# trzy/FasterRCNN

Hardware: AMD Instinct MI355X
Metric: images/sec (600x1000) Faster-RCNN VGG-16 inference (higher is better)
Workload: dtype f32 (float32 tensors and accumulation; 15 GEMM layers in the f32x3 split-operand emulation = two fp16 terms per block-scaled operand, three fp16 MFMAs per product; 0 in f32x6 = three bf16 terms, six bf16 MFMAs; the other 2 on exact-f32 MFMA; strict exact-f32 everywhere: config.strict_f32_images_per_

## Files before the change

fasterrcnn_amd/csrc/api.hip:

```cpp
#include "common.h"
#include <algorithm>
#include <cmath>
#include <cstring>
#include <string>
#include <vector>
#include <new>

namespace frcnn {

static thread_local std::string g_hip_error;
void set_hip_error(hipError_t e) { g_hip_error = hipGetErrorString(e); }

static size_t align_up(size_t v, size_t a) { return (v + a - 1) / a * a; }

struct EventRec { int cls; hipEvent_t start, stop; };

}

using namespace frcnn;

struct frcnn_ctx {
    int max_h = 0, max_w = 0, max_rois = 0, max_images = 0;
    int max_fh = 0, max_fw = 0, a_cap = 0, pre_cap = 0;
    void* slab = nullptr;
// ... 435 lines not shown
    if (!out) return FRCNN_EINVAL;
    const unsigned* c = x3_saturation_counter();
    *out = c ? (unsigned long long)*reinterpret_cast<const volatile unsigned*>(c) : 0ull;
    return FRCNN_OK;
}

int frcnn_conv_nhwc_x3g(const float* d_x, const float* d_wp, const float* d_bias, const float* d_residual, float* d_y,
                        int N, int H, int W, int cin, int cout, int ksize, int stride, int pad, unsigned flags,
                        const float* d_xmax, const float* d_wmax, float* d_ymax, void* d_ws, size_t ws_bytes, void* stream)
{
    if (!d_x || !d_wp || !d_bias || !d_y || !d_xmax || !d_wmax) return FRCNN_EINVAL;
    if (flags & FRCNN_POOL2) return FRCNN_EUNSUPPORTED;
    const GatherX3 x3{d_xmax, d_wmax, d_ymax, nullptr, (flags & FRCNN_X3G_WSPLIT) != 0};
    return launch_conv_gather(d_x, d_wp, d_bias, d_residual, d_y, N, H, W, cin, cout, ksize, stride, pad, flags,
                              d_ws, ws_bytes, as_stream(stream), FRCNN_CONV_F32X3G, &x3);
}

int frcnn_pack_conv_x3g_weights(const float* d_wp, const float* d_wmax, void* d_out, int taps, int cout, int cin, void* stream)
{
    if (taps < 1 || cout < 1) return FRCNN_EINVAL;
    return launch_pack_x3g_weights(d_wp, d_wmax, d_out, (long long)taps * cout, cin, as_stream(stream));
}

int frcnn_conv_nhwc_x3g_tickets(const float* d_x, const float* d_wp, const float* d_bias, const float* d_residual, float* d_y,
                                int N, int H, int W, int cin, int cout, int ksize, int stride, int pad, unsigned flags,
                                const float* d_xmax, const float* d_wmax, float* d_ymax, void* d_ws, size_t ws_bytes,
                                unsigned* d_tile_counters, void* stream)
{
    static_assert(FRCNN_X3G_TILE_COUNTERS == GX_TILE_COUNTERS, "one bound on both sides of the ABI");
    if (!d_x || !d_wp || !d_bias || !d_y || !d_xmax || !d_wmax || !d_tile_counters) return FRCNN_EINVAL;
    if (flags & FRCNN_POOL2) return FRCNN_EUNSUPPORTED;
    const GatherX3 x3{d_xmax, d_wmax, d_ymax, d_tile_counters, (flags & FRCNN_X3G_WSPLIT) != 0};
    return launch_conv_gather(d_x, d_wp, d_bias, d_residual, d_y, N, H, W, cin, cout, ksize, stride, pad, flags,
                              d_ws, ws_bytes, as_stream(stream), FRCNN_CONV_F32X3G, &x3);
}

int frcnn_tensor_absmax(const float* d_x, long long n, float* d_out, void* stream)
{
    if (!d_x || !d_out) return FRCNN_EINVAL;
    return launch_tensor_absmax(d_x, n, d_out, as_stream(stream));
}

int frcnn_conv7x7_s2_c3(const float* d_x, const float* d_wp, const float* d_bias, float* d_y, int H, int W,
                        int cout, unsigned flags, void* stream)
{
    if (!d_x || !d_wp || !d_bias || !d_y) return FRCNN_EINVAL;
    return launch_conv7x7_s2_c3(d_x, d_wp, d_bias, d_y, H, W, cout, flags, as_stream(stream));
}

int frcnn_maxpool3x3_s2_nhwc(const float* d_x, float* d_y, int H, int W, int c, void* stream)
{
    if (!d_x || !d_y) return FRCNN_EINVAL;
    return launch_maxpool3x3_s2(d_x, d_y, H, W, c, as_stream(stream));
}

int frcnn_spatial_mean_nhwc(const float* d_x, float* d_y, int N, int H, int W, int c, void* stream)
{
    if (!d_x || !d_y) return FRCNN_EINVAL;
    return launch_spatial_mean(d_x, d_y, N, H, W, c, as_stream(stream));
}

size_t frcnn_linear_workspace_bytes(int M, int N, int K) { return linear_workspace_bytes(M, N, K); }

int frcnn_linear(const float* d_a, int lda, const float* d_w, const float* d_bias, float* d_y, int ldy,
                 int M, int N, int K, unsigned flags, void* d_ws, size_t ws_bytes, void* stream)
{
    if (!d_a || !d_w || !d_bias || !d_y) return FRCNN_EINVAL;
    return launch_linear(d_a, lda, d_w, d_bias, d_y, ldy, M, N, K, flags, d_ws, ws_bytes, as_stream(stream));
}

int frcnn_softmax_rows(const float* d_x, int ldx, float* d_y, int M, int ncls, void* stream)
{
    if (!d_x || !d_y) return FRCNN_EINVAL;
    return launch_softmax_rows(d_x, ldx, d_y, M, ncls, as_stream(stream));
}

int frcnn_rpn_proposals(frcnn_ctx* ctx, const float* d_head, int ld_head, const float* d_anchor_map,
                        const float* d_valid_map, int fh, int fw, int image_h, int image_w, int pre_nms,
                        int post_nms, float nms_threshold, float min_side, float* d_scores,
                        int32_t* d_sorted_idx, float* d_props, int32_t* d_counts, void* stream)
{
    if (!ctx || !d_head || !d_anchor_map || !d_scores || !d_sorted_idx || !d_props || !d_counts) return FRCNN_EINVAL;
    FRCNN_HIP_TRY(hipMemsetAsync(d_counts, 0, 4 * sizeof(int32_t), as_stream(stream)));
    return launch_rpn_proposals(ctx->ps, d_head, ld_head, d_anchor_map, d_valid_map, fh, fw, image_h, image_w,
                                pre_nms, post_nms, nms_threshold, min_side, d_scores, d_sorted_idx, d_props,
                                d_counts, as_stream(stream));
}

int frcnn_nms(frcnn_ctx* ctx, const float* d_boxes, const float* d_scores, int n, float threshold,
              int max_keep, int32_t* d_keep, int32_t* d_n_keep, void* stream)
{
    if (!ctx || !d_boxes || !d_scores || !d_keep || !d_n_keep) return FRCNN_EINVAL;
    return launch_nms(ctx->ps, d_boxes, d_scores, n, threshold, max_keep, d_keep, d_n_keep, as_stream(stream));
}

int frcnn_roi_pool(const float* d_fm, int fh, int fw, int c, const float* d_rois, const int32_t* d_n_rois,
                   int max_rois, int pooled, float spatial_scale, float* d_out, void* stream)
{
    if (!d_fm || !d_rois || !d_n_rois || !d_out) return FRCNN_EINVAL;
    return launch_roi_pool(d_fm, fh, fw, c, d_rois, d_n_rois, max_rois, pooled, spatial_scale, d_out,
                           as_stream(stream));
}

int frcnn_roi_pool_x3t(const float* d_fm, int fh, int fw, int c, const float* d_rois, const int32_t* d_n_rois, int max_rois, int pooled,
                       float spatial_scale, float* d_cmax, float* d_inv_scale, void* d_rec, int rec_rows, void* stream)
{
    if (!d_fm || !d_rois || !d_n_rois || !d_cmax || !d_inv_scale || !d_rec) return FRCNN_EINVAL;
    return launch_roi_pool_x3t(d_fm, fh, fw, c, d_rois, d_n_rois, max_rois, pooled, spatial_scale, d_cmax, d_inv_scale, d_rec, rec_rows,
                               as_stream(stream));
}

int frcnn_roi_align(const float* d_fm, int fh, int fw, int c, const float* d_rois, const int32_t* d_n_rois, int max_rois,
                    int pooled, float spatial_scale, int sampling_ratio, int aligned, float* d_out, void* stream)
{
    if (!d_fm || !d_rois || !d_n_rois || !d_out) return FRCNN_EINVAL;
    return launch_roi_align(d_fm, fh, fw, c, d_rois, d_n_rois, max_rois, pooled, spatial_scale, sampling_ratio, aligned, d_out,
                            as_stream(stream));
}

int frcnn_roi_align_backward(const float* d_rois, int n_rois, int fh, int fw, int c, int pooled, float spatial_scale,
                             int sampling_ratio, int aligned, const float* d_dout, float* d_dfm, int accumulate, void* stream)
{
    if (!d_dfm || (n_rois > 0 && (!d_rois || !d_dout))) return FRCNN_EINVAL;
    return launch_roi_align_backward(d_rois, n_rois, fh, fw, c, pooled, spatial_scale, sampling_ratio, aligned, d_dout, d_dfm,
                                     accumulate, as_stream(stream));
}

int frcnn_detections(const float* d_props, const float* d_classes, const float* d_deltas,
                     const int32_t* d_n_rois, int max_rois, int ncls, int image_h, int image_w,
                     float score_threshold, float nms_threshold, double* d_out, int32_t* d_out_cnt, void* stream)
{
    if (!d_props || !d_classes || !d_deltas || !d_n_rois || !d_out || !d_out_cnt) return FRCNN_EINVAL;
    return launch_detections(d_props, d_classes, d_deltas, d_n_rois, max_rois, ncls, image_h, image_w,
                             score_threshold, nms_threshold, d_out, d_out_cnt, as_stream(stream));
}

int frcnn_label_proposals(const float* d_props, const int32_t* d_n_props, int max_props,
                          const float* d_gt_boxes, const int32_t* d_gt_class_idx, int n_gt, int num_classes,
                          float min_background_iou, float min_object_iou,
                          const float box_delta_means[4], const float box_delta_stds[4],
                          float* d_out_props, int32_t* d_out_class_idx, float* d_out_gt_classes,
                          float* d_out_gt_box_deltas, int32_t* d_out_count, void* stream)
{
    if ((!d_props && max_props > 0) || !d_n_props || !d_gt_boxes || !d_gt_class_idx || !box_delta_means || !box_delta_stds ||
        !d_out_props || !d_out_class_idx || !d_out_gt_classes || !d_out_gt_box_deltas || !d_out_count)
        return FRCNN_EINVAL;
    if (!(min_background_iou < min_object_iou)) return FRCNN_EINVAL;
    return launch_label_proposals(d_props, d_n_props, max_props, d_gt_boxes, d_gt_class_idx, n_gt, num_classes,
                                  min_background_iou, min_object_iou, box_delta_means, box_delta_stds, d_out_props,
                                  d_out_class_idx, d_out_gt_classes, d_out_gt_box_deltas, d_out_count, as_stream(stream));
}

int frcnn_gather_rows(const float* d_src, const int32_t* d_idx, int n, int row_floats, float* d_dst, void* stream)
{
    if (n > 0 && (!d_src || !d_idx || !d_dst)) return FRCNN_EINVAL;
    return launch_gather_rows(d_src, d_idx, n, row_floats, d_dst, as_stream(stream));
}

int frcnn_rpn_loss(const float* d_head, int ld_head, int cells, const int32_t* d_sample, int n_sample,
                   const float* d_rpn_map, float* d_losses, float* d_grad_head, void* stream)
{
    if (!d_head || (n_sample > 0 && !d_sample) || !d_rpn_map || !d_losses) return FRCNN_EINVAL;
    return launch_rpn_loss(d_head, ld_head, cells, d_sample, n_sample, d_rpn_map, d_losses, d_grad_head, as_stream(stream));
}

int frcnn_detector_loss(const float* d_classes, const float* d_deltas, const float* d_gt_classes,
// ... 371 lines not shown
    proposal_scratch_carve(c->ps, ps_base, c->a_cap, c->pre_cap, 2048);
    *out = c;
    return FRCNN_OK;
}

int frcnn_ctx_create_proposals(frcnn_ctx** out, int max_image_h, int max_image_w)
{
    if (!out || max_image_h < 16 || max_image_w < 16) return FRCNN_EINVAL;
    frcnn_ctx* c = new (std::nothrow) frcnn_ctx();
    if (!c) return FRCNN_ENOMEM;
    c->max_h = max_image_h; c->max_w = max_image_w; c->max_rois = 0;
    c->max_fh = cdiv(max_image_h, 16); c->max_fw = cdiv(max_image_w, 16);
    c->a_cap = c->max_fh * c->max_fw * 9;
    if (c->a_cap < 16384) c->a_cap = 16384;
    c->pre_cap = 16384;
    const size_t total = align_up(proposal_scratch_bytes(c->a_cap, c->pre_cap, 2048), 256);
    hipError_t e = hipMalloc(&c->slab, total);
    if (e != hipSuccess) { set_hip_error(e); delete c; return FRCNN_ENOMEM; }
    c->slab_bytes = total;
    proposal_scratch_carve(c->ps, c->slab, c->a_cap, c->pre_cap, 2048);
    *out = c;
    return FRCNN_OK;
}

void frcnn_ctx_destroy(frcnn_ctx* ctx)
{
    if (!ctx) return;
    for (auto& r : ctx->recs) { (void)hipEventDestroy(r.start); (void)hipEventDestroy(r.stop); }
    for (auto e : ctx->free_events) (void)hipEventDestroy(e);
    if (ctx->slab) (void)hipFree(ctx->slab);
    if (ctx->wino_ws) (void)hipFree(ctx->wino_ws);
    if (ctx->wx_ws) (void)hipFree(ctx->wx_ws);
    if (ctx->x3f_cmax) (void)hipFree(ctx->x3f_cmax);
    if (ctx->roi_rec) (void)hipFree(ctx->roi_rec);
    if (ctx->rx_rec) (void)hipFree(ctx->rx_rec);
    if (ctx->rx_ws) (void)hipFree(ctx->rx_ws);
    if (ctx->rx_aux) (void)hipFree(ctx->rx_aux);
    if (ctx->gx_max) (void)hipFree(ctx->gx_max);
    if (ctx->gx_cnt) (void)hipFree(ctx->gx_cnt);
    delete ctx;
}

size_t frcnn_ctx_bytes(const frcnn_ctx* ctx) { return ctx ? ctx->slab_bytes + ctx->wino_ws_bytes + ctx->wx_ws_bytes + ctx->rx_rec_bytes + ctx->rx_ws_bytes + (ctx->roi_rec ? (size_t)ctx->rec_rows * (49 * 512 + 4096) * 6 : 0) : 0; }

int frcnn_ctx_timing_enable(frcnn_ctx* ctx, int enable)
{
    if (!ctx) return FRCNN_EINVAL;
    ctx->timing = enable != 0;
    return FRCNN_OK;
}

int frcnn_ctx_timing_read(frcnn_ctx* ctx, double ms[FRCNN_NUM_KCLASS], int64_t launches[FRCNN_NUM_KCLASS], int reset)
{
    if (!ctx || !ms || !launches) return FRCNN_EINVAL;
    for (auto& r : ctx->recs) {
        FRCNN_HIP_TRY(hipEventSynchronize(r.stop));
        float t = 0.f;
        FRCNN_HIP_TRY(hipEventElapsedTime(&t, r.start, r.stop));
        ctx->t_ms[r.cls] += t;
        ctx->t_cnt[r.cls] += 1;
        ctx->free_events.push_back(r.start);
        ctx->free_events.push_back(r.stop);
    }
    ctx->recs.clear();
    for (int i = 0; i < FRCNN_NUM_KCLASS; ++i) { ms[i] = ctx->t_ms[i]; launches[i] = ctx->t_cnt[i]; }
    if (reset) for (int i = 0; i < FRCNN_NUM_KCLASS; ++i) { ctx->t_ms[i] = 0; ctx->t_cnt[i] = 0; }
    return FRCNN_OK;
}

int frcnn_ctx_tensor(frcnn_ctx* c, int which, void** d_ptr, size_t* bytes)
{
    if (!c || !d_ptr || !bytes) return FRCNN_EINVAL;
    const size_t fmsz = (size_t)c->last_fh * c->last_fw;
    switch (which) {
        case 0: *d_ptr = c->fm; *bytes = fmsz * c->last_c * 4; break;
        case 1: *d_ptr = c->rpn_head; *bytes = fmsz * 128 * 4; break;
        case 2: *d_ptr = c->scores; *bytes = fmsz * 9 * 4; break;
        case 3: *d_ptr = c->sorted_idx; *bytes = (size_t)c->last_pre * 4; break;
        case 4: *d_ptr = c->roi_out; *bytes = (size_t)c->last_post * 49 * c->last_c * 4; break;
        case 5: *d_ptr = c->fc2_out; *bytes = (size_t)c->last_post * c->last_vec * 4; break;
        case 6: *d_ptr = c->anchor_map; *bytes = fmsz * 9 * 16; break;
        case 7: *d_ptr = c->valid_map; *bytes = fmsz * 9 * 4; break;
        case 8: *d_ptr = c->head_logits; *bytes = (size_t)c->last_post * c->last_head_ld * 4; break;
        default: return FRCNN_EINVAL;
    }
    return FRCNN_OK;
}

namespace {
int ensure_wino_ws(frcnn_ctx* c)
{
    if (c->wino_ws) return FRCNN_OK;
    size_t need = 0;
    const int shapes[5][3] = {{4, 128, 256}, {4, 256, 256}, {8, 256, 512}, {8, 512, 512}, {16, 512, 512}};
    for (auto& sh : shapes) {
        const size_t b = c->max_h > 0 ? conv3x3_winograd_workspace_bytes(1, c->max_h / sh[0], c->max_w / sh[0], sh[1], sh[2]) : 0;
        if (b > need) need = b;
    }
    const int rois = c->max_rois > c->max_head_rois ? c->max_rois : c->max_head_rois;
    const size_t b1 = c->max_fh > 0 ? conv3x3_winograd_workspace_bytes(1, c->max_fh, c->max_fw, 1024, 1024) : 0;
    const size_t b2 = rois > 0 ? conv3x3_winograd_workspace_bytes(rois, 4, 4, 512, 512) : 0;
    if (b1 > need) need = b1;
    if (b2 > need) need = b2;
    if (need == 0) return FRCNN_EINVAL;
    hipError_t e = hipMalloc(&c->wino_ws, need);
    if (e != hipSuccess) { set_hip_error(e); c->wino_ws = nullptr; return FRCNN_ENOMEM; }
    c->wino_ws_bytes = need;
    return FRCNN_OK;
}

int run_winograd_layer(frcnn_ctx* c, const float* x, const float* u, const float* b, float* y, int N, int h, int w, int ci, int co,
                       unsigned flags, hipStream_t s)
{
    float *V = nullptr, *M = nullptr;
    int r = winograd_plan(N, h, w, ci, co, flags, c->wino_ws, c->wino_ws_bytes, &V, &M);
    if (r) return r;
    { Scope _t(c, 6, s); r = launch_winograd_input(x, V, N, h, w, ci, s); }
    if (r) return r;
    { Scope _g(c, 7, s); r = launch_winograd_gemm(V, u, M, N, h, w, ci, co, s); }
    if (r) return r;
    Scope _o(c, 6, s);
    return launch_winograd_output(M, b, y, N, h, w, co, flags, s);
}

int ensure_wx_ws(frcnn_ctx* c, size_t layer_need, hipStream_t s)
{
    if (c->wx_ws && layer_need <= c->wx_ws_bytes) return FRCNN_OK;
    size_t need = layer_need;
    const int shapes[4][4] = {{c->max_h / 8, c->max_w / 8, 256, 512}, {c->max_h / 8, c->max_w / 8, 512, 512},
                              {c->max_fh, c->max_fw, 512, 512}, {c->max_fh, c->max_fw, 1024, 1024}};
    for (auto& sh : shapes) {
        const size_t b = conv3x3_winograd_x6_workspace_bytes(1, sh[0], sh[1], sh[2], sh[3]);
        if (b > need) need = b;
    }
    if (need == 0) return FRCNN_EINVAL;
    if (c->wx_ws) {
        FRCNN_HIP_TRY(hipStreamSynchronize(s));
        (void)hipFree(c->wx_ws);
        c->wx_ws = nullptr; c->wx_ws_bytes = 0;
    }
    hipError_t e = hipMalloc(&c->wx_ws, need);
    if (e != hipSuccess) { set_hip_error(e); c->wx_ws = nullptr; return FRCNN_ENOMEM; }
    e = hipMemsetAsync(c->wx_ws, 0, need, s);
    if (e != hipSuccess) { set_hip_error(e); (void)hipFree(c->wx_ws); c->wx_ws = nullptr; return FRCNN_EHIP; }
    c->wx_ws_bytes = need;
    return FRCNN_OK;
}

int ensure_fc_records(frcnn_ctx* c, hipStream_t s)
{
    if (c->roi_rec) return FRCNN_OK;
    const size_t b1 = (size_t)c->rec_rows * 49 * 512 * 6, b2 = (size_t)c->rec_rows * 4096 * 6;
    const size_t b3 = align_up((size_t)c->rec_rows * sizeof(float), 256), b4 = align_up((size_t)c->max_fh * c->max_fw * sizeof(float), 256);
    void* p = nullptr;
    hipError_t e = hipMalloc(&p, b1 + b2 + 2 * b3 + b4);
    if (e != hipSuccess) { set_hip_error(e); return FRCNN_ENOMEM; }
    e = hipMemsetAsync(p, 0, b1 + b2 + 2 * b3 + b4, s);
    if (e != hipSuccess) { set_hip_error(e); (void)hipFree(p); return FRCNN_EHIP; }
    c->roi_rec = p;
    c->fc1_rec = static_cast<unsigned char*>(p) + b1;
    c->roi_inv = reinterpret_cast<float*>(static_cast<unsigned char*>(p) + b1 + b2);
    c->fc1_inv = reinterpret_cast<float*>(static_cast<unsigned char*>(p) + b1 + b2 + b3);
    c->fm_cmax = reinterpret_cast<float*>(static_cast<unsigned char*>(p) + b1 + b2 + 2 * b3);
    return FRCNN_OK;
}

int run_wino_x6_layer(frcnn_ctx* c, const float* x, const void* urec, const float* b, float* y, int h, int w, int ci, int co,
                      unsigned flags, hipStream_t s, int N = 1)
// ... 16 lines not shown

int run_wino_x3_layer(frcnn_ctx* c, const float* x, const void* ublob, const float* b, float* y, int h, int w, int ci, int co,
                      unsigned flags, hipStream_t s, int N = 1, const float* cmax_ready = nullptr, float* cmax_out = nullptr)
{
    if (N == 1 && !conv3x3_uses_winograd_x6(ci, co)) return FRCNN_EINVAL;
    int r = ensure_wx_ws(c, conv3x3_winograd_x3_workspace_bytes(N, h, w, ci, co), s);
    if (r) return r;
    void *V = nullptr, *G = nullptr;
    float *M = nullptr, *vinv = nullptr, *cmax = nullptr;
    size_t gb = 0;
    r = winograd_x3_plan(N, h, w, ci, co, flags, c->wx_ws, c->wx_ws_bytes, &V, &vinv, &cmax, &M, &G, &gb);
    if (r) return r;
    { Scope _t(c, 8, s); r = launch_winograd_x3_input(x, cmax, V, vinv, N, h, w, ci, s, cmax_ready); }
    if (r) return r;
    { Scope _g(c, 9, s); r = launch_winograd_x3_gemm(V, vinv, ublob, M, N, h, w, ci, co, G, gb, s); }
    if (r) return r;
    Scope _o(c, 8, s);
    return launch_winograd_output(M, b, y, N, h, w, co, flags, s, cmax_out);
}

int ensure_x3f_cmax(frcnn_ctx* c, size_t need, hipStream_t s)
{
    if (c->x3f_cmax && c->x3f_cmax_bytes >= need) return FRCNN_OK;
    if (c->x3f_cmax) { FRCNN_HIP_TRY(hipStreamSynchronize(s)); (void)hipFree(c->x3f_cmax); c->x3f_cmax = nullptr; c->x3f_cmax_bytes = 0; }
    const size_t cap = std::max(need, (size_t)c->max_h * c->max_w * sizeof(float));
    hipError_t e = hipMalloc(reinterpret_cast<void**>(&c->x3f_cmax), 3 * cap);
    if (e != hipSuccess) { set_hip_error(e); c->x3f_cmax = nullptr; return FRCNN_ENOMEM; }
    c->x3f_cmax_bytes = cap;
    return FRCNN_OK;
}
float* x3f_cmax_buffer(frcnn_ctx* c, int which) { return reinterpret_cast<float*>(reinterpret_cast<unsigned char*>(c->x3f_cmax) + (size_t)which * c->x3f_cmax_bytes); }

int run_wino_x3f_layer(frcnn_ctx* c, const float* x, const void* ublob, const float* b, float* y, int h, int w, int ci, int co,
                       unsigned flags, hipStream_t s, const float* cmax_ready = nullptr, float* cmax_out = nullptr)
{
    int r = ensure_x3f_cmax(c, conv3x3_winograd_x3_fused_workspace_bytes(1, h, w), s);
    if (r) return r;
    Scope _w(c, 10, s);
    return launch_conv3x3_winograd_x3_fused(x, ublob, b, y, 1, h, w, ci, co, flags, x3f_cmax_buffer(c, 0), c->x3f_cmax_bytes, s, cmax_ready, cmax_out);
}

int run_wino_fused_layer(frcnn_ctx* c, bool , const float* x, const float* u, const float* b, float* y, int h, int w, int ci,
                         int co, unsigned flags, hipStream_t s, int n_maps = 1)
{
    Scope _w(c, 7, s);
    return launch_conv3x3_winograd_fused(x, u, b, y, h, w, ci, co, flags, s, n_maps);
}

struct BlocksTargetScope {
    explicit BlocksTargetScope(int t, int wino_rows = 0, int x6_tiles = 0) { conv3x3_set_blocks_target(t); linear_batched_set_tile(wino_rows); gemm_x6t_set_tiles(x6_tiles); }
    ~BlocksTargetScope() { conv3x3_set_blocks_target(0); linear_batched_set_tile(0); gemm_x6t_set_tiles(0); }
};
}

int frcnn_vgg16_forward(frcnn_ctx* c, const frcnn_vgg16_weights* w, const frcnn_forward_params* p,
                        const float* d_image, int H, int W, const float* d_anchor_map,
                        const float* d_valid_map, float* d_props, float* d_classes, float* d_deltas,
                        int32_t* d_counts, void* stream)
{
    if (!c || !w || !p || !d_image || !d_props || !d_classes || !d_deltas || !d_counts) return FRCNN_EINVAL;
    if (H < 16 || W < 16 || H > c->max_h || W > c->max_w) return FRCNN_EINVAL;
    if (p->post_nms < 1 || p->post_nms > c->max_rois || p->pre_nms < 1 || p->pre_nms > c->pre_cap) return FRCNN_EINVAL;
    if (w->num_classes < 2 || w->num_classes > FRCNN_MAX_NUM_CLASSES) return FRCNN_EUNSUPPORTED;
    for (int i = 0; i < 13; ++i) if (!w->conv_w[i] || !w->conv_b[i]) return FRCNN_EINVAL;
    if (!w->rpn_conv_w || !w->rpn_conv_b || !w->rpn_head_w || !w->rpn_head_b || !w->fc1_w || !w->fc1_b ||
        !w->fc2_w || !w->fc2_b || !w->head_w || !w->head_b)
        return FRCNN_EINVAL;
    hipStream_t s = as_stream(stream);
    const unsigned R = FRCNN_RELU, RP = FRCNN_RELU | FRCNN_POOL2;
    int rc;
    if (p->math_mode != FRCNN_MATH_F32 && p->math_mode != FRCNN_MATH_F32_WINOGRAD) return FRCNN_EINVAL;
    if (p->conv_blocks_target < 0) return FRCNN_EINVAL;
    if (p->fc_math_mode != FRCNN_FC_F32 && p->fc_math_mode != FRCNN_FC_F32X6T && p->fc_math_mode != FRCNN_FC_F32X3T) return FRCNN_EINVAL;
    if ((p->roi_op != FRCNN_ROI_POOL && p->roi_op != FRCNN_ROI_ALIGN) || p->roi_sampling_ratio > 2) return FRCNN_EINVAL;
    if (p->winograd_tile_rows != 0 && p->winograd_tile_rows != 64 && p->winograd_tile_rows != 128) return FRCNN_EINVAL;
    if (p->x6_gemm_tiles < 0 || p->x6_gemm_tiles > 2) return FRCNN_EINVAL;
    if ((p->winograd_x3_mask & ~p->winograd_x6_mask) != 0) return FRCNN_EINVAL;
    BlocksTargetScope target_scope(p->conv_blocks_target, p->winograd_tile_rows, p->x6_gemm_tiles);
    const bool wino = p->math_mode == FRCNN_MATH_F32_WINOGRAD;
    if (p->winograd_x6_mask != 0 && (!wino || (p->winograd_x6_mask & ~0x3FFE) != 0)) return FRCNN_EINVAL;
    if (p->winograd_x3f_mask != 0 && (!wino || (p->winograd_x3f_mask & ~0x3FFE) != 0 || (p->winograd_x3f_mask & p->winograd_x6_mask) != 0)) return FRCNN_EINVAL;
    int layer_index = 0;
    const float* cmax_ready = nullptr;
    size_t cmax_used = 0, cmax_cleared = 0;
    if (wino && ((p->winograd_x3f_mask | (p->winograd_x3_mask & p->winograd_x6_mask)) & 0x1FFE) != 0) {
        int r0 = ensure_x3f_cmax(c, (size_t)H * W * sizeof(float), s);
        if (r0) return r0;
        static const int co_of[13] = {0, 64, 128, 128, 256, 256, 256, 512, 512, 512, 512, 512, 512};
        static const bool pool_of[13] = {false, true, false, true, false, false, true, false, false, true, false, false, false};
        size_t want = 0;
        int eh = H, ew = W;
        for (int li = 1; li <= 12; ++li) {
            const bool f3 = ((p->winograd_x3f_mask >> li) & 1) != 0;
            const bool t3 = !f3 && ((p->winograd_x6_mask >> li) & 1) && ((p->winograd_x3_mask >> li) & 1);
            const unsigned efl = FRCNN_RELU | (pool_of[li] ? FRCNN_POOL2 : 0u);
            if (pool_of[li]) { eh /= 2; ew /= 2; }
            if ((f3 || t3) && (f3 || winograd_output_emits_cmax(co_of[li], efl))) want += ((size_t)eh * ew + 63) & ~(size_t)63;
        }
        if (want > 2 * c->x3f_cmax_bytes / sizeof(float)) return FRCNN_EINVAL;
        cmax_cleared = want;
        if (want) FRCNN_HIP_TRY(hipMemsetAsync(x3f_cmax_buffer(c, 1), 0, cmax_cleared * sizeof(float), s));
    }
    auto conv3 = [&](const float* xin, const float* wgt, const float* bs, float* yout, int hh, int ww, int ci, int co,
                     unsigned fl) -> int {
        ++layer_index;
        const float* in_cmax = cmax_ready;
        cmax_ready = nullptr;
        const bool is_x3f = wino && ((p->winograd_x3f_mask >> layer_index) & 1);
        const bool is_x3 = wino && !is_x3f && ((p->winograd_x6_mask >> layer_index) & 1) && ((p->winograd_x3_mask >> layer_index) & 1);
        float* out_cmax = nullptr;
        if ((is_x3f || is_x3) && layer_index != FRCNN_X6_RPN_TRUNK_BIT && (fl & FRCNN_RELU) && (is_x3f || winograd_output_emits_cmax(co, fl))) {
            const int oh = (fl & FRCNN_POOL2) ? hh / 2 : hh, ow = (fl & FRCNN_POOL2) ? ww / 2 : ww;
            const size_t need = ((size_t)oh * ow + 63) & ~(size_t)63;
            out_cmax = x3f_cmax_buffer(c, 1) + cmax_used;
            cmax_used += need;
            if (cmax_used > cmax_cleared) return FRCNN_EINVAL;
        }
        int r1;
        if (is_x3f)
            r1 = run_wino_x3f_layer(c, xin, wgt, bs, yout, hh, ww, ci, co, fl, s, in_cmax, out_cmax);
        else if (is_x3)
            r1 = run_wino_x3_layer(c, xin, wgt, bs, yout, hh, ww, ci, co, fl, s, 1, in_cmax, out_cmax);
        else if (wino && ((p->winograd_x6_mask >> layer_index) & 1))
            r1 = run_wino_x6_layer(c, xin, wgt, bs, yout, hh, ww, ci, co, fl, s);
        else
            r1 = -9999;
        if (r1 != -9999) {
            if (r1 == FRCNN_OK) cmax_ready = out_cmax;
            return r1;
        }
        if (wino && conv3x3_uses_winograd_fused(ci, co)) {
            return run_wino_fused_layer(c, p->conv_blocks_target == 0, xin, wgt, bs, yout, hh, ww, ci, co, fl, s);
        }
        Scope _d(c, 0, s);
        return launch_conv3x3_nhwc(xin, wgt, bs, yout, hh, ww, ci, co, fl, c->conv_ws, c->conv_ws_bytes, s);
    };
#define STEP(cls, call) do { Scope _sc(c, cls, s); rc = (call); } while (0); if (rc) return rc
#define CONV(call) do { rc = (call); } while (0); if (rc) return rc

    float *A = c->act_a, *B = c->act_b;
    int h = H, wd = W;
    float* c11_cmax = (wino && ((p->winograd_x3f_mask >> 1) & 1)) ? x3f_cmax_buffer(c, 0) : nullptr;
    STEP(1, launch_conv3x3_c3(d_image, w->conv_w[0], w->conv_b[0], A, h, wd, 64, R, s, c11_cmax));
    cmax_ready = c11_cmax;
    CONV(conv3(A, w->conv_w[1], w->conv_b[1], B, h, wd, 64, 64, RP));   h /= 2; wd /= 2;
    CONV(conv3(B, w->conv_w[2], w->conv_b[2], A, h, wd, 64, 128, R));
    CONV(conv3(A, w->conv_w[3], w->conv_b[3], B, h, wd, 128, 128, RP)); h /= 2; wd /= 2;
    CONV(conv3(B, w->conv_w[4], w->conv_b[4], A, h, wd, 128, 256, R));
    CONV(conv3(A, w->conv_w[5], w->conv_b[5], B, h, wd, 256, 256, R));
    CONV(conv3(B, w->conv_w[6], w->conv_b[6], A, h, wd, 256, 256, RP)); h /= 2; wd /= 2;
    CONV(conv3(A, w->conv_w[7], w->conv_b[7], B, h, wd, 256, 512, R));
    CONV(conv3(B, w->conv_w[8], w->conv_b[8], A, h, wd, 512, 512, R));
    CONV(conv3(A, w->conv_w[9], w->conv_b[9], B, h, wd, 512, 512, RP)); h /= 2; wd /= 2;
    CONV(conv3(B, w->conv_w[10], w->conv_b[10], A, h, wd, 512, 512, R));
    CONV(conv3(A, w->conv_w[11], w->conv_b[11], B, h, wd, 512, 512, R));
    CONV(conv3(B, w->conv_w[12], w->conv_b[12], c->fm, h, wd, 512, 512, R));
    const float* fm_cmax_ready = cmax_ready;
    const int fh = h, fw = wd;
    c->last_fh = fh; c->last_fw = fw; c->last_pre = p->pre_nms; c->last_post = p->post_nms; c->last_c = 512; c->last_vec = 4096;

    CONV(conv3(c->fm, w->rpn_conv_w, w->rpn_conv_b, c->rpn_trunk, fh, fw, 512, 512, R));
    STEP(2, launch_linear(c->rpn_trunk, 512, w->rpn_head_w, w->rpn_head_b, c->rpn_head, 128, fh * fw, 45, 512,
                          0u, c->lin_ws, c->lin_ws_bytes, s));
    const float* amap = d_anchor_map;
    const float* vmap = d_valid_map;
    if (!amap || !vmap) {
        if (c->anc_h != H || c->anc_w != W || c->anc_fh != fh || c->anc_fw != fw) {
            STEP(5, launch_anchors(H, W, fh, fw, 16, c->anchor_map, c->valid_map, s));
            c->anc_h = H; c->anc_w = W; c->anc_fh = fh; c->anc_fw = fw;
        }
        amap = c->anchor_map; vmap = c->valid_map;
    }
    FRCNN_HIP_TRY(hipMemsetAsync(d_counts, 0, 4 * sizeof(int32_t), s));
    STEP(3, launch_rpn_proposals(c->ps, c->rpn_head, 128, amap, p->allow_edge_proposals ? nullptr : vmap, fh, fw,
                                 H, W, p->pre_nms, p->post_nms, p->rpn_nms_threshold, p->min_side, c->scores,
                                 c->sorted_idx, d_props, d_counts, s));

    const int R_ = p->post_nms;
    const bool fc_x6t = p->fc_math_mode == FRCNN_FC_F32X6T;
    const bool fc_x3t = p->fc_math_mode == FRCNN_FC_F32X3T;
    if (fc_x6t || fc_x3t) { rc = ensure_fc_records(c, s); if (rc) return rc; }
    if (fc_x3t) {
        const int rr = c->rec_rows;
        const size_t w1rec = x3t_record_bytes(4096, 49 * 512), w2rec = x3t_record_bytes(4096, 4096);
        const float* w1inv = reinterpret_cast<const float*>(reinterpret_cast<const unsigned char*>(w->fc1_w) + w1rec);
        const float* w2inv = reinterpret_cast<const float*>(reinterpret_cast<const unsigned char*>(w->fc2_w) + w2rec);
        if (p->roi_op == FRCNN_ROI_ALIGN) {
            STEP(4, launch_roi_align(c->fm, fh, fw, 512, d_props, d_counts + 2, R_, 7, 1.0f / 16.0f, p->roi_sampling_ratio, 0, c->roi_out, s));
            STEP(2, launch_rows_scale_x3t(c->roi_out, 49 * 512, 0, c->roi_inv, R_, rr, 49 * 512, 1, s));
            STEP(2, launch_split_rows_x3t(c->roi_out, 49 * 512, 0, c->roi_inv, c->roi_rec, R_, rr, 49 * 512, 1, s));
        } else {
            STEP(4, launch_roi_pool_x3t(c->fm, fh, fw, 512, d_props, d_counts + 2, R_, 7, 1.0f / 16.0f,
                                        fm_cmax_ready ? const_cast<float*>(fm_cmax_ready) : c->fm_cmax, c->roi_inv, c->roi_rec, rr, s, fm_cmax_ready != nullptr));
        }
        STEP(2, launch_gemm_x3t(c->roi_rec, c->roi_inv, rr, 0, 0, w->fc1_w, w1inv, 4096, 0, 0, w->fc1_b, nullptr, c->fc1_out, 4096, 0, R_, 4096,
                                49 * 512, 1, R, c->lin_ws, c->lin_ws_bytes, s, 0));
        STEP(2, launch_rows_scale_x3t(c->fc1_out, 4096, 0, c->fc1_inv, R_, rr, 4096, 1, s));
        STEP(2, launch_split_rows_x3t(c->fc1_out, 4096, 0, c->fc1_inv, c->fc1_rec, R_, rr, 4096, 1, s));
        STEP(2, launch_gemm_x3t(c->fc1_rec, c->fc1_inv, rr, 0, 0, w->fc2_w, w2inv, 4096, 0, 0, w->fc2_b, nullptr, c->fc2_out, 4096, 0, R_, 4096,
                                4096, 1, R, c->lin_ws, c->lin_ws_bytes, s, 2));
    } else
    if (fc_x6t) {
        const int rr = c->rec_rows;
        if (p->roi_op == FRCNN_ROI_ALIGN) {
            STEP(4, launch_roi_align(c->fm, fh, fw, 512, d_props, d_counts + 2, R_, 7, 1.0f / 16.0f, p->roi_sampling_ratio, 0, c->roi_out, s));
            STEP(2, launch_split_rows_x6t(c->roi_out, 49 * 512, 0, c->roi_rec, R_, rr, 49 * 512, 1, s));
        } else {
            STEP(4, launch_roi_pool_x6t(c->fm, fh, fw, 512, d_props, d_counts + 2, R_, 7, 1.0f / 16.0f, c->roi_rec, rr, s));
        }
        static const int fc_tiles = []() { const char* e = frcnn_knob("FRCNN_FC_TILES"); return e ? atoi(e) : 0; }();
        STEP(2, launch_gemm_x6t(c->roi_rec, rr, 0, w->fc1_w, 4096, 0, w->fc1_b, nullptr, c->fc1_out, 4096, 0, R_, 4096, 49 * 512, 1, R,
                                c->lin_ws, c->lin_ws_bytes, s, fc_tiles));
        STEP(2, launch_split_rows_x6t(c->fc1_out, 4096, 0, c->fc1_rec, R_, rr, 4096, 1, s));
        STEP(2, launch_gemm_x6t(c->fc1_rec, rr, 0, w->fc2_w, 4096, 0, w->fc2_b, nullptr, c->fc2_out, 4096, 0, R_, 4096, 4096, 1, R,
                                c->lin_ws, c->lin_ws_bytes, s, fc_tiles));
    } else
    {
        if (p->roi_op == FRCNN_ROI_ALIGN) {
            STEP(4, launch_roi_align(c->fm, fh, fw, 512, d_props, d_counts + 2, R_, 7, 1.0f / 16.0f, p->roi_sampling_ratio, 0, c->roi_out, s));
        } else {
            STEP(4, launch_roi_pool(c->fm, fh, fw, 512, d_props, d_counts + 2, R_, 7, 1.0f / 16.0f, c->roi_out, s));
        }
        STEP(2, launch_linear(c->roi_out, 49 * 512, w->fc1_w, w->fc1_b, c->fc1_out, 4096, R_, 4096, 49 * 512, R,
                              c->lin_ws, c->lin_ws_bytes, s));
        STEP(2, launch_linear(c->fc1_out, 4096, w->fc2_w, w->fc2_b, c->fc2_out, 4096, R_, 4096, 4096, R,
                              c->lin_ws, c->lin_ws_bytes, s));
    }
    const int ncls = w->num_classes, nd = (ncls - 1) * 4;
    const int hld = cdiv(ncls + nd, 128) * 128;
    c->last_head_ld = hld;
    STEP(2, launch_linear(c->fc2_out, 4096, w->head_w, w->head_b, c->head_logits, hld, R_, ncls + nd, 4096, 0u,
                          c->lin_ws, c->lin_ws_bytes, s));
    STEP(5, launch_head_finish(c->head_logits, hld, R_, ncls, nd, d_classes, d_deltas, s));
#undef STEP
#undef CONV
    return FRCNN_OK;
}

namespace {
int run_conv1x1_x6(frcnn_ctx* c, const float* x, const void* wrec, const float* bias, const float* residual, float* y, int N, int h,
                   int w, int cin, int cout, int stride, unsigned flags, int cls, hipStream_t s, int ksize = 1)
{
    if (cin % 16 != 0 || cout % 4 != 0 || (ksize != 1 && ksize != 3)) return FRCNN_EINVAL;
    const int ho = (h - 1) / stride + 1, wo = (w - 1) / stride + 1;
    const int K = ksize == 3 ? 9 * cin : cin;
    const long long rows = (long long)N * ho * wo;
    if (rows > 0x7fffffffLL / 8) return FRCNN_EINVAL;
    const int M = (int)rows;
    const int Mp = cdiv(M, gemm_x6t_row_tile(M)) * gemm_x6t_row_tile(M), Np = cdiv(cout, gemm_x6t_col_tile(cout)) * gemm_x6t_col_tile(cout);
    const size_t need = x6t_record_bytes(Mp, K), gneed = gemm_x6t_workspace_bytes(M, cout, K, 1);
    if (need > c->rx_rec_bytes) {
        if (c->rx_rec) { FRCNN_HIP_TRY(hipStreamSynchronize(s)); (void)hipFree(c->rx_rec); c->rx_rec = nullptr; c->rx_rec_bytes = 0; }
        hipError_t e = hipMalloc(&c->rx_rec, need);
        if (e != hipSuccess) { set_hip_error(e); c->rx_rec = nullptr; return FRCNN_ENOMEM; }
        c->rx_rec_bytes = need;
    }
    if (gneed > c->rx_ws_bytes) {
        if (c->rx_ws) { FRCNN_HIP_TRY(hipStreamSynchronize(s)); (void)hipFree(c->rx_ws); c->rx_ws = nullptr; c->rx_ws_bytes = 0; }
        hipError_t e = hipMalloc(&c->rx_ws, gneed);
        if (e != hipSuccess) { set_hip_error(e); c->rx_ws = nullptr; return FRCNN_ENOMEM; }
        c->rx_ws_bytes = gneed;
    }
    int rc;
    { Scope _t(c, 8, s); rc = ksize == 3 ? launch_split_patches3x3_x6t(x, c->rx_rec, N, h, w, cin, stride, Mp, s)
                                        : launch_split_pixels_x6t(x, c->rx_rec, N, h, w, cin, stride, Mp, s); }
    if (rc) return rc;
    Scope _g(c, cls, s);
    return launch_gemm_x6t(c->rx_rec, Mp, 0, wrec, Np, 0, bias, residual, y, cout, 0, M, cout, K, 1, flags, c->rx_ws, c->rx_ws_bytes, s);
}

int run_conv1x1_x3(frcnn_ctx* c, const float* x, const void* wblob, const float* bias, const float* residual, float* y, int N, int h,
                   int w, int cin, int cout, int stride, unsigned flags, int cls, hipStream_t s, int ksize = 1)
{
    if (cin % 16 != 0 || cout % 4 != 0 || (ksize != 1 && ksize != 3)) return FRCNN_EINVAL;
    const int ho = (h - 1) / stride + 1, wo = (w - 1) / stride + 1;
    const int K = ksize == 3 ? 9 * cin : cin;
    const long long rows = (long long)N * ho * wo;
    if (rows > 0x7fffffffLL / 8) return FRCNN_EINVAL;
    const int M = (int)rows;
    const int Mp = cdiv(M, gemm_x6t_row_tile(M)) * gemm_x6t_row_tile(M), Np = cdiv(cout, gemm_x6t_col_tile(cout)) * gemm_x6t_col_tile(cout);
    const size_t need = x3t_record_bytes(Mp, K), gneed = gemm_x3t_workspace_bytes(M, cout, K, 1);
    const size_t aneed = (size_t)Mp + (size_t)N * h * w;
    if (need > c->rx_rec_bytes) {
        if (c->rx_rec) { FRCNN_HIP_TRY(hipStreamSynchronize(s)); (void)hipFree(c->rx_rec); c->rx_rec = nullptr; c->rx_rec_bytes = 0; }
        hipError_t e = hipMalloc(&c->rx_rec, need);
        if (e != hipSuccess) { set_hip_error(e); c->rx_rec = nullptr; return FRCNN_ENOMEM; }
        c->rx_rec_bytes = need;
    }
    if (gneed > c->rx_ws_bytes) {
        if (c->rx_ws) { FRCNN_HIP_TRY(hipStreamSynchronize(s)); (void)hipFree(c->rx_ws); c->rx_ws = nullptr; c->rx_ws_bytes = 0; }
        hipError_t e = hipMalloc(&c->rx_ws, gneed);
        if (e != hipSuccess) { set_hip_error(e); c->rx_ws = nullptr; return FRCNN_ENOMEM; }
        c->rx_ws_bytes = gneed;
    }
    if (aneed > c->rx_aux_floats) {
        if (c->rx_aux) { FRCNN_HIP_TRY(hipStreamSynchronize(s)); (void)hipFree(c->rx_aux); c->rx_aux = nullptr; c->rx_aux_floats = 0; }
        hipError_t e = hipMalloc(reinterpret_cast<void**>(&c->rx_aux), aneed * sizeof(float));
        if (e != hipSuccess) { set_hip_error(e); c->rx_aux = nullptr; return FRCNN_ENOMEM; }
        c->rx_aux_floats = aneed;
    }
    float* ainv = c->rx_aux;
    float* cmax = c->rx_aux + Mp;
    int rc;
    {
        Scope _t(c, 8, s);
        static const bool two_pass = frcnn_knob("FRCNN_SPLIT_TWO_PASS") != nullptr;
        rc = (ksize == 3 || two_pass) ? launch_pixel_absmax(x, cmax, (long long)N * h * w, cin, s) : FRCNN_OK;
        if (!rc) rc = ksize == 3 ? launch_split_patches3x3_x3t(x, cmax, c->rx_rec, ainv, N, h, w, cin, stride, Mp, s)
                                 : launch_split_pixels_x3t(x, two_pass ? cmax : nullptr, c->rx_rec, ainv, N, h, w, cin, stride, Mp, s);
    }
    if (rc) return rc;
    const float* winv = reinterpret_cast<const float*>(static_cast<const unsigned char*>(wblob) + x3t_record_bytes(Np, K));
    Scope _g(c, cls, s);
    return launch_gemm_x3t(c->rx_rec, ainv, Mp, 0, 0, wblob, winv, Np, 0, 0, bias, residual, y, cout, 0, M, cout, K, 1, flags, c->rx_ws,
                           c->rx_ws_bytes, s);
}
// ... 448 lines not shown
```

fasterrcnn_amd/csrc/common.h:

```cpp
#pragma once
#include <hip/hip_runtime.h>
#include <stdint.h>
#include <stddef.h>
#include <stdlib.h>
#include "../../include/frcnn_hip.h"

typedef float f32x4  __attribute__((ext_vector_type(4)));
typedef float f32x16 __attribute__((ext_vector_type(16)));

inline const char* frcnn_knob(const char* name)
{
#ifdef FRCNN_EXPERIMENT_KNOBS
    return getenv(name);
#else
    (void)name;
    return nullptr;
#endif
}

namespace frcnn {

void set_hip_error(hipError_t e);

inline int check_launch() {
    hipError_t e = hipGetLastError();
    if (e != hipSuccess) { set_hip_error(e); return FRCNN_EHIP; }
    return FRCNN_OK;
}

#define FRCNN_HIP_TRY(expr)                                   \
    do {                                                      \
        hipError_t _e = (expr);                               \
        if (_e != hipSuccess) { ::frcnn::set_hip_error(_e); return FRCNN_EHIP; } \
    } while (0)

static inline int cdiv(int a, int b) { return (a + b - 1) / b; }

struct DeviceOnce { unsigned char done[64]; };
inline int set_max_dynamic_lds(DeviceOnce& once, const void* kern, size_t bytes)
{
    int dev = 0;
    FRCNN_HIP_TRY(hipGetDevice(&dev));
    if (dev < 0 || dev >= 64) return FRCNN_EINVAL;
    if (!once.done[dev]) {
        FRCNN_HIP_TRY(hipFuncSetAttribute(kern, hipFuncAttributeMaxDynamicSharedMemorySize, (int)bytes));
        once.done[dev] = 1;
    }
    return FRCNN_OK;
}
#define FRCNN_MAX_LDS_ONCE(kern, bytes)                                                                  \
    do {                                                                                                 \
        static ::frcnn::DeviceOnce _once = {};                                                           \
        const int _rc = ::frcnn::set_max_dynamic_lds(_once, reinterpret_cast<const void*>(kern), (bytes)); \
        if (_rc) return _rc;                                                                             \
    } while (0)

static inline bool conv3x3_uses_winograd(int cin, int cout) { return cin >= 128 && cout >= 256 && cin % 16 == 0 && cout % 128 == 0; }
static inline bool resnet_block_uses_winograd(int width, int stride) { return stride == 1 && width >= 256 && width % 128 == 0; }

struct KernelTimer;

}

namespace frcnn {

int launch_anchors(int image_h, int image_w, int fh, int fw, int feature_pixels,
                   float* anchor_map, float* valid_map, hipStream_t s);

int launch_pack_conv3x3(const float* w, float* wp, int cout, int cin, hipStream_t s);
int launch_pack_conv3x3_c3(const float* w, float* wp, int cout, hipStream_t s);
int launch_pack_fc_chw_to_hwc(const float* w, float* wp, int out_f, int c, int phw, hipStream_t s);
int launch_pack_stack_rows(const float* w1, const float* b1, int n1, const float* w2, const float* b2,
                           int n2, int k, int n_pad, float* wo, float* bo, hipStream_t s);

int launch_conv3x3_c3(const float* x, const float* wp, const float* b, float* y, int H, int W,
                      int cout, unsigned flags, hipStream_t s, float* cmax_out = nullptr);
size_t conv3x3_workspace_bytes(int H, int W, int cin, int cout);
int conv3x3_blocks_target();
void conv3x3_set_blocks_target(int target);
int launch_conv3x3_nhwc(const float* x, const float* wp, const float* b, float* y, int H, int W,
                        int cin, int cout, unsigned flags, void* ws, size_t ws_bytes, hipStream_t s);
int launch_maxpool2x2(const float* x, float* y, int H, int W, int c, hipStream_t s);

size_t conv_gather_workspace_bytes(int N, int H, int W, int cin, int cout, int R, int stride, int pad);
#define FRCNN_CONV_F32X3G 2
static constexpr int GX_TILE_COUNTERS = 16384;
struct GatherX3 { const float* xmax; const float* wmax; float* ymax; unsigned* tile_counters = nullptr; bool wsplit = false; bool trusted = false; };
int launch_pack_x3g_weights(const float* wp, const float* wmax, void* out, long long rows, int cin, hipStream_t s);
int launch_conv_gather(const float* x, const float* wp, const float* bias, const float* residual, float* y,
                       int N, int H, int W, int cin, int cout, int R, int stride, int pad, unsigned flags,
                       void* ws, size_t ws_bytes, hipStream_t s, int math = FRCNN_GRAD_F32, const GatherX3* x3 = nullptr);
unsigned* x3_saturation_counter();
int launch_tensor_absmax(const float* x, long long n, float* out, hipStream_t s);
int launch_conv7x7_s2_c3(const float* x, const float* wp, const float* b, float* y, int H, int W, int cout,
                         unsigned flags, hipStream_t s);
int launch_maxpool3x3_s2(const float* x, float* y, int H, int W, int c, hipStream_t s);
int launch_spatial_mean(const float* x, float* y, int N, int H, int W, int c, hipStream_t s);
int launch_fold_bn_pack(const float* w, const float* gamma, const float* beta, const float* mean, const float* var,
                        float eps, int cout, int cin, int ksize, float* wp, float* bp, hipStream_t s);

size_t linear_workspace_bytes(int M, int N, int K);
int launch_linear(const float* a, int lda, const float* w, const float* bias, float* y, int ldy,
                  int M, int N, int K, unsigned flags, void* ws, size_t ws_bytes, hipStream_t s);
int launch_linear_batched(const float* a, int lda, size_t a_stride, const float* w, size_t w_stride, float* y, int ldy,
                          size_t y_stride, int M, int N, int K, int batches, hipStream_t s);
void linear_batched_set_tile(int rows);
size_t conv3x3_winograd_workspace_bytes(int N, int H, int W, int cin, int cout);
int launch_pack_conv3x3_winograd(const float* w, const float* scale, float* u, int cout, int cin, hipStream_t s);
int launch_pack_conv3x3_winograd_taps(const float* wp, float* u, int cout, int cin, int data_gradient, hipStream_t s);
int launch_conv3x3_winograd(const float* x, const float* u, const float* b, float* y, int N, int H, int W, int cin, int cout,
                            unsigned flags, void* ws, size_t ws_bytes, hipStream_t s);
int winograd_plan(int N, int H, int W, int cin, int cout, unsigned flags, void* ws, size_t ws_bytes, float** V, float** M);
int launch_winograd_input(const float* x, float* V, int N, int H, int W, int cin, hipStream_t s);
int launch_winograd_gemm(const float* V, const float* u, float* M, int N, int H, int W, int cin, int cout, hipStream_t s);
int launch_winograd_output(const float* M, const float* b, float* y, int N, int H, int W, int cout, unsigned flags, hipStream_t s,
                           float* cmax_out = nullptr);
bool winograd_output_emits_cmax(int cout, unsigned flags);
static inline bool conv3x3_uses_winograd_fused(int cin, int cout) { return cin >= 64 && cin % 16 == 0 && cout >= 64 && cout % 64 == 0; }
static inline bool resnet_block_uses_winograd_fused(int n_maps, int width, int stride)
{
    return n_maps == 1 && stride == 1 && conv3x3_uses_winograd_fused(width, width);
}
bool conv3x3_winograd_fused_ok(int H, int W, int cin, int cout);
int launch_pack_conv3x3_winograd_fused(const float* w, const float* scale, float* u, int cout, int cin, hipStream_t s);
int launch_pack_conv3x3_winograd_fused_taps(const float* wp, float* u, int cout, int cin, int data_gradient, hipStream_t s);
int launch_conv3x3_winograd_fused(const float* x, const float* u, const float* b, float* y, int H, int W, int cin, int cout,
                                  unsigned flags, hipStream_t s, int n_maps = 1);
int gemm_x6t_row_tile(int M);
int gemm_x6t_col_tile(int N);
size_t x6t_record_bytes(int rows_padded, int K);
int launch_split_rows_x6t(const float* a, int lda, size_t a_batch_floats, void* rec, int R, int rows_padded, int K, int batches, hipStream_t s);
bool gemm_x6t_shape_ok(int M, int N, int K, int batches);
size_t gemm_x6t_workspace_bytes(int M, int N, int K, int batches);
void gemm_x6t_set_tiles(int mode);
int launch_gemm_x6t(const void* a_rec, int a_rows, size_t a_batch_bytes, const void* b_rec, int b_rows, size_t b_batch_bytes,
                    const float* bias, const float* residual, float* c, int ldc, size_t c_batch_floats, int M, int N, int K, int batches,
                    unsigned flags, void* ws, size_t ws_bytes, hipStream_t s, int tiles_mode = -1);
int launch_split_pixels_x6t(const float* x, void* rec, int N, int H, int W, int C, int stride, int rows_padded, hipStream_t s);
int gemm_x6t_get_tiles();
int launch_gemm_x6t_reduce(const float* ws, const float* bias, const float* residual, float* c, int ldc, size_t c_batch_floats, int M, int N,
                           int batches, int splits, int relu, hipStream_t s);
size_t x3t_record_bytes(int rows_padded, int K);
int launch_rows_scale_x3t(const float* a, int lda, size_t a_batch_floats, float* inv_scale, int R, int rows_padded, int K, int batches,
                          hipStream_t s);
int launch_split_rows_x3t(const float* a, int lda, size_t a_batch_floats, const float* inv_scale, void* rec, int R, int rows_padded, int K,
                          int batches, hipStream_t s);
int launch_split_pixels_x3t(const float* x, const float* cmax, void* rec, float* inv, int N, int H, int W, int C, int stride, int rows_padded,
                            hipStream_t s);
int launch_split_patches3x3_x3t(const float* x, const float* cmax, void* rec, float* inv, int N, int H, int W, int C, int stride,
                                int rows_padded, hipStream_t s);
size_t gemm_x3t_workspace_bytes(int M, int N, int K, int batches);
int launch_gemm_x3t(const void* a_rec, const float* a_inv, int a_rows, size_t a_batch_bytes, size_t a_inv_batch, const void* b_rec,
                    const float* b_inv, int b_rows, size_t b_batch_bytes, size_t b_inv_batch, const float* bias, const float* residual,
                    float* c, int ldc, size_t c_batch_floats, int M, int N, int K, int batches, unsigned flags, void* ws, size_t ws_bytes,
                    hipStream_t s, int tiles_mode = -1);
size_t x3t_blob_bytes(int rows_padded, int K, int batches);
int launch_pack_rows_x3t(const float* a, int lda, size_t a_batch_floats, void* blob, int R, int rows_padded, int K, int batches, hipStream_t s);
int launch_pixel_absmax(const float* x, float* cmax, long long pixels, int C, hipStream_t s);
size_t conv3x3_winograd_x3_pack_bytes(int cout, int cin);
int launch_pack_conv3x3_winograd_x3(const float* u_f32, void* ublob, int cout, int cin, hipStream_t s);
size_t conv3x3_winograd_x3_workspace_bytes(int N, int H, int W, int cin, int cout);
int winograd_x3_plan(int N, int H, int W, int cin, int cout, unsigned flags, void* ws, size_t ws_bytes, void** V, float** vinv, float** cmax,
                     float** M, void** G, size_t* g_bytes);
int launch_winograd_x3_input(const float* x, float* cmax, void* vrec, float* vinv, int N, int H, int W, int cin, hipStream_t s,
                             const float* cmax_ready = nullptr);
int launch_winograd_x3_gemm(const void* vrec, const float* vinv, const void* ublob, float* M, int N, int H, int W, int cin, int cout, void* gws,
                            size_t gws_bytes, hipStream_t s);
int launch_conv3x3_winograd_x3(const float* x, const void* ublob, const float* b, float* y, int N, int H, int W, int cin, int cout,
                               unsigned flags, void* ws, size_t ws_bytes, hipStream_t s,
                               const float* cmax_ready = nullptr, float* cmax_out = nullptr);
size_t conv3x3_winograd_x3_fused_workspace_bytes(int N, int H, int W);
int launch_conv3x3_winograd_x3_fused(const float* x, const void* ublob, const float* b, float* y, int N, int H, int W, int cin, int cout,
                                     unsigned flags, void* ws, size_t ws_bytes, hipStream_t s, const float* cmax_ready = nullptr,
                                     float* cmax_out = nullptr);
int launch_roi_pool_x3t(const float* fm, int fh, int fw, int c, const float* rois, const int32_t* n_rois, int max_rois, int pooled,
                        float scale, float* cmax, float* inv, void* rec, int rec_rows, hipStream_t s, bool cmax_ready = false);
bool conv3x3_uses_winograd_x6(int cin, int cout);
size_t conv3x3_winograd_x6_pack_bytes(int cout, int cin);
size_t conv3x3_winograd_x6_workspace_bytes(int N, int H, int W, int cin, int cout);
int launch_pack_conv3x3_winograd_x6(const float* w, const float* scale, void* urec, int cout, int cin, hipStream_t s);
int launch_winograd_x6_input(const float* x, void* vrec, int N, int H, int W, int cin, hipStream_t s);
int launch_winograd_x6_gemm(const void* vrec, const void* urec, float* M, int N, int H, int W, int cin, int cout, void* gws, size_t gws_bytes, hipStream_t s);
int winograd_x6_plan(int N, int H, int W, int cin, int cout, unsigned flags, void* ws, size_t ws_bytes, void** V, float** M, void** G, size_t* g_bytes);
int launch_conv3x3_winograd_x6(const float* x, const void* urec, const float* b, float* y, int N, int H, int W, int cin, int cout,
                               unsigned flags, void* ws, size_t ws_bytes, hipStream_t s);
int launch_split_patches3x3_x6t(const float* x, void* rec, int N, int H, int W, int C, int stride, int rows_padded, hipStream_t s);
int launch_softmax_rows(const float* x, int ldx, float* y, int M, int ncls, hipStream_t s);
int launch_head_finish(const float* x, int ldx, int M, int ncls, int ndelta, float* classes,
                       float* deltas, hipStream_t s);

struct ProposalScratch {
    unsigned long long* keys;
    float*    boxes_all;
    float*    cand_boxes;
    float*    cand_scores;
    unsigned long long* mask;
    int32_t*  keep;
    int       a_cap, pre_cap, post_cap;
};
size_t proposal_scratch_bytes(int a_cap, int pre_cap, int post_cap);
void   proposal_scratch_carve(ProposalScratch& ps, void* base, int a_cap, int pre_cap, int post_cap);

int launch_rpn_proposals(const ProposalScratch& ps, const float* head, int ld_head,
                         const float* anchor_map, const float* valid_map, int fh, int fw,
                         int image_h, int image_w, int pre_nms, int post_nms, float nms_thr,
                         float min_side, float* scores, int32_t* sorted_idx, float* props,
                         int32_t* counts, hipStream_t s);
int launch_nms(const ProposalScratch& ps, const float* boxes, const float* scores, int n, float thr,
               int max_keep, int32_t* keep, int32_t* n_keep, hipStream_t s);

int launch_roi_pool(const float* fm, int fh, int fw, int c, const float* rois, const int32_t* n_rois,
                    int max_rois, int pooled, float scale, float* out, hipStream_t s);
int launch_roi_pool_x6t(const float* fm, int fh, int fw, int c, const float* rois, const int32_t* n_rois,
                        int max_rois, int pooled, float scale, void* rec, int rec_rows, hipStream_t s);

int launch_roi_align(const float* fm, int fh, int fw, int c, const float* rois, const int32_t* n_rois, int max_rois, int pooled,
                     float scale, int sampling_ratio, int aligned, float* out, hipStream_t s);
int launch_roi_align_backward(const float* rois, int n_rois, int fh, int fw, int c, int pooled, float scale, int sampling_ratio,
                              int aligned, const float* dout, float* dfm, int accumulate, hipStream_t s);

int launch_rpn_targets(const float* anchor_map, const float* valid_map, int A, const float* gt, int M,
                       double obj_thr, double bg_thr, float* rpn_map, int32_t* obj_idx, int32_t* bg_idx,
                       int32_t* counts, void* ws, hipStream_t s);

size_t preprocess_workspace_bytes(int H, int W, int Ho, int Wo);
int launch_preprocess(const unsigned char* rgb, int H, int W, int Ho, int Wo, int bgr, int flip, float scaling,
                      const float* means, const float* stds, float* out, unsigned char* out_u8, void* ws,
                      size_t ws_bytes, hipStream_t s);

int launch_detections(const float* props, const float* classes, const float* deltas,
                      const int32_t* n_rois, int max_rois, int ncls, int image_h, int image_w,
                      float score_thr, float nms_thr, double* out, int32_t* out_cnt, hipStream_t s);

size_t gemm_tn_workspace_bytes(int M, int N, int R, int taps);
int launch_gemm_tn(const float* A, int lda, const float* B, int ldb, float* C, int ldc, int M, int N, int R,
                   void* ws, size_t ws_bytes, hipStream_t s, int math = FRCNN_GRAD_F32);
int launch_conv3x3_wgrad(const float* x, const float* dz, float* dwp, int H, int W, int cin, int cout,
                         void* ws, size_t ws_bytes, hipStream_t s, int math = FRCNN_GRAD_F32);
int launch_label_proposals(const float* props, const int32_t* n_props, int max_props, const float* gt,
                           const int32_t* gt_cls, int M, int ncls, float bg_thr, float obj_thr,
                           const float means[4], const float stds[4], float* out_props, int32_t* out_cls,
                           float* out_onehot, float* out_deltas, int32_t* out_count, hipStream_t s);
int launch_gather_rows(const float* src, const int32_t* idx, int n, int row_floats, float* dst, hipStream_t s);
int launch_rpn_loss(const float* head, int ld, int cells, const int32_t* sample, int n_sample, const float* rpn_map,
                    float* losses, float* d_head, hipStream_t s);
int launch_detector_loss(const float* classes, const float* deltas, const float* gt_onehot, const float* gt_deltas,
                         int S, int ncls, float* losses, float* d_logits, int ld, hipStream_t s);
int launch_relu_backward(float* dy, const float* y, size_t n, hipStream_t s);
int launch_dropout(float* x, size_t n, float p, float scale, const uint64_t* seed, uint32_t stream_id, uint32_t rank,
                   uint8_t* keep_out, hipStream_t s);
int launch_dropout_relu_backward(float* dy, const float* y, size_t n, float scale, hipStream_t s);
int launch_add_inplace(float* a, const float* b, size_t n, hipStream_t s);
int launch_maxpool2x2_backward(const float* x, const float* dy, float* dx, int H, int W, int C, hipStream_t s);
size_t roi_pool_backward_workspace_bytes(int n_rois, int pooled, int C);
int launch_roi_pool_backward(const float* fm, int fh, int fw, int C, const float* rois, int n_rois, int pooled,
                             float scale, const float* dout, float* dfm, int accumulate, void* ws, size_t ws_bytes,
                             hipStream_t s);
int launch_transpose(const float* x, int ldi, float* y, int ldo, int rows, int cols, hipStream_t s);
int launch_pack_conv3x3_dgrad(const float* wp, float* wd, int cout, int cin, hipStream_t s);
int launch_conv_wgrad(const float* x, const float* dz, float* dwp, int N, int H, int W, int cin, int cout, int ks, int stride,
                      int pad, void* ws, size_t ws_bytes, hipStream_t s, int math = FRCNN_GRAD_F32);
size_t conv_dgrad_workspace_bytes(int N, int H, int W, int cin, int cout, int R, int stride, int pad);
int launch_conv_dgrad(const float* dz, const float* wd, const float* residual, float* dx, int N, int H, int W, int cin,
                      int cout, int R, int stride, int pad, void* ws, size_t ws_bytes, hipStream_t s, int math = FRCNN_GRAD_F32);
int launch_pack_conv_dgrad(const float* wp, float* wd, int taps, int cout, int cin, hipStream_t s);
int launch_scale_rows(const float* src, const float* scale, float* dst, int taps, int cout, int cin, hipStream_t s);
int launch_bn_scale_shift(const float* gamma, const float* beta, const float* mean, const float* var, float eps, int c,
                          float* scale, float* shift, hipStream_t s);
int launch_spatial_mean_backward(const float* dy, float* dx, int N, int H, int W, int c, hipStream_t s);
int launch_sgd(float* w, const float* g, float* buf, size_t n, float lr, float momentum, float weight_decay, int first,
               hipStream_t s);
int launch_sgd_fold(float* w, const float* g, float* buf, size_t n, float lr, float momentum, float weight_decay, int first,
                    const float* scale, float* folded, int cout, int cin, hipStream_t s);

}
```

fasterrcnn_amd/csrc/conv.hip:

```cpp
#include "common.h"
#include <cstdlib>
#include <type_traits>

namespace frcnn {

static constexpr int LDK = 20;
static constexpr int HC  = 34;

template <int WM, int WN>
struct ConvCfg {
    static constexpr int TR  = 2 * WM;
    static constexpr int BN  = 64 * WN;
    static constexpr int HR  = TR + 2;
    static constexpr int HALO_F = HR * HC * LDK;
    static constexpr int WT_F   = BN * LDK;
    static constexpr int NHP = HR * HC * 4;
    static constexpr int NH  = (NHP + 255) / 256;
    static constexpr int NW  = BN * 4 / 256;
    static constexpr size_t LDS_BYTES = (size_t)(2 * HALO_F + 2 * WT_F) * sizeof(float);
};

template <int WM, int WN, bool POOL>
__global__ __launch_bounds__(256)
void conv3x3_mfma_kernel(const float* __restrict__ x, const float* __restrict__ wp,
// ... 225 lines not shown
                               float* __restrict__ y, int H, int W, int Cout, int relu, int pool)
{
    const int C4 = Cout >> 2;
    const int Ho = pool ? H >> 1 : H, Wo = pool ? W >> 1 : W;
    const size_t total = (size_t)Ho * Wo * C4;
    const size_t plane = (size_t)H * W * Cout;
    for (size_t i = (size_t)blockIdx.x * 256 + threadIdx.x; i < total; i += (size_t)gridDim.x * 256) {
        const int c4 = (int)(i % C4);
        const size_t p = i / C4;
        const int ox = (int)(p % Wo), oy = (int)(p / Wo);
        const f32x4 bv = reinterpret_cast<const f32x4*>(bias)[c4];
        f32x4 best;
        const int np = pool ? 4 : 1;
        for (int q = 0; q < np; ++q) {
            const int iy = pool ? 2 * oy + (q >> 1) : oy, ix = pool ? 2 * ox + (q & 1) : ox;
            const size_t off = ((size_t)iy * W + ix) * Cout + 4 * c4;
            f32x4 v = *reinterpret_cast<const f32x4*>(ws + off);
            for (int k = 1; k < ksplit; ++k) {
                const f32x4 t = *reinterpret_cast<const f32x4*>(ws + k * plane + off);
#pragma unroll
                for (int j = 0; j < 4; ++j) v[j] += t[j];
            }
            if (q == 0) best = v;
            else {
#pragma unroll
                for (int j = 0; j < 4; ++j) best[j] = fmaxf(best[j], v[j]);
            }
        }
#pragma unroll
        for (int j = 0; j < 4; ++j) {
            float t = best[j] + bv[j];
            best[j] = relu ? fmaxf(t, 0.f) : t;
        }
        reinterpret_cast<f32x4*>(y)[i] = best;
    }
}

__global__ __launch_bounds__(256)
void conv3x3_c3_kernel(const float* __restrict__ x, const float* __restrict__ wp,
                       const float* __restrict__ bias, float* __restrict__ y,
                       int H, int W, int Cout, int relu)
{
    const int pix = blockIdx.x * 256 + threadIdx.x;
    if (pix >= H * W) return;
    const int yy = pix / W, xx = pix - yy * W;
    float in[27];
#pragma unroll
    for (int ci = 0; ci < 3; ++ci)
#pragma unroll
        for (int r = 0; r < 3; ++r)
#pragma unroll
            for (int s = 0; s < 3; ++s) {
                const int gy = yy + r - 1, gx = xx + s - 1;
                const bool inb = gy >= 0 && gy < H && gx >= 0 && gx < W;
                in[ci * 9 + r * 3 + s] = inb ? x[((size_t)ci * H + gy) * W + gx] : 0.f;
            }
    for (int og = 0; og < (Cout >> 4); ++og) {
        float acc[16];
#pragma unroll
        for (int o = 0; o < 16; ++o) acc[o] = 0.f;
        const float* wg = wp + og * 16;
#pragma unroll
        for (int k = 0; k < 27; ++k)
#pragma unroll
            for (int o = 0; o < 16; ++o) acc[o] = fmaf(in[k], wg[k * Cout + o], acc[o]);
        float* out = y + (size_t)pix * Cout + og * 16;
#pragma unroll
        for (int o4 = 0; o4 < 4; ++o4) {
            f32x4 v;
#pragma unroll
            for (int j = 0; j < 4; ++j) {
                float t = acc[o4 * 4 + j] + bias[og * 16 + o4 * 4 + j];
                v[j] = relu ? fmaxf(t, 0.f) : t;
            }
            *reinterpret_cast<f32x4*>(out + 4 * o4) = v;
        }
    }
}

typedef float c3_f32x2 __attribute__((ext_vector_type(2)));
template <bool RELU, bool CMAX, int BPC>
__global__ __launch_bounds__(256, BPC)
void conv3x3_c3_p_kernel(const float* __restrict__ x, const float* __restrict__ wp, const float* __restrict__ bias,
                         float* __restrict__ y, int H, int W, float* __restrict__ cmax_out, int tiles_x, int ntiles)
{
    constexpr int COUT = 64, SEG = 64, ROWS = 2, LW = 68;
    constexpr int NEL = 3 * (ROWS + 2) * (SEG + 2);
    __shared__ __attribute__((aligned(16))) float in_s[2][3][ROWS + 2][LW];
    const int tid = threadIdx.x, q = tid & 15, g = tid >> 4;
    int e_off[4], e_rc[4];
    const int HW = H * W;
#pragma unroll
    for (int k = 0; k < 4; ++k) {
        const int e = tid + 256 * k;
        const int ci = e / ((ROWS + 2) * (SEG + 2)), rem = e - ci * (ROWS + 2) * (SEG + 2);
        const int r = rem / (SEG + 2), c = rem - r * (SEG + 2);
        e_off[k] = ci * HW + (r - 1) * W + c - 1;
        e_rc[k] = e < NEL ? (c | (r << 8) | (((ci * (ROWS + 2) + r) * LW + c) << 12)) : -1;
    }
    auto fetch = [&](int tile, float (&v)[4]) {
        const int ty = tile / tiles_x, tx = tile - ty * tiles_x;
        const int y0 = ty * ROWS, x0 = tx * SEG;
        const int base = y0 * W + x0;
#pragma unroll
        for (int k = 0; k < 4; ++k) {
            const int gy = y0 + ((e_rc[k] >> 8) & 7) - 1, gx = x0 + (e_rc[k] & 127) - 1;
            const bool inb = e_rc[k] >= 0 && gy >= 0 && gy < H && gx >= 0 && gx < W;
            v[k] = inb ? x[base + e_off[k]] : 0.f;
        }
    };
    auto stage = [&](int buf, const float (&v)[4]) {
        float* dst = &in_s[buf][0][0][0];
#pragma unroll
        for (int k = 0; k < 4; ++k)
            if (e_rc[k] >= 0) dst[e_rc[k] >> 12] = v[k];
    };
    f32x4 wq[27];
#pragma unroll
    for (int k = 0; k < 27; ++k) wq[k] = *reinterpret_cast<const f32x4*>(wp + k * COUT + 4 * q);
    const f32x4 bq = *reinterpret_cast<const f32x4*>(bias + 4 * q);
    int tile = blockIdx.x;
    if (tile >= ntiles) return;
    {
        float v[4];
        fetch(tile, v);
        stage(0, v);
    }
    __syncthreads();
    int buf = 0;
    for (; tile < ntiles; tile += gridDim.x) {
        const int next = tile + gridDim.x;
        float nv_[4];
        if (next < ntiles) fetch(next, nv_);
        const int ty = tile / tiles_x, tx = tile - ty * tiles_x;
        const int y0 = ty * ROWS, x0 = tx * SEG;
#pragma unroll
        for (int row = 0; row < ROWS; ++row) {
            const int yy = y0 + row;
            if (yy >= H) break;
            c3_f32x2 acc[4][2];
#pragma unroll
            for (int i = 0; i < 4; ++i) acc[i][0] = acc[i][1] = c3_f32x2{0.f, 0.f};
#pragma unroll
            for (int ci = 0; ci < 3; ++ci)
#pragma unroll
                for (int r = 0; r < 3; ++r) {
                    const float* src = &in_s[buf][ci][row + r][4 * g];
                    const f32x4 a = *reinterpret_cast<const f32x4*>(src);
                    c3_f32x2 pr[3];
                    pr[0] = c3_f32x2{a[0], a[1]}; pr[1] = c3_f32x2{a[2], a[3]};
                    pr[2] = *reinterpret_cast<const c3_f32x2*>(src + 4);
#pragma unroll
                    for (int s_ = 0; s_ < 3; ++s_) {
                        const f32x4 w4 = wq[ci * 9 + r * 3 + s_];
                        const c3_f32x2 wlo = {w4[0], w4[1]}, whi = {w4[2], w4[3]};
#pragma unroll
                        for (int i = 0; i < 4; ++i) {
                            const int k = i + s_;
                            if ((k & 1) == 0) {
                                asm("v_pk_fma_f32 %0, %1, %2, %0 op_sel_hi:[0,1,1]" : "+v"(acc[i][0]) : "v"(pr[k >> 1]), "v"(wlo));
                                asm("v_pk_fma_f32 %0, %1, %2, %0 op_sel_hi:[0,1,1]" : "+v"(acc[i][1]) : "v"(pr[k >> 1]), "v"(whi));
                            } else {
                                asm("v_pk_fma_f32 %0, %1, %2, %0 op_sel:[1,0,0]" : "+v"(acc[i][0]) : "v"(pr[k >> 1]), "v"(wlo));
                                asm("v_pk_fma_f32 %0, %1, %2, %0 op_sel:[1,0,0]" : "+v"(acc[i][1]) : "v"(pr[k >> 1]), "v"(whi));
                            }
                        }
                    }
                }
// ... 83 lines not shown
    dim3 grid(cdiv(W, 32), cdiv(H, C::TR), cout_tiles * ksplit);
    auto kern = conv3x3_mfma_kernel<WM, WN, POOL>;
    FRCNN_MAX_LDS_ONCE(kern, C::LDS_BYTES);
    hipLaunchKernelGGL(kern, grid, dim3(256), C::LDS_BYTES, s, x, wp, b, y, H, W, cin, cout, relu, cout_tiles,
                       cdiv(nchunks, ksplit), ksplit > 1 ? ws : (float*)nullptr);
    return check_launch();
}

static thread_local int g_blocks_target_override = 0;
void conv3x3_set_blocks_target(int target) { g_blocks_target_override = target > 0 ? target : 0; }

static int conv_blocks_target()
{
    static int env_target = -1;
    if (env_target < 0) {
        const char* e = frcnn_knob("FRCNN_CONV_BLOCKS_TARGET");
        env_target = e ? atoi(e) : 0;
        if (env_target < 0) env_target = 0;
    }
    if (env_target > 0) return env_target;
    return g_blocks_target_override > 0 ? g_blocks_target_override : 1280;
}

static int choose_ksplit(int H, int W, int cin, int cout)
{
    const bool narrow = (cout % 128) != 0;
    const int tr = narrow ? 8 : 4, bn = narrow ? 64 : 128;
    const int blocks = cdiv(W, 32) * cdiv(H, tr) * (cout / bn);
    const int nchunks = cin / 16;
    const int target = conv_blocks_target();
    if (blocks * 2 > target) return 1;
    if ((size_t)H * W * cout * sizeof(float) > ((size_t)40 << 20)) return 1;
    int k = 1;
    while (k * 2 * blocks <= target && nchunks % (k * 2) == 0 && nchunks / (k * 2) >= 4) k *= 2;
    return k;
}

int conv3x3_choose_ksplit(int H, int W, int cin, int cout) { return choose_ksplit(H, W, cin, cout); }
int conv3x3_blocks_target() { return conv_blocks_target(); }

int launch_conv_splitk_finish(const float* ws, int ksplit, const float* b, float* y, int H, int W, int cout, int relu,
                              int pool, hipStream_t s)
{
    const size_t total = (size_t)(pool ? H / 2 : H) * (pool ? W / 2 : W) * (cout / 4);
    int blocks = (int)((total + 255) / 256);
    if (blocks > 4096) blocks = 4096;
    hipLaunchKernelGGL(conv_splitk_finish_kernel, dim3(blocks), dim3(256), 0, s, ws, ksplit, b, y, H, W, cout, relu, pool);
    return check_launch();
}

size_t conv3x3_workspace_bytes(int H, int W, int cin, int cout)
{
    if (cin % 16 != 0 || cout % 64 != 0 || H < 1 || W < 1) return 0;
    const int k = choose_ksplit(H, W, cin, cout);
    return k > 1 ? (size_t)k * H * W * cout * sizeof(float) : 0;
}

int launch_conv3x3_nhwc(const float* x, const float* wp, const float* b, float* y, int H, int W,
                        int cin, int cout, unsigned flags, void* ws, size_t ws_bytes, hipStream_t s)
{
    if (cin % 16 != 0 || cout % 64 != 0 || H < 1 || W < 1) return FRCNN_EINVAL;
    const int relu = (flags & FRCNN_RELU) ? 1 : 0;
    const bool pool = (flags & FRCNN_POOL2) != 0;
    if (pool && (H < 2 || W < 2)) return FRCNN_EINVAL;
    int ksplit = choose_ksplit(H, W, cin, cout);
    if (ksplit > 1 && (ws == nullptr || ws_bytes < (size_t)ksplit * H * W * cout * sizeof(float))) ksplit = 1;
    float* wsf = static_cast<float*>(ws);
    int rc;
    if (ksplit > 1) {
        rc = (cout % 128 != 0) ? launch_cfg<4, 1, false>(x, wp, b, y, H, W, cin, cout, relu, ksplit, wsf, s)
                               : launch_cfg<2, 2, false>(x, wp, b, y, H, W, cin, cout, relu, ksplit, wsf, s);
        if (rc) return rc;
        return launch_conv_splitk_finish(wsf, ksplit, b, y, H, W, cout, relu, pool ? 1 : 0, s);
    }
    if (cout % 128 != 0) {
        return pool ? launch_cfg<4, 1, true>(x, wp, b, y, H, W, cin, cout, relu, 1, nullptr, s)
                    : launch_cfg<4, 1, false>(x, wp, b, y, H, W, cin, cout, relu, 1, nullptr, s);
    }
    return pool ? launch_cfg<2, 2, true>(x, wp, b, y, H, W, cin, cout, relu, 1, nullptr, s)
                : launch_cfg<2, 2, false>(x, wp, b, y, H, W, cin, cout, relu, 1, nullptr, s);
}

int launch_conv3x3_c3(const float* x, const float* wp, const float* b, float* y, int H, int W,
                      int cout, unsigned flags, hipStream_t s, float* cmax_out)
{
    if (cout % 16 != 0 || H < 1 || W < 1) return FRCNN_EINVAL;
    if (cmax_out && cout != 64) return FRCNN_EINVAL;
    if (cout == 64) {
        const int tiles_x = cdiv(W, 64), tiles_y = cdiv(H, 2);
        if ((long long)tiles_x * tiles_y > 0x7fffffffLL) return FRCNN_EINVAL;
        const int ntiles = tiles_x * tiles_y;
        static const int cus = []() { hipDeviceProp_t p; int d = 0; return (hipGetDevice(&d) == hipSuccess && hipGetDeviceProperties(&p, d) == hipSuccess) ? p.multiProcessorCount : 256; }();
        static const int bpc = []() { const char* e = frcnn_knob("FRCNN_C3_BPC"); return e && atoi(e) == 3 ? 3 : 2; }();
        const int grid = ntiles < bpc * cus ? ntiles : bpc * cus;
        const bool relu = (flags & FRCNN_RELU) != 0;
#define C3P_LAUNCH(R_, C_) do { if (bpc == 3) hipLaunchKernelGGL((conv3x3_c3_p_kernel<R_, C_, 3>), dim3(grid), dim3(256), 0, s, x, wp, b, y, H, W, cmax_out, tiles_x, ntiles); \
                                else hipLaunchKernelGGL((conv3x3_c3_p_kernel<R_, C_, 2>), dim3(grid), dim3(256), 0, s, x, wp, b, y, H, W, cmax_out, tiles_x, ntiles); } while (0)
        if (relu) { if (cmax_out) C3P_LAUNCH(true, true); else C3P_LAUNCH(true, false); }
        else { if (cmax_out) C3P_LAUNCH(false, true); else C3P_LAUNCH(false, false); }
#undef C3P_LAUNCH
        return check_launch();
    }
    dim3 grid(cdiv(H * W, 256), 1);
    hipLaunchKernelGGL(conv3x3_c3_kernel, grid, dim3(256), 0, s, x, wp, b, y, H, W, cout,
                       (flags & FRCNN_RELU) ? 1 : 0);
    return check_launch();
}

int launch_maxpool2x2(const float* x, float* y, int H, int W, int c, hipStream_t s)
{
    if (c % 4 != 0 || H < 2 || W < 2) return FRCNN_EINVAL;
    const size_t total = (size_t)(H / 2) * (W / 2) * (c / 4);
    int blocks = (int)((total + 255) / 256);
    if (blocks > 8192) blocks = 8192;
    hipLaunchKernelGGL(maxpool2x2_kernel, dim3(blocks), dim3(256), 0, s, x, y, H, W, c);
    return check_launch();
}

int launch_pack_conv3x3(const float* w, float* wp, int cout, int cin, hipStream_t s)
{
    if (cout < 1 || cin < 1) return FRCNN_EINVAL;
    const size_t total = (size_t)9 * cout * cin;
    int blocks = (int)((total + 255) / 256);
    if (blocks > 4096) blocks = 4096;
    hipLaunchKernelGGL(pack_conv3x3_kernel, dim3(blocks), dim3(256), 0, s, w, wp, cout, cin);
    return check_launch();
}

int launch_pack_conv3x3_c3(const float* w, float* wp, int cout, hipStream_t s)
{
    if (cout < 1) return FRCNN_EINVAL;
    hipLaunchKernelGGL(pack_conv3x3_c3_kernel, dim3(cdiv(27 * cout, 256)), dim3(256), 0, s, w, wp, cout);
    return check_launch();
}

}
```

fasterrcnn_amd/csrc/gemm_x3t.hip:

```cpp
#include "x3t.h"

namespace frcnn {

typedef _Float16 hx_f16x8 __attribute__((ext_vector_type(8)));

#ifndef HX_ABLATE
#define HX_ABLATE 0
#endif
__global__ __launch_bounds__(256)
void rows_scale_x3t_kernel(const float* __restrict__ a, int lda, size_t a_batch, float* __restrict__ inv_scale, int R, int rows_padded,
                           int K, int batches)
{
    const int lane = threadIdx.x & 63;
    const long long wave = (long long)blockIdx.x * 4 + (threadIdx.x >> 6);
    if (wave >= (long long)batches * rows_padded) return;
    const int row = (int)(wave % rows_padded), batch = (int)(wave / rows_padded);
    float mx = 0.f;
    if (row < R) {
        const float* src = a + (size_t)batch * a_batch + (size_t)row * lda;
        for (int k = 4 * lane; k < K; k += 256) {
            const f32x4 v = *reinterpret_cast<const f32x4*>(src + k);
            mx = fmaxf(fmaxf(mx, fmaxf(fabsf(v[0]), fabsf(v[1]))), fmaxf(fabsf(v[2]), fabsf(v[3])));
        }
    }
#pragma unroll
    for (int off = 32; off >= 1; off >>= 1) mx = fmaxf(mx, __shfl_xor(mx, off));
    float mult, inv;
    hx_row_scale(mx, mult, inv);
    if (lane == 0) inv_scale[(size_t)batch * rows_padded + row] = inv;
}

__global__ __launch_bounds__(256)
void split_rows_x3t_kernel(const float* __restrict__ a, int lda, size_t a_batch, const float* __restrict__ inv_scale,
                           unsigned char* __restrict__ rec, int R, int rbt, int K16, int batches)
{
    const int lane = threadIdx.x & 63;
    const long long wave = (long long)blockIdx.x * 4 + (threadIdx.x >> 6);
    const long long total = (long long)batches * K16 * rbt;
    if (wave >= total) return;
    const int rb = (int)(wave % rbt);
    const long long t = wave / rbt;
    const int chunk = (int)(t % K16), batch = (int)(t / K16);
    const int row = rb * 32 + (lane & 31), k = chunk * 16 + 8 * (lane >> 5);
    float v[8] = {0.f, 0.f, 0.f, 0.f, 0.f, 0.f, 0.f, 0.f};
    if (row < R) {
        const float inv = inv_scale[(size_t)batch * rbt * 32 + row];
        const float mult = hx_mult_of_inv(inv);
        const float* src = a + (size_t)batch * a_batch + (size_t)row * lda + k;
        const f32x4 v0 = *reinterpret_cast<const f32x4*>(src), v1 = *reinterpret_cast<const f32x4*>(src + 4);
#pragma unroll
        for (int j = 0; j < 4; ++j) { v[j] = v0[j] * mult; v[4 + j] = v1[j] * mult; }
    }
    uint4 ph, pl;
    hx_split8(v, ph, pl);
    unsigned char* dst = rec + (size_t)wave * HX_RB + lane * 16;
    *reinterpret_cast<uint4*>(dst) = ph;
    *reinterpret_cast<uint4*>(dst + HX_PIECE) = pl;
}

__global__ __launch_bounds__(256)
void split_pixels_x3t_kernel(const float* __restrict__ x, const float* __restrict__ cmax, unsigned char* __restrict__ rec,
                             float* __restrict__ inv_out, int H, int W, int Ho, int Wo, int C, int stride, int R, int rbt, int K16)
{
    const int lane = threadIdx.x & 63;
    const long long wave = (long long)blockIdx.x * 4 + (threadIdx.x >> 6);
    if (wave >= (long long)K16 * rbt) return;
    const int chunk = (int)(wave % K16), rb = (int)(wave / K16);
    const int row = rb * 32 + (lane & 31), k = chunk * 16 + 8 * (lane >> 5);
    float v[8] = {0.f, 0.f, 0.f, 0.f, 0.f, 0.f, 0.f, 0.f};
    float mult = 1.f, inv = 1.f;
    if (row < R) {
        const int n = row / (Ho * Wo), rem = row - n * (Ho * Wo);
        const int oy = rem / Wo, ox = rem - oy * Wo;
        const size_t pix = ((size_t)n * H + (size_t)oy * stride) * W + (size_t)ox * stride;
        hx_row_scale(cmax[pix], mult, inv);
        const float* src = x + pix * C + k;
        const f32x4 v0 = *reinterpret_cast<const f32x4*>(src), v1 = *reinterpret_cast<const f32x4*>(src + 4);
#pragma unroll
        for (int j = 0; j < 4; ++j) { v[j] = v0[j] * mult; v[4 + j] = v1[j] * mult; }
    }
    if (chunk == 0 && lane < 32) inv_out[row] = inv;
    uint4 ph, pl;
    hx_split8(v, ph, pl);
    unsigned char* dst = rec + ((size_t)chunk * rbt + rb) * HX_RB + lane * 16;
    *reinterpret_cast<uint4*>(dst) = ph;
    *reinterpret_cast<uint4*>(dst + HX_PIECE) = pl;
}

__global__ __launch_bounds__(256)
void split_pixels_x3t_max_kernel(const float* __restrict__ x, unsigned char* __restrict__ rec, float* __restrict__ inv_out, int H, int W, int Ho,
                                 int Wo, int C, int stride, int R, int rbt, int K16)
{
    __shared__ float smax[32];
    const int lane = threadIdx.x & 63, wave = threadIdx.x >> 6;
    const int rb = blockIdx.x;
    auto pixel_of = [&](int row) -> size_t {
        const int n = row / (Ho * Wo), rem = row - n * (Ho * Wo);
        const int oy = rem / Wo, ox = rem - oy * Wo;
        return ((size_t)n * H + (size_t)oy * stride) * W + (size_t)ox * stride;
    };
    {
        const float* src[8];
        float mx[8];
#pragma unroll
        for (int r = 0; r < 8; ++r) {
            const int row = rb * 32 + wave * 8 + r;
            src[r] = row < R ? x + pixel_of(row) * C : nullptr;
            mx[r] = 0.f;
        }
        for (int c = 4 * lane; c < C; c += 256) {
            f32x4 v[8];
#pragma unroll
            for (int r = 0; r < 8; ++r) v[r] = src[r] ? *reinterpret_cast<const f32x4*>(src[r] + c) : f32x4{0.f, 0.f, 0.f, 0.f};
#pragma unroll
            for (int r = 0; r < 8; ++r)
                mx[r] = fmaxf(fmaxf(mx[r], fmaxf(fabsf(v[r][0]), fabsf(v[r][1]))), fmaxf(fabsf(v[r][2]), fabsf(v[r][3])));
        }
#pragma unroll
        for (int r = 0; r < 8; ++r) {
            float m = mx[r];
#pragma unroll
            for (int off = 32; off >= 1; off >>= 1) m = fmaxf(m, __shfl_xor(m, off));
            if (lane == 0) smax[wave * 8 + r] = m;
        }
    }
    __syncthreads();
    const int row = rb * 32 + (lane & 31);
    float mult = 1.f, inv = 1.f;
    const float* src = nullptr;
    if (row < R) {
        hx_row_scale(smax[lane & 31], mult, inv);
        src = x + pixel_of(row) * C + 8 * (lane >> 5);
    }
    if (wave == 0 && lane < 32) inv_out[row] = inv;
    for (int chunk = wave; chunk < K16; chunk += 4) {
        float v[8] = {0.f, 0.f, 0.f, 0.f, 0.f, 0.f, 0.f, 0.f};
        if (src) {
            const f32x4 v0 = *reinterpret_cast<const f32x4*>(src + chunk * 16), v1 = *reinterpret_cast<const f32x4*>(src + chunk * 16 + 4);
#pragma unroll
            for (int j = 0; j < 4; ++j) { v[j] = v0[j] * mult; v[4 + j] = v1[j] * mult; }
// ... 292 lines not shown
    const long long waves = (long long)batches * (K / 16) * (rows_padded / 32);
    const long long blocks = (waves + 3) / 4;
    if (blocks > 0x7fffffffLL) return FRCNN_EINVAL;
    hipLaunchKernelGGL(split_rows_x3t_kernel, dim3((unsigned)blocks), dim3(256), 0, s, a, lda, a_batch_floats, inv_scale,
                       static_cast<unsigned char*>(rec), R, rows_padded / 32, K / 16, batches);
    return check_launch();
}

int launch_split_pixels_x3t(const float* x, const float* cmax, void* rec, float* inv, int N, int H, int W, int C, int stride, int rows_padded,
                            hipStream_t s)
{
    if (N < 1 || H < 1 || W < 1 || C < 16 || C % 16 != 0 || stride < 1 || stride > 2 || rows_padded % 32 != 0 || !inv) return FRCNN_EINVAL;
    const int Ho = (H - 1) / stride + 1, Wo = (W - 1) / stride + 1;
    const long long R = (long long)N * Ho * Wo;
    if (R > rows_padded || R > 0x7fffffffLL) return FRCNN_EINVAL;
    if (!cmax) {
        hipLaunchKernelGGL(split_pixels_x3t_max_kernel, dim3((unsigned)(rows_padded / 32)), dim3(256), 0, s, x, static_cast<unsigned char*>(rec), inv, H, W,
                           Ho, Wo, C, stride, (int)R, rows_padded / 32, C / 16);
        return check_launch();
    }
    const long long waves = (long long)(C / 16) * (rows_padded / 32);
    hipLaunchKernelGGL(split_pixels_x3t_kernel, dim3((unsigned)((waves + 3) / 4)), dim3(256), 0, s, x, cmax, static_cast<unsigned char*>(rec),
                       inv, H, W, Ho, Wo, C, stride, (int)R, rows_padded / 32, C / 16);
    return check_launch();
}

int launch_split_patches3x3_x3t(const float* x, const float* cmax, void* rec, float* inv, int N, int H, int W, int C, int stride,
                                int rows_padded, hipStream_t s)
{
    if (N < 1 || H < 1 || W < 1 || C < 16 || C % 16 != 0 || stride < 1 || stride > 2 || rows_padded % 32 != 0 || !cmax || !inv) return FRCNN_EINVAL;
    const int Ho = (H - 1) / stride + 1, Wo = (W - 1) / stride + 1;
    const long long R = (long long)N * Ho * Wo;
    if (R > rows_padded || R > 0x7fffffffLL) return FRCNN_EINVAL;
    const long long waves = (long long)(9 * C / 16) * (rows_padded / 32);
    hipLaunchKernelGGL(split_patches3x3_x3t_kernel, dim3((unsigned)((waves + 3) / 4)), dim3(256), 0, s, x, cmax,
                       static_cast<unsigned char*>(rec), inv, H, W, Ho, Wo, C, stride, (int)R, rows_padded / 32, 9 * C / 16);
    return check_launch();
}

struct HxPlan { int cfg, mtiles, ntiles, splits, chunks_per_split; };

static HxPlan plan_gemm_x3t(int M, int N, int K, int batches, int tiles_mode = -1)
{
    HxPlan pl;
    const int chunks = K / 16;
    static const int env_force = []() { const char* e = frcnn_knob("FRCNN_HX_CFG"); return e ? atoi(e) : -1; }();
    const int mode = tiles_mode >= 0 ? tiles_mode : gemm_x6t_get_tiles();
    const int force = (env_force >= 0 && tiles_mode < 0) ? env_force : (mode == 1 ? 0 : mode == 2 ? 1 : -1);
    const long long u0 = (long long)cdiv(M, 320) * cdiv(N, 256) * batches;
    const long long u1 = (long long)cdiv(M, 160) * cdiv(N, 128) * batches;
    int splits0 = 1;
    while (u0 * splits0 * 2 <= 256 && chunks / (splits0 * 2) >= 8) splits0 *= 2;
    const double c0 = (double)((u0 * splits0 + 255) / 256) * 1920.0 / splits0 + (splits0 > 1 ? 600.0 : 0.0);
    int splits1 = 1;
    while (u1 * splits1 * 2 <= 256 && chunks / (splits1 * 2) >= 8) splits1 *= 2;
    const double c1 = (double)((u1 * splits1 + 255) / 256) * 480.0 / 0.85 / splits1 + (splits1 > 1 ? 600.0 : 0.0);
    pl.cfg = (force == 0 || force == 1) ? force : (c1 < c0 ? 1 : 0);
    static const bool big_unsplit = frcnn_knob("FRCNN_HX_BIG_UNSPLIT") != nullptr;
    if (big_unsplit && force < 0 && pl.cfg == 1 && splits1 == 1) { pl.cfg = 0; splits0 = 1; }
    int splits = pl.cfg == 1 ? splits1 : splits0;
    if (splits > chunks) splits = chunks;
    pl.mtiles = pl.cfg == 1 ? cdiv(M, 160) : cdiv(M, 320);
    pl.ntiles = pl.cfg == 1 ? cdiv(N, 128) : cdiv(N, 256);
    pl.chunks_per_split = cdiv(chunks, splits);
    pl.splits = cdiv(chunks, pl.chunks_per_split);
    return pl;
}

size_t gemm_x3t_workspace_bytes(int M, int N, int K, int batches)
{
    if (!gemm_x6t_shape_ok(M, N, K, batches)) return 0;
    size_t need = 0;
    for (int mode = 0; mode < 3; ++mode) {
        const HxPlan pl = plan_gemm_x3t(M, N, K, batches, mode);
        const size_t b = pl.splits > 1 ? (size_t)pl.splits * batches * M * N * sizeof(float) : 0;
        if (b > need) need = b;
    }
    return need;
}

int launch_gemm_x3t(const void* a_rec, const float* a_inv, int a_rows, size_t a_batch_bytes, size_t a_inv_batch, const void* b_rec,
                    const float* b_inv, int b_rows, size_t b_batch_bytes, size_t b_inv_batch, const float* bias, const float* residual,
                    float* c, int ldc, size_t c_batch_floats, int M, int N, int K, int batches, unsigned flags, void* ws, size_t ws_bytes,
                    hipStream_t s, int tiles_mode)
{
    if (!gemm_x6t_shape_ok(M, N, K, batches)) return FRCNN_EUNSUPPORTED;
    if (!a_rec || !b_rec || !a_inv || !b_inv || !c || a_rows % 320 != 0 || a_rows < M || b_rows % 256 != 0 || b_rows < N || ldc < N ||
        ldc % 4 != 0)
        return FRCNN_EINVAL;
    const HxPlan pl = plan_gemm_x3t(M, N, K, batches, tiles_mode);
    if (pl.splits > 1 && (ws == nullptr || ws_bytes < (size_t)pl.splits * batches * M * N * sizeof(float))) return FRCNN_EINVAL;
    HxParams p;
    p.a = static_cast<const unsigned char*>(a_rec);
    p.b = static_cast<const unsigned char*>(b_rec);
    p.a_inv = a_inv; p.b_inv = b_inv;
    p.c = c;
    p.ws = static_cast<float*>(ws);
    p.bias = bias;
    p.residual = residual;
    p.a_batch = a_batch_bytes; p.b_batch = b_batch_bytes; p.c_batch = c_batch_floats;
    p.a_inv_batch = a_inv_batch; p.b_inv_batch = b_inv_batch;
    p.a_rbt = a_rows / 32; p.b_rbt = b_rows / 32;
    p.M = M; p.N = N; p.ldc = ldc;
    p.nchunks = K / 16; p.chunks_per_split = pl.chunks_per_split; p.splits = pl.splits; p.batches = batches;
    p.mtiles = pl.mtiles; p.ntiles = pl.ntiles;
    p.relu = (flags & FRCNN_RELU) ? 1 : 0;
    const long long total = (long long)pl.mtiles * pl.ntiles * batches * pl.splits;
    if (total > 0x7fffffffLL) return FRCNN_EINVAL;
    p.total = (int)total;
    static const int env_nsub = []() { const char* e = frcnn_knob("FRCNN_HX_NSUB"); return e ? atoi(e) : 0; }();
    const int last = p.nchunks - (pl.splits - 1) * pl.chunks_per_split;
    const bool even = pl.chunks_per_split % 2 == 0 && last % 2 == 0;
    const int nsub = !even ? 1 : (env_nsub == 1 || env_nsub == 2) ? env_nsub : (pl.chunks_per_split >= 64 ? 2 : 1);
#define HX_LAUNCH(TM, TN, VM, VN, NS)                                                                          \
    do {                                                                                                      \
        using C = HxCfg<TM, TN, VM, VN, NS>;                                                                    \
        auto kern = gemm_x3t_kernel<TM, TN, VM, VN, NS>;                                                        \
        FRCNN_MAX_LDS_ONCE(kern, C::LDS_BYTES);                                                                 \
        hipLaunchKernelGGL(kern, dim3((unsigned)total), dim3(C::THREADS), C::LDS_BYTES, s, p);                  \
    } while (0)
    if (pl.cfg == 1) { if (nsub == 2) HX_LAUNCH(5, 1, 1, 4, 2); else HX_LAUNCH(5, 1, 1, 4, 1); }
    else             { if (nsub == 2) HX_LAUNCH(5, 2, 2, 4, 2); else HX_LAUNCH(5, 2, 2, 4, 1); }
#undef HX_LAUNCH
    int rc = check_launch();
    if (rc || pl.splits == 1) return rc;
    return launch_gemm_x6t_reduce(static_cast<const float*>(ws), bias, residual, c, ldc, c_batch_floats, M, N, batches, pl.splits, p.relu, s);
}

}
```

fasterrcnn_amd/csrc/linear.hip:

```cpp
#include "common.h"
#include <cstdlib>

namespace frcnn {

static constexpr int LLDK = 20;

template <int TM, int TN, int WM, int WN>
struct GemmCfg {
    static constexpr int BM = 32 * TM * WM;
    static constexpr int BN = 32 * TN * WN;
    static constexpr int THREADS = 64 * WM * WN;
    static constexpr int NA = (BM * 4 + THREADS - 1) / THREADS;
    static constexpr int NB = (BN * 4 + THREADS - 1) / THREADS;
    static constexpr int A_F = BM * LLDK;
    static constexpr int B_F = BN * LLDK;
    static constexpr size_t LDS_BYTES = (size_t)2 * (A_F + B_F) * sizeof(float);
    static_assert(THREADS == 256 || THREADS == 512, "4 or 8 waves per block");
};

struct BatchGeom { long long a_stride, w_stride, y_stride; int nblocks, mblocks, batches; };

template <int TM, int TN, int WM, int WN, bool BATCHED, int NSETS = 2>
__global__ __launch_bounds__(64 * WM * WN)
void linear_mfma_kernel(const float* __restrict__ a, int lda, const float* __restrict__ w,
// ... 148 lines not shown
            if (s < nst) stage(s, areg[0], breg[0]);
        } else {
            for (int s = 0; s < nst; ++s) stage(s, areg[0], breg[0]);
        }
    }

    const bool direct = (gridDim.z == 1);
    float* const dst = direct ? y : ws + (size_t)blockIdx.z * M * N;
    const int ldd = direct ? ldy : N;
#pragma unroll
    for (int j = 0; j < TN; ++j) {
        const int n = n0 + 32 * (TN * wn + j) + li;
        if (n >= N) continue;
        const float bv = (direct && bias != nullptr) ? bias[n] : 0.f;
#pragma unroll
        for (int i = 0; i < TM; ++i) {
#pragma unroll
            for (int r = 0; r < 16; ++r) {
                const int m = m0 + 32 * (TM * wm + i) + (r & 3) + 8 * (r >> 2) + 4 * lh;
                if (m < M) {
                    float v = acc[i][j][r] + bv;
                    if (direct && relu) v = fmaxf(v, 0.f);
                    dst[(size_t)m * ldd + n] = v;
                }
            }
        }
    }
}

__global__ __launch_bounds__(256)
void splitk_reduce_kernel(const float* __restrict__ ws, const float* __restrict__ bias,
                          float* __restrict__ y, int ldy, int M, int N, int splits, int relu)
{
    const size_t total = (size_t)M * N;
    for (size_t i = (size_t)blockIdx.x * 256 + threadIdx.x; i < total; i += (size_t)gridDim.x * 256) {
        const int n = (int)(i % N);
        const size_t m = i / N;
        float v = ws[i];
        for (int z = 1; z < splits; ++z) v += ws[(size_t)z * total + i];
        v += bias[n];
        if (relu) v = fmaxf(v, 0.f);
        y[m * ldy + n] = v;
    }
}

__global__ __launch_bounds__(256)
void softmax_rows_kernel(const float* __restrict__ x, int ldx, float* __restrict__ y, int M, int ncls)
{
    const int row = blockIdx.x * 4 + (threadIdx.x >> 6);
    const int lane = threadIdx.x & 63;
    if (row >= M) return;
    const float* xr = x + (size_t)row * ldx;
    const float v0 = lane < ncls ? xr[lane] : -INFINITY, v1 = lane + 64 < ncls ? xr[lane + 64] : -INFINITY;
    float mx = fmaxf(v0, v1);
#pragma unroll
    for (int o = 32; o > 0; o >>= 1) mx = fmaxf(mx, __shfl_xor(mx, o));
    const float e0 = lane < ncls ? expf(v0 - mx) : 0.f, e1 = lane + 64 < ncls ? expf(v1 - mx) : 0.f;
    float sum = e0 + e1;
#pragma unroll
    for (int o = 32; o > 0; o >>= 1) sum += __shfl_xor(sum, o);
    if (lane < ncls) y[(size_t)row * ncls + lane] = e0 / sum;
    if (lane + 64 < ncls) y[(size_t)row * ncls + lane + 64] = e1 / sum;
}

__global__ __launch_bounds__(256)
void head_finish_kernel(const float* __restrict__ x, int ldx, int M, int ncls, int ndelta,
                        float* __restrict__ classes, float* __restrict__ deltas)
{
    const int row = blockIdx.x * 4 + (threadIdx.x >> 6);
    const int lane = threadIdx.x & 63;
    if (row >= M) return;
    const float* xr = x + (size_t)row * ldx;
    const float v0 = lane < ncls ? xr[lane] : -INFINITY, v1 = lane + 64 < ncls ? xr[lane + 64] : -INFINITY;
    float mx = fmaxf(v0, v1);
#pragma unroll
    for (int o = 32; o > 0; o >>= 1) mx = fmaxf(mx, __shfl_xor(mx, o));
    const float e0 = lane < ncls ? expf(v0 - mx) : 0.f, e1 = lane + 64 < ncls ? expf(v1 - mx) : 0.f;
    float sum = e0 + e1;
#pragma unroll
    for (int o = 32; o > 0; o >>= 1) sum += __shfl_xor(sum, o);
    if (lane < ncls) classes[(size_t)row * ncls + lane] = e0 / sum;
    if (lane + 64 < ncls) classes[(size_t)row * ncls + lane + 64] = e1 / sum;
    for (int j = lane; j < ndelta; j += 64) deltas[(size_t)row * ndelta + j] = xr[ncls + j];
}

__global__ void pack_fc_chw_to_hwc_kernel(const float* __restrict__ w, float* __restrict__ wp,
                                          int out_f, int c, int hw)
{
    const size_t K = (size_t)c * hw;
    const size_t total = (size_t)out_f * K;
    for (size_t i = (size_t)blockIdx.x * 256 + threadIdx.x; i < total; i += (size_t)gridDim.x * 256) {
        const size_t o = i / K, kk = i % K;
        const int p = (int)(kk / c), ch = (int)(kk % c);
        wp[i] = w[o * K + (size_t)ch * hw + p];
    }
}

__global__ void pack_stack_rows_kernel(const float* __restrict__ w1, const float* __restrict__ b1, int n1,
                                       const float* __restrict__ w2, const float* __restrict__ b2, int n2,
                                       int k, int n_pad, float* __restrict__ wo, float* __restrict__ bo)
{
    const size_t total = (size_t)n_pad * k;
    for (size_t i = (size_t)blockIdx.x * 256 + threadIdx.x; i < total; i += (size_t)gridDim.x * 256) {
        const int row = (int)(i / k), col = (int)(i % k);
        float v = 0.f;
        if (row < n1) v = w1[(size_t)row * k + col];
        else if (row < n1 + n2) v = w2[(size_t)(row - n1) * k + col];
        wo[i] = v;
        if (col == 0) bo[row] = row < n1 ? b1[row] : (row < n1 + n2 ? b2[row - n1] : 0.f);
    }
}

struct LinearPlan { bool big; int mblocks, nblocks, splits, stages_per_split; };

static LinearPlan plan_linear(int M, int N, int K)
{
    LinearPlan p;
    p.big = (M <= 320) || (M % 320 == 0);
    const int bm = p.big ? 320 : 128;
    p.mblocks = cdiv(M, bm);
    p.nblocks = cdiv(N, 128);
    const int stages = K / 16;
    static int target = -1;
    if (target < 0) { const char* e = frcnn_knob("FRCNN_LINEAR_BLOCKS_TARGET"); target = e ? atoi(e) : 256; if (target < 1) target = 1; }
    int want = target / (p.mblocks * p.nblocks);
    int cap = stages / 8;
    if (cap < 1) cap = 1;
    if (want > cap) want = cap;
    if (want < 1) want = 1;
    p.stages_per_split = cdiv(stages, want);
    p.splits = cdiv(stages, p.stages_per_split);
    return p;
}

size_t linear_workspace_bytes(int M, int N, int K)
{
    if (M < 1 || N < 1 || K < 16) return 0;
    const LinearPlan p = plan_linear(M, N, K);
    return p.splits > 1 ? (size_t)p.splits * M * N * sizeof(float) : 0;
}

template <int TM, int TN, int WM, int WN>
static int launch_linear_cfg(const LinearPlan& p, const float* a, int lda, const float* w,
                             const float* bias, float* y, int ldy, float* ws, int M, int N, int K,
                             int relu, hipStream_t s)
{
    using C = GemmCfg<TM, TN, WM, WN>;
    auto kern = linear_mfma_kernel<TM, TN, WM, WN, false>;
    FRCNN_MAX_LDS_ONCE(kern, C::LDS_BYTES);
    dim3 grid(p.nblocks, p.mblocks, p.splits);
    hipLaunchKernelGGL(kern, grid, dim3(C::THREADS), C::LDS_BYTES, s, a, lda, w, bias, y, ldy, ws, M, N, K,
                       p.stages_per_split, relu, BatchGeom{0, 0, 0, 0, 0, 0});
    return check_launch();
}

template <int TM, int TN, int WM, int WN, int NSETS>
static int launch_linear_batched_cfg(const float* a, int lda, const float* w, float* y, int ldy, int M, int N, int K,
                                     const BatchGeom& bg, hipStream_t s)
{
    using C = GemmCfg<TM, TN, WM, WN>;
    auto kern = linear_mfma_kernel<TM, TN, WM, WN, true, NSETS>;
    FRCNN_MAX_LDS_ONCE(kern, C::LDS_BYTES);
    const long long total = (long long)bg.nblocks * bg.mblocks * bg.batches;
    if (total < 1 || total > 0x7fffffffLL) return FRCNN_EINVAL;
    hipLaunchKernelGGL(kern, dim3((unsigned)total), dim3(C::THREADS), C::LDS_BYTES, s, a, lda, w,
                       (const float*)nullptr, y, ldy, (float*)nullptr, M, N, K, K >> 4, 0, bg);
    return check_launch();
}

static thread_local int g_batched_tile = 0;
void linear_batched_set_tile(int rows) { g_batched_tile = rows; }

int launch_linear_batched(const float* a, int lda, size_t a_stride, const float* w, size_t w_stride, float* y, int ldy,
                          size_t y_stride, int M, int N, int K, int batches, hipStream_t s)
{
    if (M < 1 || N < 1 || K < 16 || K % 16 != 0 || lda % 4 != 0 || lda < K || ldy < N || batches < 1) return FRCNN_EINVAL;
    static int env_tile = -1;
    if (env_tile < 0) { const char* e = frcnn_knob("FRCNN_WINO_TILE"); env_tile = e ? atoi(e) : 0; }
    const int tile = env_tile ? env_tile : (g_batched_tile ? g_batched_tile : 64);
    BatchGeom bg{(long long)a_stride, (long long)w_stride, (long long)y_stride, cdiv(N, 128), cdiv(M, 128), batches};
    if (tile == 128) return launch_linear_batched_cfg<2, 2, 2, 2, 1>(a, lda, w, y, ldy, M, N, K, bg, s);
    bg.mblocks = cdiv(M, 64);
    return launch_linear_batched_cfg<1, 2, 2, 2, 1>(a, lda, w, y, ldy, M, N, K, bg, s);
}

int launch_linear(const float* a, int lda, const float* w, const float* bias, float* y, int ldy,
                  int M, int N, int K, unsigned flags, void* ws, size_t ws_bytes, hipStream_t s)
{
    if (M < 1 || N < 1 || K < 16 || K % 16 != 0 || lda % 4 != 0 || lda < K || ldy < N) return FRCNN_EINVAL;
    const LinearPlan p = plan_linear(M, N, K);
    const size_t need = p.splits > 1 ? (size_t)p.splits * M * N * sizeof(float) : 0;
    if (need > ws_bytes || (need > 0 && ws == nullptr)) return FRCNN_EINVAL;
    const int relu = (flags & FRCNN_RELU) ? 1 : 0;
    int rc = p.big ? launch_linear_cfg<5, 1, 2, 4>(p, a, lda, w, bias, y, ldy, (float*)ws, M, N, K, relu, s)
                   : launch_linear_cfg<2, 2, 2, 2>(p, a, lda, w, bias, y, ldy, (float*)ws, M, N, K, relu, s);
    if (rc != FRCNN_OK) return rc;
    if (p.splits > 1) {
        const size_t total = (size_t)M * N;
        int blocks = (int)((total + 255) / 256);
        if (blocks > 2048) blocks = 2048;
        hipLaunchKernelGGL(splitk_reduce_kernel, dim3(blocks), dim3(256), 0, s, (const float*)ws, bias,
                           y, ldy, M, N, p.splits, relu);
        rc = check_launch();
    }
    return rc;
}

int launch_softmax_rows(const float* x, int ldx, float* y, int M, int ncls, hipStream_t s)
{
    if (M < 1 || ncls < 1 || ncls > 128 || ldx < ncls) return FRCNN_EINVAL;
    hipLaunchKernelGGL(softmax_rows_kernel, dim3(cdiv(M, 4)), dim3(256), 0, s, x, ldx, y, M, ncls);
    return check_launch();
}

int launch_head_finish(const float* x, int ldx, int M, int ncls, int ndelta, float* classes,
                       float* deltas, hipStream_t s)
{
    if (M < 1 || ncls < 1 || ncls > 128 || ndelta < 0 || ldx < ncls + ndelta) return FRCNN_EINVAL;
    hipLaunchKernelGGL(head_finish_kernel, dim3(cdiv(M, 4)), dim3(256), 0, s, x, ldx, M, ncls, ndelta,
                       classes, deltas);
    return check_launch();
}

int launch_pack_fc_chw_to_hwc(const float* w, float* wp, int out_f, int c, int phw, hipStream_t s)
{
    if (out_f < 1 || c < 1 || phw < 1) return FRCNN_EINVAL;
    hipLaunchKernelGGL(pack_fc_chw_to_hwc_kernel, dim3(8192), dim3(256), 0, s, w, wp, out_f, c, phw);
    return check_launch();
}

int launch_pack_stack_rows(const float* w1, const float* b1, int n1, const float* w2, const float* b2,
                           int n2, int k, int n_pad, float* wo, float* bo, hipStream_t s)
{
    if (n1 < 0 || n2 < 0 || n1 + n2 > n_pad || k < 1) return FRCNN_EINVAL;
    const size_t total = (size_t)n_pad * k;
    int blocks = (int)((total + 255) / 256);
    if (blocks > 2048) blocks = 2048;
    hipLaunchKernelGGL(pack_stack_rows_kernel, dim3(blocks), dim3(256), 0, s, w1, b1, n1, w2, b2, n2, k,
                       n_pad, wo, bo);
    return check_launch();
}

}
```

fasterrcnn_amd/csrc/proposals.hip:

```cpp
#include "geometry.h"
#include <type_traits>

namespace frcnn {

typedef unsigned long long u64;

__device__ __forceinline__ unsigned ordered_bits(float f)
{
    const unsigned b = __float_as_uint(f);
    return (b & 0x80000000u) ? ~b : (b | 0x80000000u);
}
__device__ __forceinline__ float from_ordered_bits(unsigned o)
{
    const unsigned b = (o & 0x80000000u) ? (o & 0x7fffffffu) : ~o;
    return __uint_as_float(b);
}

__global__ __launch_bounds__(256)
void rpn_decode_kernel(const float* __restrict__ head, int ld, const float* __restrict__ anchors,
                       const float* __restrict__ valid, int A, float* __restrict__ scores,
                       f32x4* __restrict__ boxes_all, u64* __restrict__ keys)
{
    const int n = blockIdx.x * 256 + threadIdx.x;
    if (n >= A) return;
    const int pix = n / 9, k = n - pix * 9;
    const float* row = head + (size_t)pix * ld;
    const float logit = row[k];
    const float score = 1.0f / (1.0f + expf(-logit));
    const float dy = row[9 + 4 * k + 0], dx = row[9 + 4 * k + 1];
    const float dh = row[9 + 4 * k + 2], dw = row[9 + 4 * k + 3];
    const f32x4 a = reinterpret_cast<const f32x4*>(anchors)[n];
    const float cy = __fadd_rn(__fmul_rn(a[2], dy), a[0]);
    const float cx = __fadd_rn(__fmul_rn(a[3], dx), a[1]);
    const float h = __fmul_rn(a[2], expf(dh));
    const float w = __fmul_rn(a[3], expf(dw));
    const float hh = 0.5f * h, hw = 0.5f * w;
    f32x4 b;
    b[0] = cy - hh; b[1] = cx - hw; b[2] = cy + hh; b[3] = cx + hw;
    scores[n] = score;
    boxes_all[n] = b;
    const bool ok = (valid == nullptr) || (valid[n] > 0.f);
    keys[n] = ok ? (((u64)ordered_bits(score) << 32) | (u64)(unsigned)(n + 1)) : 0ull;
}

__global__ __launch_bounds__(256)
void nms_keys_kernel(const float* __restrict__ scores, int n, u64* __restrict__ keys)
{
    const int i = blockIdx.x * 256 + threadIdx.x;
    if (i >= n) return;
    const float f = scores[i];
    const unsigned hi = f != f ? 0u : ordered_bits(f == 0.f ? 0.f : f);
    keys[i] = ((u64)hi << 32) | (u64)(0xFFFFFFFFu - (unsigned)i);
}

__device__ __forceinline__ u64 shfl_xor_u64(u64 v, int lane_mask)
{
    const unsigned lo = __shfl_xor((unsigned)(v & 0xFFFFFFFFull), lane_mask);
    const unsigned hi = __shfl_xor((unsigned)(v >> 32), lane_mask);
    return ((u64)hi << 32) | lo;
}

__device__ __forceinline__ u64 bitonic_pick(u64 mine, u64 other, int g, int j, int k)
{
    const bool keep_max = (((g & k) == 0) == ((g & j) == 0));
    const bool other_bigger = other > mine;
    return (keep_max == other_bigger) ? other : mine;
}

template <int PER, int J>
__device__ __forceinline__ void bitonic_inthread(u64 (&e)[PER], int base, int k)
{
#pragma unroll
    for (int r = 0; r < PER; ++r) {
        if ((r & J) == 0) {
            const u64 a = e[r], b = e[r | J];
            e[r] = bitonic_pick(a, b, base + r, J, k);
            e[r | J] = bitonic_pick(b, a, base + (r | J), J, k);
        }
    }
}

template <int PER>
__device__ void bitonic_sort_regs(u64* buf, int tid)
{
    constexpr int N = 1024 * PER;
    u64 e[PER];
    const int base = tid * PER;
#pragma unroll
    for (int r = 0; r < PER; ++r) e[r] = buf[base + r];
    for (int k = 2; k <= N; k <<= 1) {
        for (int j = k >> 1; j > 0; j >>= 1) {
            if (j >= 64 * PER) {
#pragma unroll
                for (int r = 0; r < PER; ++r) buf[base + r] = e[r];
                __syncthreads();
#pragma unroll
                for (int r = 0; r < PER; ++r) e[r] = bitonic_pick(e[r], buf[(base + r) ^ j], base + r, j, k);
                __syncthreads();
            } else if (j >= PER) {
                const int lane_mask = j / PER;
#pragma unroll
                for (int r = 0; r < PER; ++r) e[r] = bitonic_pick(e[r], shfl_xor_u64(e[r], lane_mask), base + r, j, k);
            } else {
                if (PER > 8 && j == 8) bitonic_inthread<PER, (PER > 8 ? 8 : 1)>(e, base, k);
                else if (PER > 4 && j == 4) bitonic_inthread<PER, (PER > 4 ? 4 : 1)>(e, base, k);
                else if (PER > 2 && j == 2) bitonic_inthread<PER, (PER > 2 ? 2 : 1)>(e, base, k);
                else if (PER > 1 && j == 1) bitonic_inthread<PER, 1>(e, base, k);
            }
        }
    }
#pragma unroll
    for (int r = 0; r < PER; ++r) buf[base + r] = e[r];
    __syncthreads();
}

template <int MODE, bool SPLIT = false>
__global__ __launch_bounds__(1024)
void topk_sort_kernel(const u64* __restrict__ keys, int n_keys, int K, int sort_n,
                      const f32x4* __restrict__ boxes_src, float image_h, float image_w, float min_side,
                      int32_t* __restrict__ sorted_idx, f32x4* __restrict__ cand_boxes,
                      float* __restrict__ cand_scores, int32_t* __restrict__ counts, u64* __restrict__ sel_out = nullptr)
{
    extern __shared__ __attribute__((aligned(16))) unsigned char smem_raw[];
    u64* buf = reinterpret_cast<u64*>(smem_raw);
    int* hist = reinterpret_cast<int*>(buf + sort_n);
// ... 603 lines not shown
    if (lane == 0) *n_keep_out = kept;
#ifdef NMS_CLOCKS
    if (lane == 0 && props && max_keep >= 4) {
        const unsigned long long t_out = __builtin_amdgcn_s_memrealtime();
        props[max_keep - 1] = f32x4{nms_acc[1], nms_acc[2], nms_acc[3], nms_acc[4]};
        props[max_keep - 2] = f32x4{nms_acc[5], nms_acc[6], (float)(t_out - nms_t_in), (float)c_done};
        props[max_keep - 3] = f32x4{nms_acc[0], nms_acc[7], (float)n, (float)kept};
    }
#endif
}
#undef NMS_T

static size_t align_up(size_t v, size_t a) { return (v + a - 1) / a * a; }

size_t proposal_scratch_bytes(int a_cap, int pre_cap, int post_cap)
{
    size_t b = 0;
    b += align_up((size_t)a_cap * 8, 256);
    b += align_up((size_t)a_cap * 16, 256);
    b += align_up((size_t)pre_cap * 16, 256);
    b += align_up((size_t)pre_cap * 4, 256);
    b += align_up((size_t)pre_cap * (pre_cap / 64) * 8 + 256, 256);
    b += align_up((size_t)post_cap * 4, 256);
    return b;
}

void proposal_scratch_carve(ProposalScratch& ps, void* base, int a_cap, int pre_cap, int post_cap)
{
    unsigned char* p = static_cast<unsigned char*>(base);
    ps.keys = reinterpret_cast<u64*>(p);         p += align_up((size_t)a_cap * 8, 256);
    ps.boxes_all = reinterpret_cast<float*>(p);  p += align_up((size_t)a_cap * 16, 256);
    ps.cand_boxes = reinterpret_cast<float*>(p); p += align_up((size_t)pre_cap * 16, 256);
    ps.cand_scores = reinterpret_cast<float*>(p); p += align_up((size_t)pre_cap * 4, 256);
    ps.mask = reinterpret_cast<u64*>(p);         p += align_up((size_t)pre_cap * (pre_cap / 64) * 8 + 256, 256);
    ps.keep = reinterpret_cast<int32_t*>(p);
    ps.a_cap = a_cap; ps.pre_cap = pre_cap; ps.post_cap = post_cap;
}

static int pow2_at_least(int v) { int p = 1024; while (p < v) p <<= 1; return p; }

template <int MODE>
static int launch_topk(const u64* keys, int n_keys, int K, const float* boxes_src, float ih, float iw,
                       float min_side, int32_t* sorted_idx, float* cand_boxes, float* cand_scores,
                       int32_t* counts, hipStream_t s, void* tmp = nullptr)
{
    const int sort_n = pow2_at_least(K);
    if (sort_n > 16384) return FRCNN_EUNSUPPORTED;
    const size_t lds = (size_t)sort_n * 8 + 4096 * 4 + 64 * 4;
    static const bool no_split = frcnn_knob("FRCNN_TOPK_ONE_BLOCK") != nullptr;
    if (MODE == 0 && tmp != nullptr && !no_split) {
        unsigned char* tb = static_cast<unsigned char*>(tmp);
        u64* sel = reinterpret_cast<u64*>(tb);
        f32x4* tboxes = reinterpret_cast<f32x4*>(tb + (size_t)sort_n * 8);
        float* tscores = reinterpret_cast<float*>(tb + (size_t)sort_n * 24);
        int32_t* flags = reinterpret_cast<int32_t*>(tb + (size_t)sort_n * 28);
        auto k1 = topk_sort_kernel<0, true>;
        FRCNN_MAX_LDS_ONCE(k1, 16384 * 8 + 4096 * 4 + 64 * 4);
        hipLaunchKernelGGL(k1, dim3(1), dim3(1024), lds, s, keys, n_keys, K, sort_n, reinterpret_cast<const f32x4*>(boxes_src), ih, iw,
                           min_side, sorted_idx, reinterpret_cast<f32x4*>(cand_boxes), cand_scores, counts, sel);
        int rc = check_launch();
        if (rc) return rc;
        const size_t lds2 = (size_t)sort_n * 8 + 32 * 32 * 4;
        FRCNN_MAX_LDS_ONCE(topk_rank_kernel, 16384 * 8 + 32 * 32 * 4);
        hipLaunchKernelGGL(topk_rank_kernel, dim3(cdiv(K, 32)), dim3(1024), lds2, s, sel, counts, sort_n,
                           reinterpret_cast<const f32x4*>(boxes_src), ih, iw, min_side, sorted_idx, tboxes, tscores, flags);
        rc = check_launch();
        if (rc) return rc;
        hipLaunchKernelGGL(topk_emit_kernel, dim3(1), dim3(1024), 0, s, tboxes, tscores, flags, sort_n, reinterpret_cast<f32x4*>(cand_boxes),
                           cand_scores, counts);
        return check_launch();
    }
    auto kern = topk_sort_kernel<MODE>;
    FRCNN_MAX_LDS_ONCE(kern, 16384 * 8 + 4096 * 4 + 64 * 4);
    hipLaunchKernelGGL(kern, dim3(1), dim3(1024), lds, s, keys, n_keys, K, sort_n,
                       reinterpret_cast<const f32x4*>(boxes_src), ih, iw, min_side, sorted_idx,
                       reinterpret_cast<f32x4*>(cand_boxes), cand_scores, counts, (u64*)nullptr);
    return check_launch();
}

int launch_rpn_proposals(const ProposalScratch& ps, const float* head, int ld_head,
                         const float* anchor_map, const float* valid_map, int fh, int fw,
                         int image_h, int image_w, int pre_nms, int post_nms, float nms_thr,
                         float min_side, float* scores, int32_t* sorted_idx, float* props,
                         int32_t* counts, hipStream_t s)
{
    const int A = fh * fw * 9;
    if (A < 1 || A > ps.a_cap || pre_nms < 1 || pre_nms > ps.pre_cap || post_nms < 1 ||
        post_nms > ps.post_cap || post_nms > 2048 || ld_head < 45)
        return FRCNN_EINVAL;
    hipLaunchKernelGGL(rpn_decode_kernel, dim3(cdiv(A, 256)), dim3(256), 0, s, head, ld_head, anchor_map,
                       valid_map, A, scores, reinterpret_cast<f32x4*>(ps.boxes_all), ps.keys);
    int rc = check_launch();
    if (rc) return rc;
    rc = launch_topk<0>(ps.keys, A, pre_nms, ps.boxes_all, (float)image_h, (float)image_w, min_side,
                        sorted_idx, ps.cand_boxes, ps.cand_scores, counts, s, ps.mask);
    if (rc) return rc;
    const int nw = cdiv(pre_nms, 64);
    const int nw_stride = ps.pre_cap / 64;
    hipLaunchKernelGGL(nms_mask_kernel, dim3(nw, nw), dim3(64), 0, s,
                       reinterpret_cast<const f32x4*>(ps.cand_boxes), counts + 1, nms_thr, nw_stride, ps.mask);
    rc = check_launch();
    if (rc) return rc;
    FRCNN_MAX_LDS_ONCE(nms_reduce_kernel, NMS_LDS_BYTES);
    hipLaunchKernelGGL(nms_reduce_kernel, dim3(1), dim3(64), NMS_LDS_BYTES, s, ps.mask, nw_stride, counts + 1, post_nms,
                       reinterpret_cast<const f32x4*>(ps.cand_boxes), (const int32_t*)nullptr,
                       (int32_t*)nullptr, reinterpret_cast<f32x4*>(props), counts + 2);
    return check_launch();
}

int launch_nms(const ProposalScratch& ps, const float* boxes, const float* scores, int n, float thr,
               int max_keep, int32_t* keep, int32_t* n_keep, hipStream_t s)
{
    if (n < 0 || n > ps.pre_cap || n > ps.a_cap || max_keep < 1 || max_keep > 2048) return FRCNN_EINVAL;
    if (n == 0) {
        FRCNN_HIP_TRY(hipMemsetAsync(n_keep, 0, sizeof(int32_t), s));
        return FRCNN_OK;
    }
    hipLaunchKernelGGL(nms_keys_kernel, dim3(cdiv(n, 256)), dim3(256), 0, s, scores, n, ps.keys);
    int rc = check_launch();
    if (rc) return rc;
    int32_t* order = reinterpret_cast<int32_t*>(ps.boxes_all);
    int32_t* counts = order + ps.a_cap;
    rc = launch_topk<1>(ps.keys, n, n, boxes, 0.f, 0.f, 0.f, order, ps.cand_boxes, ps.cand_scores, counts, s);
    if (rc) return rc;
    const int nw = cdiv(n, 64);
    const int nw_stride = ps.pre_cap / 64;
    hipLaunchKernelGGL(nms_mask_kernel, dim3(nw, nw), dim3(64), 0, s,
                       reinterpret_cast<const f32x4*>(ps.cand_boxes), counts + 1, thr, nw_stride, ps.mask);
    rc = check_launch();
    if (rc) return rc;
    FRCNN_MAX_LDS_ONCE(nms_reduce_kernel, NMS_LDS_BYTES);
    hipLaunchKernelGGL(nms_reduce_kernel, dim3(1), dim3(64), NMS_LDS_BYTES, s, ps.mask, nw_stride, counts + 1, max_keep,
                       reinterpret_cast<const f32x4*>(ps.cand_boxes), order, keep, (f32x4*)nullptr, n_keep);
    return check_launch();
}

}
```

fasterrcnn_amd/csrc/roipool.hip:

```cpp
#include "x3t.h"
#include <cfloat>
#include <cmath>

namespace frcnn {

__global__ __launch_bounds__(128)
void roi_pool_kernel(const float* __restrict__ fm, int fh, int fw, int C,
                     const float* __restrict__ rois, const int32_t* __restrict__ n_rois,
                     int pooled, float scale, float* __restrict__ out)
{
    const int r = blockIdx.x, ph = blockIdx.y, pw = blockIdx.z;
    const int C4 = C >> 2;
    f32x4* obin = reinterpret_cast<f32x4*>(out + (((size_t)(r * pooled + ph) * pooled) + pw) * C);
    if (r >= *n_rois) {
        for (int i = threadIdx.x; i < C4; i += 128) obin[i] = f32x4{0.f, 0.f, 0.f, 0.f};
        return;
    }
    const f32x4 roi = reinterpret_cast<const f32x4*>(rois)[r];
    const int rs_h = (int)roundf(roi[0] * scale), rs_w = (int)roundf(roi[1] * scale);
    const int re_h = (int)roundf(roi[2] * scale), re_w = (int)roundf(roi[3] * scale);
    const int roi_h = max(re_h - rs_h + 1, 1), roi_w = max(re_w - rs_w + 1, 1);
    const float bin_h = (float)roi_h / (float)pooled, bin_w = (float)roi_w / (float)pooled;
    int hs = (int)floorf((float)ph * bin_h) + rs_h;
    int he = (int)ceilf((float)(ph + 1) * bin_h) + rs_h;
// ... 18 lines not shown
            if (two && ++cw == we) { cw = ws; ++ch; }
            f32x4 a0 = lowest, a1 = lowest, b0 = lowest, b1 = lowest;
            if (has_a) { a0 = p0[c4a]; a1 = p1[c4a]; }
            if (has_b) { b0 = p0[c4b]; b1 = p1[c4b]; }
#pragma unroll
            for (int j = 0; j < 4; ++j) {
                const float a = a0[j] > a1[j] ? a0[j] : a1[j], b = b0[j] > b1[j] ? b0[j] : b1[j];
                ma[j] = a > ma[j] ? a : ma[j]; mb[j] = b > mb[j] ? b : mb[j];
            }
        }
        if (empty) { ma = f32x4{0.f, 0.f, 0.f, 0.f}; mb = ma; }
        if (has_a) obin[c40 + c4a] = ma;
        if (has_b) obin[c40 + c4b] = mb;
    }
}

__device__ __forceinline__ unsigned short rp_bf16_rne(float f)
{
    unsigned u = __float_as_uint(f);
    u += 0x7FFFu + ((u >> 16) & 1u);
    return (unsigned short)(u >> 16);
}
__device__ __forceinline__ float rp_bf16_f32(unsigned short h) { return __uint_as_float((unsigned)h << 16); }

__global__ __launch_bounds__(256)
void roi_pool_x6t_kernel(const float* __restrict__ fm, int fh, int fw, int C, const float* __restrict__ rois,
                         const int32_t* __restrict__ n_rois, int max_rois, int pooled, float scale, unsigned char* __restrict__ rec, int rbt)
{
    const int lane = threadIdx.x & 63;
    const int K16c = C >> 4;
    const long long wave = (long long)blockIdx.x * 4 + (threadIdx.x >> 6);
    const long long total = (long long)pooled * pooled * rbt * K16c;
    if (wave >= total) return;
    const int cc = (int)(wave % K16c);
    long long t = wave / K16c;
    const int rb = (int)(t % rbt);
    const int bin = (int)(t / rbt);
    const int ph = bin / pooled, pw = bin - ph * pooled;
    const int r = rb * 32 + (lane & 31);
    const int c0 = cc * 16 + 8 * (lane >> 5);
    float m[8] = {0.f, 0.f, 0.f, 0.f, 0.f, 0.f, 0.f, 0.f};
    int n = *n_rois;
    if (n > max_rois) n = max_rois;
    if (r < n) {
        const f32x4 roi = reinterpret_cast<const f32x4*>(rois)[r];
        const int rs_h = (int)roundf(roi[0] * scale), rs_w = (int)roundf(roi[1] * scale);
        const int re_h = (int)roundf(roi[2] * scale), re_w = (int)roundf(roi[3] * scale);
        const int roi_h = max(re_h - rs_h + 1, 1), roi_w = max(re_w - rs_w + 1, 1);
        const float bin_h = (float)roi_h / (float)pooled, bin_w = (float)roi_w / (float)pooled;
        int hs = (int)floorf((float)ph * bin_h) + rs_h;
        int he = (int)ceilf((float)(ph + 1) * bin_h) + rs_h;
        hs = min(max(hs, 0), fh); he = min(max(he, 0), fh);
        int ws = (int)floorf((float)pw * bin_w) + rs_w;
        int we = (int)ceilf((float)(pw + 1) * bin_w) + rs_w;
        ws = min(max(ws, 0), fw); we = min(max(we, 0), fw);
        if (he > hs && we > ws) {
#pragma unroll
            for (int e = 0; e < 8; ++e) m[e] = -FLT_MAX;
            for (int h = hs; h < he; ++h) {
                const float* p = fm + ((size_t)h * fw + ws) * C + c0;
                for (int w = ws; w < we; ++w, p += C) {
                    const f32x4 v0 = *reinterpret_cast<const f32x4*>(p), v1 = *reinterpret_cast<const f32x4*>(p + 4);
#pragma unroll
                    for (int e = 0; e < 4; ++e) { m[e] = v0[e] > m[e] ? v0[e] : m[e]; m[4 + e] = v1[e] > m[4 + e] ? v1[e] : m[4 + e]; }
                }
            }
        }
    }
    unsigned hi[8], mid[8], lo[8];
#pragma unroll
    for (int e = 0; e < 8; ++e) {
        hi[e] = rp_bf16_rne(m[e]);
        const float r1 = m[e] - rp_bf16_f32((unsigned short)hi[e]);
        mid[e] = rp_bf16_rne(r1);
        lo[e] = rp_bf16_rne(r1 - rp_bf16_f32((unsigned short)mid[e]));
    }
    const int chunk = bin * K16c + cc;
    unsigned char* dst = rec + ((size_t)chunk * rbt + rb) * 3072 + lane * 16;
    *reinterpret_cast<uint4*>(dst) = make_uint4(hi[0] | (hi[1] << 16), hi[2] | (hi[3] << 16), hi[4] | (hi[5] << 16), hi[6] | (hi[7] << 16));
    *reinterpret_cast<uint4*>(dst + 1024) = make_uint4(mid[0] | (mid[1] << 16), mid[2] | (mid[3] << 16), mid[4] | (mid[5] << 16), mid[6] | (mid[7] << 16));
    *reinterpret_cast<uint4*>(dst + 2048) = make_uint4(lo[0] | (lo[1] << 16), lo[2] | (lo[3] << 16), lo[4] | (lo[5] << 16), lo[6] | (lo[7] << 16));
}

__global__ __launch_bounds__(256)
void roi_scale_x3t_kernel(const float* __restrict__ cmax, int fh, int fw, const float* __restrict__ rois, const int32_t* __restrict__ n_rois,
                          int max_rois, int rec_rows, int pooled, float scale, float* __restrict__ inv)
{
    const int lane = threadIdx.x & 63;
    const int r = blockIdx.x * 4 + (threadIdx.x >> 6);
    if (r >= rec_rows) return;
    int n = *n_rois;
    if (n > max_rois) n = max_rois;
    float mx = 0.f;
    if (r < n) {
        const f32x4 roi = reinterpret_cast<const f32x4*>(rois)[r];
        const int rs_h = (int)roundf(roi[0] * scale), rs_w = (int)roundf(roi[1] * scale);
        const int re_h = (int)roundf(roi[2] * scale), re_w = (int)roundf(roi[3] * scale);
        const int roi_h = max(re_h - rs_h + 1, 1), roi_w = max(re_w - rs_w + 1, 1);
        const float bin_h = (float)roi_h / (float)pooled, bin_w = (float)roi_w / (float)pooled;
        const int hs = min(max(rs_h, 0), fh), he = min(max((int)ceilf((float)pooled * bin_h) + rs_h, 0), fh);
        const int ws = min(max(rs_w, 0), fw), we = min(max((int)ceilf((float)pooled * bin_w) + rs_w, 0), fw);
        const int ww = we - ws, cells = (he - hs) * ww;
        for (int i = lane; i < cells; i += 64) {
            const int h = hs + i / ww, w = ws + i % ww;
            mx = fmaxf(mx, cmax[(size_t)h * fw + w]);
        }
    }
#pragma unroll
    for (int off = 32; off >= 1; off >>= 1) mx = fmaxf(mx, __shfl_xor(mx, off));
    float mult, iv;
    hx_row_scale(mx, mult, iv);
    if (lane == 0) inv[r] = iv;
}

__global__ __launch_bounds__(256)
void roi_pool_x3t_kernel(const float* __restrict__ fm, int fh, int fw, int C, const float* __restrict__ rois,
                         const int32_t* __restrict__ n_rois, int max_rois, int pooled, float scale, const float* __restrict__ inv,
                         unsigned char* __restrict__ rec, int rbt)
{
    const int lane = threadIdx.x & 63;
    const int K16c = C >> 4;
    const long long wave = (long long)blockIdx.x * 4 + (threadIdx.x >> 6);
    const long long total = (long long)pooled * pooled * rbt * K16c;
    if (wave >= total) return;
    const int cc = (int)(wave % K16c);
    long long t = wave / K16c;
    const int rb = (int)(t % rbt);
    const int bin = (int)(t / rbt);
    const int ph = bin / pooled, pw = bin - ph * pooled;
    const int r = rb * 32 + (lane & 31);
    const int c0 = cc * 16 + 8 * (lane >> 5);
    float m[8] = {0.f, 0.f, 0.f, 0.f, 0.f, 0.f, 0.f, 0.f};
    int n = *n_rois;
    if (n > max_rois) n = max_rois;
    if (r < n) {
        const f32x4 roi = reinterpret_cast<const f32x4*>(rois)[r];
        const int rs_h = (int)roundf(roi[0] * scale), rs_w = (int)roundf(roi[1] * scale);
        const int re_h = (int)roundf(roi[2] * scale), re_w = (int)roundf(roi[3] * scale);
        const int roi_h = max(re_h - rs_h + 1, 1), roi_w = max(re_w - rs_w + 1, 1);
        const float bin_h = (float)roi_h / (float)pooled, bin_w = (float)roi_w / (float)pooled;
        int hs = (int)floorf((float)ph * bin_h) + rs_h;
        int he = (int)ceilf((float)(ph + 1) * bin_h) + rs_h;
        hs = min(max(hs, 0), fh); he = min(max(he, 0), fh);
        int ws = (int)floorf((float)pw * bin_w) + rs_w;
        int we = (int)ceilf((float)(pw + 1) * bin_w) + rs_w;
        ws = min(max(ws, 0), fw); we = min(max(we, 0), fw);
        if (he > hs && we > ws) {
#pragma unroll
            for (int e = 0; e < 8; ++e) m[e] = -FLT_MAX;
            for (int h = hs; h < he; ++h) {
                const float* p = fm + ((size_t)h * fw + ws) * C + c0;
                for (int w = ws; w < we; ++w, p += C) {
                    const f32x4 v0 = *reinterpret_cast<const f32x4*>(p), v1 = *reinterpret_cast<const f32x4*>(p + 4);
#pragma unroll
                    for (int e = 0; e < 4; ++e) { m[e] = v0[e] > m[e] ? v0[e] : m[e]; m[4 + e] = v1[e] > m[4 + e] ? v1[e] : m[4 + e]; }
                }
            }
        }
        const float mult = hx_mult_of_inv(inv[r]);
#pragma unroll
        for (int e = 0; e < 8; ++e) m[e] *= mult;
    }
    uint4 phh, pll;
    hx_split8(m, phh, pll);
    const int chunk = bin * K16c + cc;
    unsigned char* dst = rec + ((size_t)chunk * rbt + rb) * HX_RB + lane * 16;
    *reinterpret_cast<uint4*>(dst) = phh;
    *reinterpret_cast<uint4*>(dst + HX_PIECE) = pll;
}

#ifndef FRCNN_ROI_ROWS_WAVES
#define FRCNN_ROI_ROWS_WAVES 8
#endif
template <int NW>
__global__ __launch_bounds__(64 * NW)
void roi_pool_x3t_rows_kernel(const float* __restrict__ fm, int fh, int fw, int C, const float* __restrict__ rois,
                              const int32_t* __restrict__ n_rois, int max_rois, int pooled, float scale, const float* __restrict__ inv,
                              unsigned char* __restrict__ rec, int rbt)
{
    extern __shared__ __attribute__((aligned(16))) float rp_pool[];
    const int tid = threadIdx.x, lane = tid & 63, wave = tid >> 6;
    const int bin = blockIdx.x / rbt, rb = blockIdx.x - bin * rbt;
    const int ph = bin / pooled, pw = bin - ph * pooled;
    const int LD = C + 4;
    int n = *n_rois;
    if (n > max_rois) n = max_rois;
    for (int q = 0; q < 32 / NW; ++q) {
        const int rl = wave * (32 / NW) + q, r = rb * 32 + rl;
        int hs = 0, he = 0, ws = 0, we = 0;
        float mult = 0.f;
        if (r < n) {
            const f32x4 roi = reinterpret_cast<const f32x4*>(rois)[r];
            const int rs_h = (int)roundf(roi[0] * scale), rs_w = (int)roundf(roi[1] * scale);
            const int re_h = (int)roundf(roi[2] * scale), re_w = (int)roundf(roi[3] * scale);
            const int roi_h = max(re_h - rs_h + 1, 1), roi_w = max(re_w - rs_w + 1, 1);
            const float bin_h = (float)roi_h / (float)pooled, bin_w = (float)roi_w / (float)pooled;
            hs = (int)floorf((float)ph * bin_h) + rs_h;
            he = (int)ceilf((float)(ph + 1) * bin_h) + rs_h;
            hs = min(max(hs, 0), fh); he = min(max(he, 0), fh);
            ws = (int)floorf((float)pw * bin_w) + rs_w;
            we = (int)ceilf((float)(pw + 1) * bin_w) + rs_w;
            ws = min(max(ws, 0), fw); we = min(max(we, 0), fw);
            mult = hx_mult_of_inv(inv[r]);
        }
        const bool any = r < n && he > hs && we > ws;
        for (int c0 = 8 * lane; c0 < C; c0 += 512) {
            float m[8] = {0.f, 0.f, 0.f, 0.f, 0.f, 0.f, 0.f, 0.f};
            if (any) {
#pragma unroll
                for (int e = 0; e < 8; ++e) m[e] = -FLT_MAX;
                const int ww = we - ws, ncell = (he - hs) * ww;
                const float rww = __builtin_amdgcn_rcpf((float)ww);
                constexpr int UN = 4;
                for (int i0 = 0; i0 < ncell; i0 += UN) {
                    f32x4 v[UN][2];
#pragma unroll
                    for (int u = 0; u < UN; ++u) {
                        const int i = min(i0 + u, ncell - 1);
                        int dh = (int)((float)i * rww);
                        int dw = i - dh * ww;
                        if (dw < 0) { --dh; dw += ww; } else if (dw >= ww) { ++dh; dw -= ww; }
                        const float* p = fm + ((size_t)(hs + dh) * fw + ws + dw) * C + c0;
                        v[u][0] = *reinterpret_cast<const f32x4*>(p); v[u][1] = *reinterpret_cast<const f32x4*>(p + 4);
                    }
#pragma unroll
                    for (int u = 0; u < UN; ++u)
#pragma unroll
                        for (int e = 0; e < 4; ++e) {
                            asm("v_max_f32 %0, %1, %2" : "=v"(m[e]) : "v"(v[u][0][e]), "v"(m[e]));
                            asm("v_max_f32 %0, %1, %2" : "=v"(m[4 + e]) : "v"(v[u][1][e]), "v"(m[4 + e]));
                        }
                }
            }
            if (r < n) {
#pragma unroll
                for (int e = 0; e < 8; ++e) m[e] *= mult;
            }
            float* d = rp_pool + rl * LD + c0;
            *reinterpret_cast<f32x4*>(d) = f32x4{m[0], m[1], m[2], m[3]};
            *reinterpret_cast<f32x4*>(d + 4) = f32x4{m[4], m[5], m[6], m[7]};
        }
    }
    __syncthreads();
    const int K16c = C >> 4;
    for (int cc = wave; cc < K16c; cc += NW) {
        const float* sp = rp_pool + (lane & 31) * LD + cc * 16 + 8 * (lane >> 5);
        const f32x4 a = *reinterpret_cast<const f32x4*>(sp), b = *reinterpret_cast<const f32x4*>(sp + 4);
        const float m[8] = {a[0], a[1], a[2], a[3], b[0], b[1], b[2], b[3]};
        uint4 phh, pll;
        hx_split8(m, phh, pll);
        const int chunk = bin * K16c + cc;
        unsigned char* dst = rec + ((size_t)chunk * rbt + rb) * HX_RB + lane * 16;
        *reinterpret_cast<uint4*>(dst) = phh;
        *reinterpret_cast<uint4*>(dst + HX_PIECE) = pll;
    }
}

template <int P>
__global__ __launch_bounds__(256)
void roi_pool_x3t_bands_kernel(const float* __restrict__ fm, int fh, int fw, int C, const float* __restrict__ rois,
                               const int32_t* __restrict__ n_rois, int max_rois, float scale, const float* __restrict__ inv,
                               unsigned char* __restrict__ rec, int rbt)
{
    const int lane = threadIdx.x & 63;
    const int wid = __builtin_amdgcn_readfirstlane((int)blockIdx.x * 4 + (int)(threadIdx.x >> 6));
    if (wid >= rbt * 32 * P) return;
    const int ph = wid % P, r = wid / P;
    int n = *n_rois;
    if (n > max_rois) n = max_rois;
    int hs = 0, he = 0, ws[P], we[P], wlo = 0, whi = 0;
    float mult = 0.f;
#pragma unroll
    for (int q = 0; q < P; ++q) { ws[q] = 0; we[q] = 0; }
    if (r < n) {
        const f32x4 roi = reinterpret_cast<const f32x4*>(rois)[r];
        const int rs_h = (int)roundf(roi[0] * scale), rs_w = (int)roundf(roi[1] * scale);
        const int re_h = (int)roundf(roi[2] * scale), re_w = (int)roundf(roi[3] * scale);
        const int roi_h = max(re_h - rs_h + 1, 1), roi_w = max(re_w - rs_w + 1, 1);
        const float bin_h = (float)roi_h / (float)P, bin_w = (float)roi_w / (float)P;
        hs = (int)floorf((float)ph * bin_h) + rs_h;
        he = (int)ceilf((float)(ph + 1) * bin_h) + rs_h;
        hs = min(max(hs, 0), fh); he = min(max(he, 0), fh);
        wlo = fw; whi = 0;
#pragma unroll
        for (int q = 0; q < P; ++q) {
            int a = (int)floorf((float)q * bin_w) + rs_w;
// ... 26 lines not shown
                    v[u][0] = *reinterpret_cast<const f32x4*>(p); v[u][1] = *reinterpret_cast<const f32x4*>(p + 4);
                }
#pragma unroll
                for (int u = 0; u < 4; ++u) {
                    const int w = min(w0 + u, whi - 1);
#pragma unroll
                    for (int q = 0; q < P; ++q) {
                        if (w >= ws[q] && w < we[q]) {
#pragma unroll
                            for (int e = 0; e < 4; ++e) {
                                acc[q][e] = v[u][0][e] > acc[q][e] ? v[u][0][e] : acc[q][e];
                                acc[q][4 + e] = v[u][1][e] > acc[q][4 + e] ? v[u][1][e] : acc[q][4 + e];
                            }
                        }
                    }
                }
            }
        }
        const int cc = c0 >> 4, kh = (c0 >> 3) & 1;
#pragma unroll
        for (int q = 0; q < P; ++q) {
            float m[8];
#pragma unroll
            for (int e = 0; e < 8; ++e) m[e] = r < n ? acc[q][e] * mult : 0.f;
            uint4 phh, pll;
            hx_split8(m, phh, pll);
            const int chunk = (ph * P + q) * K16c + cc;
            unsigned char* dst = rec + ((size_t)chunk * rbt + rb) * HX_RB + kh * 512 + row * 16;
            *reinterpret_cast<uint4*>(dst) = phh;
            *reinterpret_cast<uint4*>(dst + HX_PIECE) = pll;
        }
    }
}

struct AnchorSizes { double h[9]; double w[9]; };

__global__ __launch_bounds__(256)
void anchors_kernel(AnchorSizes sz, int image_h, int image_w, int fh, int fw, int feature_pixels,
                    float* __restrict__ anchor_map, float* __restrict__ valid_map)
{
    const int n = blockIdx.x * 256 + threadIdx.x;
    const int A = fh * fw * 9;
    if (n >= A) return;
    const int cell = n / 9, k = n - cell * 9;
    const int cy_i = cell / fw, cx_i = cell - cy_i * fw;
    const float cyf = (float)((double)(cy_i * feature_pixels) + 0.5 * (double)feature_pixels);
    const float cxf = (float)((double)(cx_i * feature_pixels) + 0.5 * (double)feature_pixels);
    const double y1 = (double)cyf + (-0.5 * sz.h[k]);
    const double x1 = (double)cxf + (-0.5 * sz.w[k]);
    const double y2 = (double)cyf + (0.5 * sz.h[k]);
    const double x2 = (double)cxf + (0.5 * sz.w[k]);
    const bool valid = (y1 >= 0.0) && (x1 >= 0.0) && (y2 <= (double)image_h) && (x2 <= (double)image_w);
    f32x4 a;
    a[0] = (float)(0.5 * (y1 + y2));
    a[1] = (float)(0.5 * (x1 + x2));
    a[2] = (float)(y2 - y1);
    a[3] = (float)(x2 - x1);
    reinterpret_cast<f32x4*>(anchor_map)[n] = a;
    valid_map[n] = valid ? 1.0f : 0.0f;
}

int launch_roi_pool(const float* fm, int fh, int fw, int c, const float* rois, const int32_t* n_rois,
                    int max_rois, int pooled, float scale, float* out, hipStream_t s)
{
    if (fh < 1 || fw < 1 || c < 4 || c % 4 != 0 || max_rois < 1 || pooled < 1) return FRCNN_EINVAL;
    hipLaunchKernelGGL(roi_pool_kernel, dim3(max_rois, pooled, pooled), dim3(128), 0, s, fm, fh, fw, c, rois,
                       n_rois, pooled, scale, out);
    return check_launch();
}

int launch_roi_pool_x6t(const float* fm, int fh, int fw, int c, const float* rois, const int32_t* n_rois,
                        int max_rois, int pooled, float scale, void* rec, int rec_rows, hipStream_t s)
{
    if (fh < 1 || fw < 1 || c < 16 || c % 16 != 0 || max_rois < 1 || pooled < 1 || rec_rows < max_rois || rec_rows % 32 != 0) return FRCNN_EINVAL;
    const int rbt = rec_rows / 32, rb_live = cdiv(max_rois, 32);
    (void)rb_live;
    const long long waves = (long long)pooled * pooled * rbt * (c / 16);
    hipLaunchKernelGGL(roi_pool_x6t_kernel, dim3((unsigned)((waves + 3) / 4)), dim3(256), 0, s, fm, fh, fw, c, rois, n_rois, max_rois,
                       pooled, scale, static_cast<unsigned char*>(rec), rbt);
    return check_launch();
}

int launch_roi_pool_x3t(const float* fm, int fh, int fw, int c, const float* rois, const int32_t* n_rois, int max_rois, int pooled,
                        float scale, float* cmax, float* inv, void* rec, int rec_rows, hipStream_t s, bool cmax_ready)
{
    if (fh < 1 || fw < 1 || c < 16 || c % 16 != 0 || max_rois < 1 || pooled < 1 || rec_rows < max_rois || rec_rows % 32 != 0 || !cmax || !inv)
        return FRCNN_EINVAL;
    int rc = cmax_ready ? FRCNN_OK : launch_pixel_absmax(fm, cmax, (long long)fh * fw, c, s);
    if (rc) return rc;
    hipLaunchKernelGGL(roi_scale_x3t_kernel, dim3(cdiv(rec_rows, 4)), dim3(256), 0, s, cmax, fh, fw, rois, n_rois, max_rois, rec_rows, pooled, scale, inv);
    if ((rc = check_launch()) != FRCNN_OK) return rc;
    const int rbt = rec_rows / 32;
#ifdef FRCNN_ROI_BANDS
    if (pooled == 7 && c % 8 == 0) {
        const long long waves = (long long)rec_rows * pooled;
        hipLaunchKernelGGL(roi_pool_x3t_bands_kernel<7>, dim3((unsigned)((waves + 3) / 4)), dim3(256), 0, s, fm, fh, fw, c, rois, n_rois, max_rois, scale,
                           inv, static_cast<unsigned char*>(rec), rbt);
        return check_launch();
    }
#endif
    const size_t lds = (size_t)32 * (c + 4) * sizeof(float);
    if (c % 8 == 0 && lds <= 160 * 1024) {
        constexpr int NW = FRCNN_ROI_ROWS_WAVES;
        auto kern = roi_pool_x3t_rows_kernel<NW>;
        FRCNN_MAX_LDS_ONCE(kern, 160 * 1024);
        hipLaunchKernelGGL(kern, dim3((unsigned)(pooled * pooled * rbt)), dim3(64 * NW), lds, s, fm, fh, fw, c, rois, n_rois, max_rois, pooled, scale,
                           inv, static_cast<unsigned char*>(rec), rbt);
        return check_launch();
    }
    const long long waves = (long long)pooled * pooled * rbt * (c / 16);
    hipLaunchKernelGGL(roi_pool_x3t_kernel, dim3((unsigned)((waves + 3) / 4)), dim3(256), 0, s, fm, fh, fw, c, rois, n_rois, max_rois,
                       pooled, scale, inv, static_cast<unsigned char*>(rec), rbt);
    return check_launch();
}

int launch_anchors(int image_h, int image_w, int fh, int fw, int feature_pixels,
                   float* anchor_map, float* valid_map, hipStream_t s)
{
    if (fh < 1 || fw < 1 || feature_pixels < 1) return FRCNN_EINVAL;
    static const double areas[3] = {128.0 * 128.0, 256.0 * 256.0, 512.0 * 512.0};
    static const double aspects[3] = {0.5, 1.0, 2.0};
    AnchorSizes sz;
    for (int i = 0; i < 3; ++i)
        for (int j = 0; j < 3; ++j) {
            const double root = std::sqrt(areas[i] / aspects[j]);
            sz.h[i * 3 + j] = aspects[j] * root;
            sz.w[i * 3 + j] = root;
        }
    const int A = fh * fw * 9;
    hipLaunchKernelGGL(anchors_kernel, dim3(cdiv(A, 256)), dim3(256), 0, s, sz, image_h, image_w, fh, fw,
                       feature_pixels, anchor_map, valid_map);
    return check_launch();
}

}
```

Measured before the change: 850.6.

## Fuse small post-backbone kernels to cut launches across RPN, ROI and FC stages

Several independent kernel-fusion changes are made. The cmax memset is folded into the first conv kernel. The RPN head GEMM is fused into the proposal decode kernel when the split plan is small. The ROI scale computation is folded into the ROI pooling kernel. The fc1 split-K reduction is merged with the row scaling and splitting. The class head GEMM is combined with the softmax/finish step. The aim is to cut launch overhead and intermediate memory round-trips in the small post-backbone stages, at the cost of redundant per-bin window max work and more complex kernels.

```diff
diff --git a/fasterrcnn_amd/csrc/api.hip b/fasterrcnn_amd/csrc/api.hip
--- a/fasterrcnn_amd/csrc/api.hip
+++ b/fasterrcnn_amd/csrc/api.hip
@@ -541,6 +541,7 @@
 {
     if (!ctx || !d_head || !d_anchor_map || !d_scores || !d_sorted_idx || !d_props || !d_counts) return FRCNN_EINVAL;
     FRCNN_HIP_TRY(hipMemsetAsync(d_counts, 0, 4 * sizeof(int32_t), as_stream(stream)));
+    ctx->last_fh = fh; ctx->last_fw = fw;
     return launch_rpn_proposals(ctx->ps, d_head, ld_head, d_anchor_map, d_valid_map, fh, fw, image_h, image_w,
                                 pre_nms, post_nms, nms_threshold, min_side, d_scores, d_sorted_idx, d_props,
                                 d_counts, as_stream(stream));
@@ -1078,8 +1079,17 @@
         case 6: *d_ptr = c->anchor_map; *bytes = fmsz * 9 * 16; break;
         case 7: *d_ptr = c->valid_map; *bytes = fmsz * 9 * 4; break;
         case 8: *d_ptr = c->head_logits; *bytes = (size_t)c->last_post * c->last_head_ld * 4; break;
+        case 9: *d_ptr = c->rpn_trunk; *bytes = fmsz * c->last_c * 4; break;
+        case 10: *d_ptr = c->ps.keys; *bytes = fmsz * 9 * 8; break;
+        case 11: *d_ptr = c->ps.boxes_all; *bytes = fmsz * 9 * 16; break;
+        case 12: *d_ptr = c->fc1_out; *bytes = (size_t)c->last_post * c->last_vec * 4; break;
+        case 13: *d_ptr = c->fc1_inv; *bytes = (size_t)c->rec_rows * 4; break;
+        case 14: *d_ptr = c->fc1_rec; *bytes = x3t_record_bytes(c->rec_rows, 4096); break;
+        case 15: *d_ptr = c->roi_inv; *bytes = (size_t)c->rec_rows * 4; break;
+        case 16: *d_ptr = c->roi_rec; *bytes = x3t_record_bytes(c->rec_rows, 49 * 512); break;
         default: return FRCNN_EINVAL;
     }
+    if (*d_ptr == nullptr) return FRCNN_EINVAL;
     return FRCNN_OK;
 }
 
@@ -1262,7 +1272,7 @@
     if (p->winograd_x3f_mask != 0 && (!wino || (p->winograd_x3f_mask & ~0x3FFE) != 0 || (p->winograd_x3f_mask & p->winograd_x6_mask) != 0)) return FRCNN_EINVAL;
     int layer_index = 0;
     const float* cmax_ready = nullptr;
-    size_t cmax_used = 0, cmax_cleared = 0;
+    size_t cmax_used = 0, cmax_cleared = 0, cmax_zero = 0;
     if (wino && ((p->winograd_x3f_mask | (p->winograd_x3_mask & p->winograd_x6_mask)) & 0x1FFE) != 0) {
         int r0 = ensure_x3f_cmax(c, (size_t)H * W * sizeof(float), s);
         if (r0) return r0;
@@ -1279,7 +1289,11 @@
         }
         if (want > 2 * c->x3f_cmax_bytes / sizeof(float)) return FRCNN_EINVAL;
         cmax_cleared = want;
-        if (want) FRCNN_HIP_TRY(hipMemsetAsync(x3f_cmax_buffer(c, 1), 0, cmax_cleared * sizeof(float), s));
+        if (want && (reinterpret_cast<uintptr_t>(x3f_cmax_buffer(c, 1)) & 15) != 0) {
+            FRCNN_HIP_TRY(hipMemsetAsync(x3f_cmax_buffer(c, 1), 0, cmax_cleared * sizeof(float), s));
+            want = 0;
+        }
+        cmax_zero = want;
     }
     auto conv3 = [&](const float* xin, const float* wgt, const float* bs, float* yout, int hh, int ww, int ci, int co,
                      unsigned fl) -> int {
@@ -1321,7 +1335,8 @@
     float *A = c->act_a, *B = c->act_b;
     int h = H, wd = W;
     float* c11_cmax = (wino && ((p->winograd_x3f_mask >> 1) & 1)) ? x3f_cmax_buffer(c, 0) : nullptr;
-    STEP(1, launch_conv3x3_c3(d_image, w->conv_w[0], w->conv_b[0], A, h, wd, 64, R, s, c11_cmax));
+    STEP(1, launch_conv3x3_c3(d_image, w->conv_w[0], w->conv_b[0], A, h, wd, 64, R, s, c11_cmax,
+                              cmax_zero ? x3f_cmax_buffer(c, 1) : nullptr, cmax_zero));
     cmax_ready = c11_cmax;
     CONV(conv3(A, w->conv_w[1], w->conv_b[1], B, h, wd, 64, 64, RP));   h /= 2; wd /= 2;
     CONV(conv3(B, w->conv_w[2], w->conv_b[2], A, h, wd, 64, 128, R));
@@ -1340,8 +1355,11 @@
     c->last_fh = fh; c->last_fw = fw; c->last_pre = p->pre_nms; c->last_post = p->post_nms; c->last_c = 512; c->last_vec = 4096;
 
     CONV(conv3(c->fm, w->rpn_conv_w, w->rpn_conv_b, c->rpn_trunk, fh, fw, 512, 512, R));
-    STEP(2, launch_linear(c->rpn_trunk, 512, w->rpn_head_w, w->rpn_head_b, c->rpn_head, 128, fh * fw, 45, 512,
-                          0u, c->lin_ws, c->lin_ws_bytes, s));
+    const bool fuse_heads = linear_plan_splits(fh * fw, 45, 512, nullptr) <= 4;
+    if (!fuse_heads) {
+        STEP(2, launch_linear(c->rpn_trunk, 512, w->rpn_head_w, w->rpn_head_b, c->rpn_head, 128, fh * fw, 45, 512,
+                              0u, c->lin_ws, c->lin_ws_bytes, s));
+    }
     const float* amap = d_anchor_map;
     const float* vmap = d_valid_map;
     if (!amap || !vmap) {
@@ -1351,10 +1369,11 @@
         }
         amap = c->anchor_map; vmap = c->valid_map;
     }
-    FRCNN_HIP_TRY(hipMemsetAsync(d_counts, 0, 4 * sizeof(int32_t), s));
+    const RpnHeadsGemm heads{c->rpn_trunk, 512, w->rpn_head_w, w->rpn_head_b, 512};
+    if (!fuse_heads) FRCNN_HIP_TRY(hipMemsetAsync(d_counts, 0, 4 * sizeof(int32_t), s));
     STEP(3, launch_rpn_proposals(c->ps, c->rpn_head, 128, amap, p->allow_edge_proposals ? nullptr : vmap, fh, fw,
                                  H, W, p->pre_nms, p->post_nms, p->rpn_nms_threshold, p->min_side, c->scores,
-                                 c->sorted_idx, d_props, d_counts, s));
+                                 c->sorted_idx, d_props, d_counts, s, fuse_heads ? &heads : nullptr));
 
     const int R_ = p->post_nms;
     const bool fc_x6t = p->fc_math_mode == FRCNN_FC_F32X6T;
@@ -1371,12 +1390,18 @@
             STEP(2, launch_split_rows_x3t(c->roi_out, 49 * 512, 0, c->roi_inv, c->roi_rec, R_, rr, 49 * 512, 1, s));
         } else {
             STEP(4, launch_roi_pool_x3t(c->fm, fh, fw, 512, d_props, d_counts + 2, R_, 7, 1.0f / 16.0f,
-                                        fm_cmax_ready ? const_cast<float*>(fm_cmax_ready) : c->fm_cmax, c->roi_inv, c->roi_rec, rr, s, fm_cmax_ready != nullptr));
+                                        fm_cmax_ready ? const_cast<float*>(fm_cmax_ready) : c->fm_cmax, c->roi_inv, c->roi_rec, rr, s, fm_cmax_ready != nullptr, true));
         }
+        int fc1_splits = 1;
         STEP(2, launch_gemm_x3t(c->roi_rec, c->roi_inv, rr, 0, 0, w->fc1_w, w1inv, 4096, 0, 0, w->fc1_b, nullptr, c->fc1_out, 4096, 0, R_, 4096,
-                                49 * 512, 1, R, c->lin_ws, c->lin_ws_bytes, s, 0));
-        STEP(2, launch_rows_scale_x3t(c->fc1_out, 4096, 0, c->fc1_inv, R_, rr, 4096, 1, s));
-        STEP(2, launch_split_rows_x3t(c->fc1_out, 4096, 0, c->fc1_inv, c->fc1_rec, R_, rr, 4096, 1, s));
+                                49 * 512, 1, R, c->lin_ws, c->lin_ws_bytes, s, 0, &fc1_splits));
+        if (fc1_splits > 1) {
+            STEP(2, launch_reduce_scale_split_x3t(static_cast<const float*>(c->lin_ws), w->fc1_b, c->fc1_out, 4096, c->fc1_inv, c->fc1_rec, R_, rr,
+                                                  4096, fc1_splits, R, s));
+        } else {
+            STEP(2, launch_rows_scale_x3t(c->fc1_out, 4096, 0, c->fc1_inv, R_, rr, 4096, 1, s));
+            STEP(2, launch_split_rows_x3t(c->fc1_out, 4096, 0, c->fc1_inv, c->fc1_rec, R_, rr, 4096, 1, s));
+        }
         STEP(2, launch_gemm_x3t(c->fc1_rec, c->fc1_inv, rr, 0, 0, w->fc2_w, w2inv, 4096, 0, 0, w->fc2_b, nullptr, c->fc2_out, 4096, 0, R_, 4096,
                                 4096, 1, R, c->lin_ws, c->lin_ws_bytes, s, 2));
     } else
@@ -1409,9 +1434,8 @@
     const int ncls = w->num_classes, nd = (ncls - 1) * 4;
     const int hld = cdiv(ncls + nd, 128) * 128;
     c->last_head_ld = hld;
-    STEP(2, launch_linear(c->fc2_out, 4096, w->head_w, w->head_b, c->head_logits, hld, R_, ncls + nd, 4096, 0u,
-                          c->lin_ws, c->lin_ws_bytes, s));
-    STEP(5, launch_head_finish(c->head_logits, hld, R_, ncls, nd, d_classes, d_deltas, s));
+    STEP(2, launch_linear_head(c->fc2_out, 4096, w->head_w, w->head_b, c->head_logits, hld, R_, ncls, nd, 4096, d_classes, d_deltas,
+                               c->lin_ws, c->lin_ws_bytes, s));
 #undef STEP
 #undef CONV
     return FRCNN_OK;
diff --git a/fasterrcnn_amd/csrc/common.h b/fasterrcnn_amd/csrc/common.h
--- a/fasterrcnn_amd/csrc/common.h
+++ b/fasterrcnn_amd/csrc/common.h
@@ -74,7 +74,8 @@
                            int n2, int k, int n_pad, float* wo, float* bo, hipStream_t s);
 
 int launch_conv3x3_c3(const float* x, const float* wp, const float* b, float* y, int H, int W,
-                      int cout, unsigned flags, hipStream_t s, float* cmax_out = nullptr);
+                      int cout, unsigned flags, hipStream_t s, float* cmax_out = nullptr, float* zero_out = nullptr,
+                      size_t zero_floats = 0);
 size_t conv3x3_workspace_bytes(int H, int W, int cin, int cout);
 int conv3x3_blocks_target();
 void conv3x3_set_blocks_target(int target);
@@ -102,6 +103,7 @@
 size_t linear_workspace_bytes(int M, int N, int K);
 int launch_linear(const float* a, int lda, const float* w, const float* bias, float* y, int ldy,
                   int M, int N, int K, unsigned flags, void* ws, size_t ws_bytes, hipStream_t s);
+int linear_plan_splits(int M, int N, int K, int* stages_per_split);
 int launch_linear_batched(const float* a, int lda, size_t a_stride, const float* w, size_t w_stride, float* y, int ldy,
                           size_t y_stride, int M, int N, int K, int batches, hipStream_t s);
 void linear_batched_set_tile(int rows);
@@ -153,7 +155,9 @@
 int launch_gemm_x3t(const void* a_rec, const float* a_inv, int a_rows, size_t a_batch_bytes, size_t a_inv_batch, const void* b_rec,
                     const float* b_inv, int b_rows, size_t b_batch_bytes, size_t b_inv_batch, const float* bias, const float* residual,
                     float* c, int ldc, size_t c_batch_floats, int M, int N, int K, int batches, unsigned flags, void* ws, size_t ws_bytes,
-                    hipStream_t s, int tiles_mode = -1);
+                    hipStream_t s, int tiles_mode = -1, int* pending_splits = nullptr);
+int launch_reduce_scale_split_x3t(const float* ws, const float* bias, float* c, int ldc, float* inv_scale, void* rec, int R, int rows_padded,
+                                  int N, int splits, unsigned flags, hipStream_t s);
 size_t x3t_blob_bytes(int rows_padded, int K, int batches);
 int launch_pack_rows_x3t(const float* a, int lda, size_t a_batch_floats, void* blob, int R, int rows_padded, int K, int batches, hipStream_t s);
 int launch_pixel_absmax(const float* x, float* cmax, long long pixels, int C, hipStream_t s);
@@ -174,7 +178,8 @@
                                      unsigned flags, void* ws, size_t ws_bytes, hipStream_t s, const float* cmax_ready = nullptr,
                                      float* cmax_out = nullptr);
 int launch_roi_pool_x3t(const float* fm, int fh, int fw, int c, const float* rois, const int32_t* n_rois, int max_rois, int pooled,
-                        float scale, float* cmax, float* inv, void* rec, int rec_rows, hipStream_t s, bool cmax_ready = false);
+                        float scale, float* cmax, float* inv, void* rec, int rec_rows, hipStream_t s, bool cmax_ready = false,
+                        bool fuse_scale = false);
 bool conv3x3_uses_winograd_x6(int cin, int cout);
 size_t conv3x3_winograd_x6_pack_bytes(int cout, int cin);
 size_t conv3x3_winograd_x6_workspace_bytes(int N, int H, int W, int cin, int cout);
@@ -188,6 +193,8 @@
 int launch_softmax_rows(const float* x, int ldx, float* y, int M, int ncls, hipStream_t s);
 int launch_head_finish(const float* x, int ldx, int M, int ncls, int ndelta, float* classes,
                        float* deltas, hipStream_t s);
+int launch_linear_head(const float* a, int lda, const float* w, const float* bias, float* logits, int ldy, int M, int ncls, int ndelta,
+                       int K, float* classes, float* deltas, void* ws, size_t ws_bytes, hipStream_t s);
 
 struct ProposalScratch {
     unsigned long long* keys;
@@ -201,11 +208,12 @@
 size_t proposal_scratch_bytes(int a_cap, int pre_cap, int post_cap);
 void   proposal_scratch_carve(ProposalScratch& ps, void* base, int a_cap, int pre_cap, int post_cap);
 
+struct RpnHeadsGemm { const float* a; int lda; const float* w; const float* bias; int K; };
 int launch_rpn_proposals(const ProposalScratch& ps, const float* head, int ld_head,
                          const float* anchor_map, const float* valid_map, int fh, int fw,
                          int image_h, int image_w, int pre_nms, int post_nms, float nms_thr,
                          float min_side, float* scores, int32_t* sorted_idx, float* props,
-                         int32_t* counts, hipStream_t s);
+                         int32_t* counts, hipStream_t s, const RpnHeadsGemm* fused_heads = nullptr);
 int launch_nms(const ProposalScratch& ps, const float* boxes, const float* scores, int n, float thr,
                int max_keep, int32_t* keep, int32_t* n_keep, hipStream_t s);
 
diff --git a/fasterrcnn_amd/csrc/conv.hip b/fasterrcnn_amd/csrc/conv.hip
--- a/fasterrcnn_amd/csrc/conv.hip
+++ b/fasterrcnn_amd/csrc/conv.hip
@@ -331,8 +331,10 @@
 template <bool RELU, bool CMAX, int BPC>
 __global__ __launch_bounds__(256, BPC)
 void conv3x3_c3_p_kernel(const float* __restrict__ x, const float* __restrict__ wp, const float* __restrict__ bias,
-                         float* __restrict__ y, int H, int W, float* __restrict__ cmax_out, int tiles_x, int ntiles)
-{
+                         float* __restrict__ y, int H, int W, float* __restrict__ cmax_out, int tiles_x, int ntiles,
+                         f32x4* __restrict__ zero_out, int zero_n4)
+{
+    for (int i = blockIdx.x * 256 + threadIdx.x; i < zero_n4; i += gridDim.x * 256) zero_out[i] = f32x4{0.f, 0.f, 0.f, 0.f};
     constexpr int COUT = 64, SEG = 64, ROWS = 2, LW = 68;
     constexpr int NEL = 3 * (ROWS + 2) * (SEG + 2);
     __shared__ __attribute__((aligned(16))) float in_s[2][3][ROWS + 2][LW];
@@ -582,9 +584,12 @@
 }
 
 int launch_conv3x3_c3(const float* x, const float* wp, const float* b, float* y, int H, int W,
-                      int cout, unsigned flags, hipStream_t s, float* cmax_out)
+                      int cout, unsigned flags, hipStream_t s, float* cmax_out, float* zero_out, size_t zero_floats)
 {
     if (cout % 16 != 0 || H < 1 || W < 1) return FRCNN_EINVAL;
+    if (zero_floats != 0 && (cout != 64 || !zero_out || zero_floats % 4 != 0 || zero_floats > 0x7fffffffu)) return FRCNN_EINVAL;
+    f32x4* const z4 = reinterpret_cast<f32x4*>(zero_out);
+    const int zn4 = (int)(zero_floats / 4);
     if (cmax_out && cout != 64) return FRCNN_EINVAL;
     if (cout == 64) {
         const int tiles_x = cdiv(W, 64), tiles_y = cdiv(H, 2);
@@ -594,8 +599,8 @@
         static const int bpc = []() { const char* e = frcnn_knob("FRCNN_C3_BPC"); return e && atoi(e) == 3 ? 3 : 2; }();
         const int grid = ntiles < bpc * cus ? ntiles : bpc * cus;
         const bool relu = (flags & FRCNN_RELU) != 0;
-#define C3P_LAUNCH(R_, C_) do { if (bpc == 3) hipLaunchKernelGGL((conv3x3_c3_p_kernel<R_, C_, 3>), dim3(grid), dim3(256), 0, s, x, wp, b, y, H, W, cmax_out, tiles_x, ntiles); \
-                                else hipLaunchKernelGGL((conv3x3_c3_p_kernel<R_, C_, 2>), dim3(grid), dim3(256), 0, s, x, wp, b, y, H, W, cmax_out, tiles_x, ntiles); } while (0)
+#define C3P_LAUNCH(R_, C_) do { if (bpc == 3) hipLaunchKernelGGL((conv3x3_c3_p_kernel<R_, C_, 3>), dim3(grid), dim3(256), 0, s, x, wp, b, y, H, W, cmax_out, tiles_x, ntiles, z4, zn4); \
+                                else hipLaunchKernelGGL((conv3x3_c3_p_kernel<R_, C_, 2>), dim3(grid), dim3(256), 0, s, x, wp, b, y, H, W, cmax_out, tiles_x, ntiles, z4, zn4); } while (0)
         if (relu) { if (cmax_out) C3P_LAUNCH(true, true); else C3P_LAUNCH(true, false); }
         else { if (cmax_out) C3P_LAUNCH(false, true); else C3P_LAUNCH(false, false); }
 #undef C3P_LAUNCH
diff --git a/fasterrcnn_amd/csrc/gemm_x3t.hip b/fasterrcnn_amd/csrc/gemm_x3t.hip
--- a/fasterrcnn_amd/csrc/gemm_x3t.hip
+++ b/fasterrcnn_amd/csrc/gemm_x3t.hip
@@ -56,6 +56,63 @@
     unsigned char* dst = rec + (size_t)wave * HX_RB + lane * 16;
     *reinterpret_cast<uint4*>(dst) = ph;
     *reinterpret_cast<uint4*>(dst + HX_PIECE) = pl;
+}
+
+__global__ __launch_bounds__(512)
+void reduce_scale_split_x3t_kernel(const float* __restrict__ ws, const float* __restrict__ bias, float* __restrict__ c, int ldc,
+                                   float* __restrict__ inv_scale, unsigned char* __restrict__ rec, int R, int rbt, int N, int splits, int relu)
+{
+    __shared__ float smax[8];
+    const int tid = threadIdx.x, lane = tid & 63, wave = tid >> 6;
+    const int row = blockIdx.x;
+    const size_t plane = (size_t)R * N;
+    float* const crow = c + (size_t)row * ldc;
+    float mx = 0.f;
+    if (row < R) {
+        for (int k = 8 * tid; k < N; k += 8 * 512) {
+            const size_t off = (size_t)row * N + k;
+            f32x4 v0 = *reinterpret_cast<const f32x4*>(ws + off), v1 = *reinterpret_cast<const f32x4*>(ws + off + 4);
+#pragma unroll 8
+            for (int z = 1; z < splits; ++z) {
+                v0 = v0 + *reinterpret_cast<const f32x4*>(ws + (size_t)z * plane + off);
+                v1 = v1 + *reinterpret_cast<const f32x4*>(ws + (size_t)z * plane + off + 4);
+            }
+            if (bias != nullptr) { v0 = v0 + *reinterpret_cast<const f32x4*>(bias + k); v1 = v1 + *reinterpret_cast<const f32x4*>(bias + k + 4); }
+            if (relu) {
+#pragma unroll
+                for (int j = 0; j < 4; ++j) { v0[j] = fmaxf(v0[j], 0.f); v1[j] = fmaxf(v1[j], 0.f); }
+            }
+            *reinterpret_cast<f32x4*>(crow + k) = v0;
+            *reinterpret_cast<f32x4*>(crow + k + 4) = v1;
+            mx = fmaxf(fmaxf(mx, fmaxf(fabsf(v0[0]), fabsf(v0[1]))), fmaxf(fabsf(v0[2]), fabsf(v0[3])));
+            mx = fmaxf(fmaxf(mx, fmaxf(fabsf(v1[0]), fabsf(v1[1]))), fmaxf(fabsf(v1[2]), fabsf(v1[3])));
+        }
+    }
+#pragma unroll
+    for (int off = 32; off >= 1; off >>= 1) mx = fmaxf(mx, __shfl_xor(mx, off));
+    if (lane == 0) smax[wave] = mx;
+    __syncthreads();
+    mx = smax[0];
+#pragma unroll
+    for (int i = 1; i < 8; ++i) mx = fmaxf(mx, smax[i]);
+    float mult, inv;
+    hx_row_scale(mx, mult, inv);
+    if (tid == 0) inv_scale[row] = inv;
+    mult = hx_mult_of_inv(inv);
+    const int rb = row >> 5, slot = (row & 31) * 16;
+    for (int k = 8 * tid; k < N; k += 8 * 512) {
+        float v[8] = {0.f, 0.f, 0.f, 0.f, 0.f, 0.f, 0.f, 0.f};
+        if (row < R) {
+            const f32x4 v0 = *reinterpret_cast<const f32x4*>(crow + k), v1 = *reinterpret_cast<const f32x4*>(crow + k + 4);
+#pragma unroll
+            for (int j = 0; j < 4; ++j) { v[j] = v0[j] * mult; v[4 + j] = v1[j] * mult; }
+        }
+        uint4 ph, pl;
+        hx_split8(v, ph, pl);
+        unsigned char* dst = rec + ((size_t)(k >> 4) * rbt + rb) * HX_RB + ((k >> 3) & 1) * 512 + slot;
+        *reinterpret_cast<uint4*>(dst) = ph;
+        *reinterpret_cast<uint4*>(dst + HX_PIECE) = pl;
+    }
 }
 
 __global__ __launch_bounds__(256)
@@ -514,8 +571,9 @@
 int launch_gemm_x3t(const void* a_rec, const float* a_inv, int a_rows, size_t a_batch_bytes, size_t a_inv_batch, const void* b_rec,
                     const float* b_inv, int b_rows, size_t b_batch_bytes, size_t b_inv_batch, const float* bias, const float* residual,
                     float* c, int ldc, size_t c_batch_floats, int M, int N, int K, int batches, unsigned flags, void* ws, size_t ws_bytes,
-                    hipStream_t s, int tiles_mode)
-{
+                    hipStream_t s, int tiles_mode, int* pending_splits)
+{
+    if (pending_splits) *pending_splits = 1;
     if (!gemm_x6t_shape_ok(M, N, K, batches)) return FRCNN_EUNSUPPORTED;
     if (!a_rec || !b_rec || !a_inv || !b_inv || !c || a_rows % 320 != 0 || a_rows < M || b_rows % 256 != 0 || b_rows < N || ldc < N ||
         ldc % 4 != 0)
@@ -556,7 +614,19 @@
 #undef HX_LAUNCH
     int rc = check_launch();
     if (rc || pl.splits == 1) return rc;
+    if (pending_splits) { *pending_splits = pl.splits; return FRCNN_OK; }
     return launch_gemm_x6t_reduce(static_cast<const float*>(ws), bias, residual, c, ldc, c_batch_floats, M, N, batches, pl.splits, p.relu, s);
 }
 
-}
+int launch_reduce_scale_split_x3t(const float* ws, const float* bias, float* c, int ldc, float* inv_scale, void* rec, int R, int rows_padded,
+                                  int N, int splits, unsigned flags, hipStream_t s)
+{
+    if (!ws || !c || !inv_scale || !rec || R < 1 || rows_padded < R || rows_padded % 32 != 0 || N < 16 || N % 16 != 0 || ldc < N ||
+        ldc % 4 != 0 || splits < 2)
+        return FRCNN_EINVAL;
+    hipLaunchKernelGGL(reduce_scale_split_x3t_kernel, dim3((unsigned)rows_padded), dim3(512), 0, s, ws, bias, c, ldc, inv_scale,
+                       static_cast<unsigned char*>(rec), R, rows_padded / 32, N, splits, (flags & FRCNN_RELU) ? 1 : 0);
+    return check_launch();
+}
+
+}
diff --git a/fasterrcnn_amd/csrc/linear.hip b/fasterrcnn_amd/csrc/linear.hip
--- a/fasterrcnn_amd/csrc/linear.hip
+++ b/fasterrcnn_amd/csrc/linear.hip
@@ -254,6 +254,46 @@
     if (lane < ncls) classes[(size_t)row * ncls + lane] = e0 / sum;
     if (lane + 64 < ncls) classes[(size_t)row * ncls + lane + 64] = e1 / sum;
     for (int j = lane; j < ndelta; j += 64) deltas[(size_t)row * ndelta + j] = xr[ncls + j];
+}
+
+__global__ __launch_bounds__(128)
+void splitk_head_finish_kernel(const float* __restrict__ ws, const float* __restrict__ bias, float* __restrict__ y, int ldy, int M, int N,
+                               int splits, int ncls, int ndelta, float* __restrict__ classes, float* __restrict__ deltas)
+{
+    __shared__ float srow[128];
+    const int row = blockIdx.x, col = threadIdx.x;
+    const size_t total = (size_t)M * N;
+    if (col < N) {
+        const float* p = ws + (size_t)row * N + col;
+        float v = p[0];
+        int z = 1;
+        for (; z + 8 <= splits; z += 8) {
+            float t[8];
+#pragma unroll
+            for (int u = 0; u < 8; ++u) t[u] = p[(size_t)(z + u) * total];
+#pragma unroll
+            for (int u = 0; u < 8; ++u) v += t[u];
+        }
+        for (; z < splits; ++z) v += p[(size_t)z * total];
+        v += bias[col];
+        y[(size_t)row * ldy + col] = v;
+        srow[col] = v;
+    }
+    __syncthreads();
+    if (col < 64) {
+        const int lane = col;
+        const float v0 = lane < ncls ? srow[lane] : -INFINITY, v1 = lane + 64 < ncls ? srow[lane + 64] : -INFINITY;
+        float mx = fmaxf(v0, v1);
+#pragma unroll
+        for (int o = 32; o > 0; o >>= 1) mx = fmaxf(mx, __shfl_xor(mx, o));
+        const float e0 = lane < ncls ? expf(v0 - mx) : 0.f, e1 = lane + 64 < ncls ? expf(v1 - mx) : 0.f;
+        float sum = e0 + e1;
+#pragma unroll
+        for (int o = 32; o > 0; o >>= 1) sum += __shfl_xor(sum, o);
+        if (lane < ncls) classes[(size_t)row * ncls + lane] = e0 / sum;
+        if (lane + 64 < ncls) classes[(size_t)row * ncls + lane + 64] = e1 / sum;
+    }
+    if (col >= ncls && col < ncls + ndelta) deltas[(size_t)row * ndelta + col - ncls] = srow[col];
 }
 
 __global__ void pack_fc_chw_to_hwc_kernel(const float* __restrict__ w, float* __restrict__ wp,
@@ -312,6 +352,14 @@
     return p.splits > 1 ? (size_t)p.splits * M * N * sizeof(float) : 0;
 }
 
+int linear_plan_splits(int M, int N, int K, int* stages_per_split)
+{
+    if (M < 1 || N < 1 || K < 16) return 0;
+    const LinearPlan p = plan_linear(M, N, K);
+    if (stages_per_split) *stages_per_split = p.stages_per_split;
+    return p.splits;
+}
+
 template <int TM, int TN, int WM, int WN>
 static int launch_linear_cfg(const LinearPlan& p, const float* a, int lda, const float* w,
                              const float* bias, float* y, int ldy, float* ws, int M, int N, int K,
@@ -356,17 +404,48 @@
     return launch_linear_batched_cfg<1, 2, 2, 2, 1>(a, lda, w, y, ldy, M, N, K, bg, s);
 }
 
-int launch_linear(const float* a, int lda, const float* w, const float* bias, float* y, int ldy,
-                  int M, int N, int K, unsigned flags, void* ws, size_t ws_bytes, hipStream_t s)
+static int launch_linear_gemm(LinearPlan& p, const float* a, int lda, const float* w, const float* bias, float* y, int ldy,
+                              int M, int N, int K, unsigned flags, void* ws, size_t ws_bytes, hipStream_t s)
 {
     if (M < 1 || N < 1 || K < 16 || K % 16 != 0 || lda % 4 != 0 || lda < K || ldy < N) return FRCNN_EINVAL;
-    const LinearPlan p = plan_linear(M, N, K);
+    p = plan_linear(M, N, K);
     const size_t need = p.splits > 1 ? (size_t)p.splits * M * N * sizeof(float) : 0;
     if (need > ws_bytes || (need > 0 && ws == nullptr)) return FRCNN_EINVAL;
     const int relu = (flags & FRCNN_RELU) ? 1 : 0;
-    int rc = p.big ? launch_linear_cfg<5, 1, 2, 4>(p, a, lda, w, bias, y, ldy, (float*)ws, M, N, K, relu, s)
-                   : launch_linear_cfg<2, 2, 2, 2>(p, a, lda, w, bias, y, ldy, (float*)ws, M, N, K, relu, s);
+    return p.big ? launch_linear_cfg<5, 1, 2, 4>(p, a, lda, w, bias, y, ldy, (float*)ws, M, N, K, relu, s)
+                 : launch_linear_cfg<2, 2, 2, 2>(p, a, lda, w, bias, y, ldy, (float*)ws, M, N, K, relu, s);
+}
+
+int launch_linear_head(const float* a, int lda, const float* w, const float* bias, float* logits, int ldy, int M, int ncls, int ndelta,
+                       int K, float* classes, float* deltas, void* ws, size_t ws_bytes, hipStream_t s)
+{
+    const int N = ncls + ndelta;
+    if (ncls < 1 || ncls > 128 || ndelta < 0 || !bias || !classes || !deltas) return FRCNN_EINVAL;
+    LinearPlan p;
+    int rc = launch_linear_gemm(p, a, lda, w, bias, logits, ldy, M, N, K, 0u, ws, ws_bytes, s);
     if (rc != FRCNN_OK) return rc;
+    if (p.splits > 1 && N <= 128) {
+        hipLaunchKernelGGL(splitk_head_finish_kernel, dim3(M), dim3(128), 0, s, (const float*)ws, bias, logits, ldy, M, N, p.splits,
+                           ncls, ndelta, classes, deltas);
+        return check_launch();
+    }
+    if (p.splits > 1) {
+        const size_t total = (size_t)M * N;
+        int blocks = (int)((total + 255) / 256);
+        if (blocks > 2048) blocks = 2048;
+        hipLaunchKernelGGL(splitk_reduce_kernel, dim3(blocks), dim3(256), 0, s, (const float*)ws, bias, logits, ldy, M, N, p.splits, 0);
+        if ((rc = check_launch()) != FRCNN_OK) return rc;
+    }
+    return launch_head_finish(logits, ldy, M, ncls, ndelta, classes, deltas, s);
+}
+
+int launch_linear(const float* a, int lda, const float* w, const float* bias, float* y, int ldy,
+                  int M, int N, int K, unsigned flags, void* ws, size_t ws_bytes, hipStream_t s)
+{
+    LinearPlan p;
+    int rc = launch_linear_gemm(p, a, lda, w, bias, y, ldy, M, N, K, flags, ws, ws_bytes, s);
+    if (rc != FRCNN_OK) return rc;
+    const int relu = (flags & FRCNN_RELU) ? 1 : 0;
     if (p.splits > 1) {
         const size_t total = (size_t)M * N;
         int blocks = (int)((total + 255) / 256);
diff --git a/fasterrcnn_amd/csrc/proposals.hip b/fasterrcnn_amd/csrc/proposals.hip
--- a/fasterrcnn_amd/csrc/proposals.hip
+++ b/fasterrcnn_amd/csrc/proposals.hip
@@ -16,19 +16,11 @@
     return __uint_as_float(b);
 }
 
-__global__ __launch_bounds__(256)
-void rpn_decode_kernel(const float* __restrict__ head, int ld, const float* __restrict__ anchors,
-                       const float* __restrict__ valid, int A, float* __restrict__ scores,
-                       f32x4* __restrict__ boxes_all, u64* __restrict__ keys)
-{
-    const int n = blockIdx.x * 256 + threadIdx.x;
-    if (n >= A) return;
-    const int pix = n / 9, k = n - pix * 9;
-    const float* row = head + (size_t)pix * ld;
-    const float logit = row[k];
+__device__ __forceinline__ void rpn_decode_anchor(float logit, float dy, float dx, float dh, float dw, int n, const float* __restrict__ anchors,
+                                                  const float* __restrict__ valid, float* __restrict__ scores, f32x4* __restrict__ boxes_all,
+                                                  u64* __restrict__ keys)
+{
     const float score = 1.0f / (1.0f + expf(-logit));
-    const float dy = row[9 + 4 * k + 0], dx = row[9 + 4 * k + 1];
-    const float dh = row[9 + 4 * k + 2], dw = row[9 + 4 * k + 3];
     const f32x4 a = reinterpret_cast<const f32x4*>(anchors)[n];
     const float cy = __fadd_rn(__fmul_rn(a[2], dy), a[0]);
     const float cx = __fadd_rn(__fmul_rn(a[3], dx), a[1]);
@@ -41,6 +33,86 @@
     boxes_all[n] = b;
     const bool ok = (valid == nullptr) || (valid[n] > 0.f);
     keys[n] = ok ? (((u64)ordered_bits(score) << 32) | (u64)(unsigned)(n + 1)) : 0ull;
+}
+
+__global__ __launch_bounds__(256)
+void rpn_decode_kernel(const float* __restrict__ head, int ld, const float* __restrict__ anchors,
+                       const float* __restrict__ valid, int A, float* __restrict__ scores,
+                       f32x4* __restrict__ boxes_all, u64* __restrict__ keys)
+{
+    const int n = blockIdx.x * 256 + threadIdx.x;
+    if (n >= A) return;
+    const int pix = n / 9, k = n - pix * 9;
+    const float* row = head + (size_t)pix * ld;
+    rpn_decode_anchor(row[k], row[9 + 4 * k + 0], row[9 + 4 * k + 1], row[9 + 4 * k + 2], row[9 + 4 * k + 3], n, anchors, valid, scores,
+                      boxes_all, keys);
+}
+
+__global__ __launch_bounds__(256)
+void rpn_heads_decode_kernel(const float* __restrict__ a, int lda, const float* __restrict__ w, const float* __restrict__ bias,
+                             float* __restrict__ head, int ld, int M, int K, int stages_per_split, int splits,
+                             const float* __restrict__ anchors, const float* __restrict__ valid, float* __restrict__ scores,
+                             f32x4* __restrict__ boxes_all, u64* __restrict__ keys, int32_t* __restrict__ counts)
+{
+    constexpr int NH = 45, LDP = 65, LDH = 48;
+    __shared__ float part[4][32][LDP];
+    __shared__ float hrow[32][LDH];
+    const int tid = threadIdx.x, lane = tid & 63, z = tid >> 6;
+    const int li = lane & 31, lh = lane >> 5;
+    const int m0 = blockIdx.x * 32;
+    if (blockIdx.x == 0 && tid < 4) counts[tid] = 0;
+    if (z < splits) {
+        const int stages = K >> 4;
+        const int st_begin = z * stages_per_split;
+        const int st_end = min(st_begin + stages_per_split, stages);
+        const int gr = min(m0 + li, M - 1);
+        const float* ap = a + (size_t)gr * lda + 4 * lh;
+        const float* w0 = w + (size_t)li * K + 4 * lh;
+        const float* w1 = w + (size_t)(32 + li) * K + 4 * lh;
+        f32x16 acc0, acc1;
+#pragma unroll
+        for (int r = 0; r < 16; ++r) { acc0[r] = 0.f; acc1[r] = 0.f; }
+#pragma unroll 2
+        for (int st = st_begin; st < st_end; ++st) {
+            const int k0 = st << 4;
+            const f32x4 a0 = *reinterpret_cast<const f32x4*>(ap + k0), a1 = *reinterpret_cast<const f32x4*>(ap + k0 + 8);
+            const f32x4 b00 = *reinterpret_cast<const f32x4*>(w0 + k0), b01 = *reinterpret_cast<const f32x4*>(w0 + k0 + 8);
+            const f32x4 b10 = *reinterpret_cast<const f32x4*>(w1 + k0), b11 = *reinterpret_cast<const f32x4*>(w1 + k0 + 8);
+#pragma unroll
+            for (int kk = 0; kk < 4; ++kk) {
+                acc0 = __builtin_amdgcn_mfma_f32_32x32x2f32(a0[kk], b00[kk], acc0, 0, 0, 0);
+                acc1 = __builtin_amdgcn_mfma_f32_32x32x2f32(a0[kk], b10[kk], acc1, 0, 0, 0);
+            }
+#pragma unroll
+            for (int kk = 0; kk < 4; ++kk) {
+                acc0 = __builtin_amdgcn_mfma_f32_32x32x2f32(a1[kk], b01[kk], acc0, 0, 0, 0);
+                acc1 = __builtin_amdgcn_mfma_f32_32x32x2f32(a1[kk], b11[kk], acc1, 0, 0, 0);
+            }
+        }
+#pragma unroll
+        for (int r = 0; r < 16; ++r) {
+            const int m = (r & 3) + 8 * (r >> 2) + 4 * lh;
+            part[z][m][li] = acc0[r];
+            part[z][m][32 + li] = acc1[r];
+        }
+    }
+    __syncthreads();
+    for (int i = tid; i < 32 * NH; i += 256) {
+        const int m = i / NH, n = i - m * NH;
+        float v = part[0][m][n];
+        for (int q = 1; q < splits; ++q) v += part[q][m][n];
+        v += bias[n];
+        hrow[m][n] = v;
+        if (m0 + m < M) head[(size_t)(m0 + m) * ld + n] = v;
+    }
+    __syncthreads();
+    for (int i = tid; i < 32 * 9; i += 256) {
+        const int m = i / 9, k = i - m * 9;
+        if (m0 + m >= M) continue;
+        const float* row = hrow[m];
+        rpn_decode_anchor(row[k], row[9 + 4 * k + 0], row[9 + 4 * k + 1], row[9 + 4 * k + 2], row[9 + 4 * k + 3], (m0 + m) * 9 + k, anchors,
+                          valid, scores, boxes_all, keys);
+    }
 }
 
 __global__ __launch_bounds__(256)
@@ -810,15 +882,27 @@
                          const float* anchor_map, const float* valid_map, int fh, int fw,
                          int image_h, int image_w, int pre_nms, int post_nms, float nms_thr,
                          float min_side, float* scores, int32_t* sorted_idx, float* props,
-                         int32_t* counts, hipStream_t s)
+                         int32_t* counts, hipStream_t s, const RpnHeadsGemm* fused_heads)
 {
     const int A = fh * fw * 9;
     if (A < 1 || A > ps.a_cap || pre_nms < 1 || pre_nms > ps.pre_cap || post_nms < 1 ||
         post_nms > ps.post_cap || post_nms > 2048 || ld_head < 45)
         return FRCNN_EINVAL;
-    hipLaunchKernelGGL(rpn_decode_kernel, dim3(cdiv(A, 256)), dim3(256), 0, s, head, ld_head, anchor_map,
-                       valid_map, A, scores, reinterpret_cast<f32x4*>(ps.boxes_all), ps.keys);
-    int rc = check_launch();
+    int rc;
+    if (fused_heads != nullptr) {
+        const RpnHeadsGemm& g = *fused_heads;
+        int sps = 0;
+        const int splits = linear_plan_splits(fh * fw, 45, g.K, &sps);
+        if (!g.a || !g.w || !g.bias || g.K < 16 || g.K % 16 != 0 || g.lda < g.K || g.lda % 4 != 0 || splits < 1 || splits > 4)
+            return FRCNN_EINVAL;
+        hipLaunchKernelGGL(rpn_heads_decode_kernel, dim3(cdiv(fh * fw, 32)), dim3(256), 0, s, g.a, g.lda, g.w, g.bias,
+                           const_cast<float*>(head), ld_head, fh * fw, g.K, sps, splits, anchor_map, valid_map, scores,
+                           reinterpret_cast<f32x4*>(ps.boxes_all), ps.keys, counts);
+    } else {
+        hipLaunchKernelGGL(rpn_decode_kernel, dim3(cdiv(A, 256)), dim3(256), 0, s, head, ld_head, anchor_map,
+                           valid_map, A, scores, reinterpret_cast<f32x4*>(ps.boxes_all), ps.keys);
+    }
+    rc = check_launch();
     if (rc) return rc;
     rc = launch_topk<0>(ps.keys, A, pre_nms, ps.boxes_all, (float)image_h, (float)image_w, min_side,
                         sorted_idx, ps.cand_boxes, ps.cand_scores, counts, s, ps.mask);
diff --git a/fasterrcnn_amd/csrc/roipool.hip b/fasterrcnn_amd/csrc/roipool.hip
--- a/fasterrcnn_amd/csrc/roipool.hip
+++ b/fasterrcnn_amd/csrc/roipool.hip
@@ -124,6 +124,30 @@
     *reinterpret_cast<uint4*>(dst + 2048) = make_uint4(lo[0] | (lo[1] << 16), lo[2] | (lo[3] << 16), lo[4] | (lo[5] << 16), lo[6] | (lo[7] << 16));
 }
 
+__device__ __forceinline__ float roi_window_absmax_lane(const float* __restrict__ cmax, int fh, int fw, const f32x4 roi, int pooled, float scale,
+                                                        int lane)
+{
+    const int rs_h = (int)roundf(roi[0] * scale), rs_w = (int)roundf(roi[1] * scale);
+    const int re_h = (int)roundf(roi[2] * scale), re_w = (int)roundf(roi[3] * scale);
+    const int roi_h = max(re_h - rs_h + 1, 1), roi_w = max(re_w - rs_w + 1, 1);
+    const float bin_h = (float)roi_h / (float)pooled, bin_w = (float)roi_w / (float)pooled;
+    const int hs = min(max(rs_h, 0), fh), he = min(max((int)ceilf((float)pooled * bin_h) + rs_h, 0), fh);
+    const int ws = min(max(rs_w, 0), fw), we = min(max((int)ceilf((float)pooled * bin_w) + rs_w, 0), fw);
+    const int ww = we - ws, cells = (he - hs) * ww;
+    float mx = 0.f;
+    for (int i0 = lane; i0 < cells; i0 += 256) {
+        float v[4];
+#pragma unroll
+        for (int u = 0; u < 4; ++u) {
+            const int i = min(i0 + 64 * u, cells - 1);
+            const int h = hs + i / ww, w = ws + i % ww;
+            v[u] = cmax[(size_t)h * fw + w];
+        }
+        mx = fmaxf(fmaxf(mx, fmaxf(v[0], v[1])), fmaxf(v[2], v[3]));
+    }
+    return mx;
+}
+
 __global__ __launch_bounds__(256)
 void roi_scale_x3t_kernel(const float* __restrict__ cmax, int fh, int fw, const float* __restrict__ rois, const int32_t* __restrict__ n_rois,
                           int max_rois, int rec_rows, int pooled, float scale, float* __restrict__ inv)
@@ -134,20 +158,7 @@
     int n = *n_rois;
     if (n > max_rois) n = max_rois;
     float mx = 0.f;
-    if (r < n) {
-        const f32x4 roi = reinterpret_cast<const f32x4*>(rois)[r];
-        const int rs_h = (int)roundf(roi[0] * scale), rs_w = (int)roundf(roi[1] * scale);
-        const int re_h = (int)roundf(roi[2] * scale), re_w = (int)roundf(roi[3] * scale);
-        const int roi_h = max(re_h - rs_h + 1, 1), roi_w = max(re_w - rs_w + 1, 1);
-        const float bin_h = (float)roi_h / (float)pooled, bin_w = (float)roi_w / (float)pooled;
-        const int hs = min(max(rs_h, 0), fh), he = min(max((int)ceilf((float)pooled * bin_h) + rs_h, 0), fh);
-        const int ws = min(max(rs_w, 0), fw), we = min(max((int)ceilf((float)pooled * bin_w) + rs_w, 0), fw);
-        const int ww = we - ws, cells = (he - hs) * ww;
-        for (int i = lane; i < cells; i += 64) {
-            const int h = hs + i / ww, w = ws + i % ww;
-            mx = fmaxf(mx, cmax[(size_t)h * fw + w]);
-        }
-    }
+    if (r < n) mx = roi_window_absmax_lane(cmax, fh, fw, reinterpret_cast<const f32x4*>(rois)[r], pooled, scale, lane);
 #pragma unroll
     for (int off = 32; off >= 1; off >>= 1) mx = fmaxf(mx, __shfl_xor(mx, off));
     float mult, iv;
@@ -217,8 +228,8 @@
 template <int NW>
 __global__ __launch_bounds__(64 * NW)
 void roi_pool_x3t_rows_kernel(const float* __restrict__ fm, int fh, int fw, int C, const float* __restrict__ rois,
-                              const int32_t* __restrict__ n_rois, int max_rois, int pooled, float scale, const float* __restrict__ inv,
-                              unsigned char* __restrict__ rec, int rbt)
+                              const int32_t* __restrict__ n_rois, int max_rois, int pooled, float scale, float* inv,
+                              unsigned char* __restrict__ rec, int rbt, const float* __restrict__ cmax)
 {
     extern __shared__ __attribute__((aligned(16))) float rp_pool[];
     const int tid = threadIdx.x, lane = tid & 63, wave = tid >> 6;
@@ -243,7 +254,17 @@
             ws = (int)floorf((float)pw * bin_w) + rs_w;
             we = (int)ceilf((float)(pw + 1) * bin_w) + rs_w;
             ws = min(max(ws, 0), fw); we = min(max(we, 0), fw);
-            mult = hx_mult_of_inv(inv[r]);
+            if (cmax == nullptr) mult = hx_mult_of_inv(inv[r]);
+        }
+        if (cmax != nullptr) {
+            float mx = 0.f;
+            if (r < n) mx = roi_window_absmax_lane(cmax, fh, fw, reinterpret_cast<const f32x4*>(rois)[r], pooled, scale, lane);
+#pragma unroll
+            for (int off = 32; off >= 1; off >>= 1) mx = fmaxf(mx, __shfl_xor(mx, off));
+            float m_unused, iv;
+            hx_row_scale(mx, m_unused, iv);
+            if (bin == 0 && lane == 0) inv[r] = iv;
+            if (r < n) mult = hx_mult_of_inv(iv);
         }
         const bool any = r < n && he > hs && we > ws;
         for (int c0 = 8 * lane; c0 < C; c0 += 512) {
@@ -436,15 +457,26 @@
 }
 
 int launch_roi_pool_x3t(const float* fm, int fh, int fw, int c, const float* rois, const int32_t* n_rois, int max_rois, int pooled,
-                        float scale, float* cmax, float* inv, void* rec, int rec_rows, hipStream_t s, bool cmax_ready)
+                        float scale, float* cmax, float* inv, void* rec, int rec_rows, hipStream_t s, bool cmax_ready, bool fuse_scale)
 {
     if (fh < 1 || fw < 1 || c < 16 || c % 16 != 0 || max_rois < 1 || pooled < 1 || rec_rows < max_rois || rec_rows % 32 != 0 || !cmax || !inv)
         return FRCNN_EINVAL;
     int rc = cmax_ready ? FRCNN_OK : launch_pixel_absmax(fm, cmax, (long long)fh * fw, c, s);
     if (rc) return rc;
+    const int rbt = rec_rows / 32;
+    const size_t lds = (size_t)32 * (c + 4) * sizeof(float);
+#ifndef FRCNN_ROI_BANDS
+    if (fuse_scale && c % 8 == 0 && lds <= 160 * 1024) {
+        constexpr int NW = FRCNN_ROI_ROWS_WAVES;
+        auto kern = roi_pool_x3t_rows_kernel<NW>;
+        FRCNN_MAX_LDS_ONCE(kern, 160 * 1024);
+        hipLaunchKernelGGL(kern, dim3((unsigned)(pooled * pooled * rbt)), dim3(64 * NW), lds, s, fm, fh, fw, c, rois, n_rois, max_rois, pooled, scale,
+                           inv, static_cast<unsigned char*>(rec), rbt, (const float*)cmax);
+        return check_launch();
+    }
+#endif
     hipLaunchKernelGGL(roi_scale_x3t_kernel, dim3(cdiv(rec_rows, 4)), dim3(256), 0, s, cmax, fh, fw, rois, n_rois, max_rois, rec_rows, pooled, scale, inv);
     if ((rc = check_launch()) != FRCNN_OK) return rc;
-    const int rbt = rec_rows / 32;
 #ifdef FRCNN_ROI_BANDS
     if (pooled == 7 && c % 8 == 0) {
         const long long waves = (long long)rec_rows * pooled;
@@ -453,13 +485,12 @@
         return check_launch();
     }
 #endif
-    const size_t lds = (size_t)32 * (c + 4) * sizeof(float);
     if (c % 8 == 0 && lds <= 160 * 1024) {
         constexpr int NW = FRCNN_ROI_ROWS_WAVES;
         auto kern = roi_pool_x3t_rows_kernel<NW>;
         FRCNN_MAX_LDS_ONCE(kern, 160 * 1024);
         hipLaunchKernelGGL(kern, dim3((unsigned)(pooled * pooled * rbt)), dim3(64 * NW), lds, s, fm, fh, fw, c, rois, n_rois, max_rois, pooled, scale,
-                           inv, static_cast<unsigned char*>(rec), rbt);
+                           inv, static_cast<unsigned char*>(rec), rbt, (const float*)nullptr);
         return check_launch();
     }
     const long long waves = (long long)pooled * pooled * rbt * (c / 16);
```

After: 855.4, median of 6. No clear change (+0.6%).
